# levs57/halo2-liam-eagen-msm

Measured on AMD Instinct MI355X. Metric: BN254 G1 MSM scalar-point-pairs/s, higher is better.
Workload: dtype u32 limbs (256-bit Montgomery integers)

## Files before the change

### halo2_liam_eagen_msm_amd/csrc/fixed_base.inc

```

namespace {

struct FixedPlan { u32 c, W, m, h; u32 kadd[8]; size_t bytes; };

const u32 FIXED_C_MIN = 3, FIXED_C_MAX = 17;

u32 fixed_num_windows(int curve, u32 c, u32 kadd[8]) {
  const u32* order = order_of(curve);
  for (u32 W = (254 + c - 1) / c;; W++) {
    u32 K[8] = {0, 0, 0, 0, 0, 0, 0, 0};
    for (u32 w = 0; w + 1 < W; w++) {
      u32 bit = w * c + c - 1;
      if (bit < 256) K[bit >> 5] |= 1u << (bit & 31);
    }
    u32 s[9]; u64 cy = 0;
    for (int i = 0; i < 8; i++) { cy += (u64)order[i] + K[i] - (i == 0 ? 1u : 0u); s[i] = (u32)cy; cy >>= 32; }
    s[8] = (u32)cy;
    const u32 sh = c * (W - 1);
    u64 top = 0; bool big = s[8] != 0;
    for (int bit = 255; bit >= (int)sh; bit--) {
      if (top >> 62) big = true;
      top = (top << 1) | ((s[bit >> 5] >> (bit & 31)) & 1u);
    }
    if (!big && top < (1ull << (c - 1))) { memcpy(kadd, K, 32); return W; }
  }
}

double fixed_cost(size_t n, u32 c, u32 W, u32 m) {
  const u32 h = (W + m - 1) / m;
  const double slabs = std::ceil((double)n * m / (double)((size_t)1 << MAX_SLAB_LOG));
  return (double)n * W + 2.0 * h * (double)(1u << (c - 1)) + slabs * (double)(1u << 24);
}

const size_t FIXED_AUTO_BYTES = (size_t)16 << 30;

int make_fixed_plan(int curve, size_t n, u32 window_bits, u32 tables, FixedPlan& p) {
  if (curve != LEMSM_BN254_G1 && curve != LEMSM_GRUMPKIN) return LEMSM_ERR_BAD_CURVE;
  if (window_bits && (window_bits < FIXED_C_MIN || window_bits > FIXED_C_MAX)) return LEMSM_ERR_BAD_ARG;
  memset(&p, 0, sizeof p);
  double best = 0; bool have = false;
  for (u32 c = window_bits ? window_bits : FIXED_C_MIN; c <= (window_bits ? window_bits : FIXED_C_MAX); c++) {
    u32 K[8]; const u32 W = fixed_num_windows(curve, c, K);
    if (tables > W) { if (window_bits) return LEMSM_ERR_BAD_ARG; continue; }
    for (u32 m = tables ? tables : 1; m <= (tables ? tables : W); m++) {
      const u32 h = (W + m - 1) / m;
      if (!tables && m > 1 && (W + m - 2) / (m - 1) == h) continue;
      const size_t bytes = (size_t)m * std::max<size_t>(n, 1) * 64;
      if (!tables && m > 1 && bytes > FIXED_AUTO_BYTES) continue;
      const double cost = fixed_cost(n, c, W, m);
      if (!have || cost < best) { best = cost; have = true; p.c = c; p.W = W; p.m = m; p.h = h; memcpy(p.kadd, K, 32); }
    }
  }
  if (!have) return LEMSM_ERR_BAD_ARG;
  p.bytes = (size_t)p.m * n * 64;
  return LEMSM_OK;
}

template <class F>
__global__ __launch_bounds__(256) void k_fixed_table(const uint4* __restrict__ bases, u32 cnt, u32 m, u32 shift,
                                                     uint4* __restrict__ out, char* __restrict__ scratch) {
  typedef XYZZ<F> G; typedef typename F::fe fe;
  const u32 j = blockIdx.x * 256 + threadIdx.x;
  if (j >= cnt) return;
  uint4* o0 = out + (size_t)j * m * 4;
  typename G::aff a;
  F::load(a.x, bases + (size_t)j * 4); F::load(a.y, bases + (size_t)j * 4 + 2);
  for (int q = 0; q < 4; q++) o0[q] = bases[(size_t)j * 4 + q];
  typename G::pt acc; G::from_affine(acc, a);
  fe pref; F::set_one(pref);
  for (u32 k = 1; k < m; k++) {
    for (u32 s = 0; s < shift; s++) { typename G::pt t; G::dbl(t, acc); acc = t; }
    char* sp = scratch + ((size_t)(k - 1) * cnt + j) * 160;
    G::store(sp, acc); F::store(sp + 128, pref);
    if (!G::is_identity(acc)) F::mul(pref, pref, acc.zzz);
  }
  if (m < 2) return;
  fe inv; inv_via_lazy<F>(inv, pref);
  for (u32 k = m - 1; k >= 1; k--) {
    const char* sp = scratch + ((size_t)(k - 1) * cnt + j) * 160;
    typename G::pt q; G::load(q, sp); fe pr; F::load(pr, sp + 128);
    uint4* o = o0 + (size_t)k * 4;
    if (G::is_identity(q)) { uint4 z = make_uint4(0, 0, 0, 0); o[0] = z; o[1] = z; o[2] = z; o[3] = z; continue; }
    fe izzz, izz, x, y;
    F::mul(izzz, inv, pr);
    F::mul(inv, inv, q.zzz);
    F::mul(izz, izzz, q.zz); F::sqr(izz, izz);
    F::mul(x, q.x, izz); F::mul(y, q.y, izzz);
    F::store(o, x); F::store(o + 2, y);
  }
}

struct FixedDigitArgs { KAdd kadd; u32 m, h, W, i0, k0; };

__global__ __launch_bounds__(256) void k_fixed_digits(const uint4* __restrict__ scalars, FixedDigitArgs fa, GroupPlan pl,
                                                      uint16_t* __restrict__ dig16, unsigned long long* __restrict__ signbm,
                                                      u32* __restrict__ block_counts, u32* __restrict__ bin_total, u32* __restrict__ err) {
  __shared__ u32 hist[MAX_BINS];
  const u32 tid = threadIdx.x, r = blockIdx.x;
  for (u32 i = tid; i < pl.nbins; i += 256) hist[i] = 0;
  __syncthreads();
  const u32 c = pl.c, half = 1u << (c - 1);
  const u32 j0 = r * pl.spb, j1 = min(j0 + pl.spb, pl.n);
  for (u32 jb = j0; jb < j1; jb += 256) {
    const u32 j = jb + tid;
    const bool valid = j < j1;
    const u32 kq = fa.k0 + j, q = kq / fa.m, k = kq - q * fa.m;
    const size_t i = (size_t)fa.i0 + q;
    u32 s[8] = {0, 0, 0, 0, 0, 0, 0, 0};
    if (valid) {
      const uint4 a = scalars[2 * i], b = scalars[2 * i + 1];
      s[0] = a.x; s[1] = a.y; s[2] = a.z; s[3] = a.w; s[4] = b.x; s[5] = b.y; s[6] = b.z; s[7] = b.w;
    }
    u32 bw = 0;
#pragma unroll
    for (int w = 0; w < 8; w++) { u32 dmy = __builtin_subc(s[w], fa.kadd.order[w], bw, &bw); (void)dmy; }
    if (valid && !bw) {
      if (k == 0) { atomicAdd(&err[0], 1u); atomicMax(&err[1], ~j); }
#pragma unroll
      for (int w = 0; w < 8; w++) s[w] = 0;
    }
    u32 cy = 0;
#pragma unroll
    for (int w = 0; w < 8; w++) s[w] = __builtin_addc(s[w], fa.kadd.k[w], cy, &cy);
    for (u32 t = pl.w0; t < pl.w1; t++) {
      const u32 ow = k * fa.h + t;
      int d = 0;
      if (valid && ow < fa.W && c * ow < 256) {
        const u32 raw = extract_bits(s, c * ow, c);
        d = (ow + 1 < fa.W) ? (int)raw - (int)half : (int)raw;
      }
      const u32 bucket = (u32)(d < 0 ? -d : d);
      if (c == 17) {
        const u32 neg = d < 0 ? 1u : 0u;
        if (valid) dig16[(size_t)(t - pl.w0) * pl.dstride + j] = (uint16_t)(neg ? bucket - 1u : bucket);
        const unsigned long long bal = __ballot(neg != 0);
        if ((tid & 63u) == 0 && valid) signbm[(size_t)(t - pl.w0) * ((pl.n + 63) / 64) + (j >> 6)] = bal;
      } else if (valid) {
        dig16[(size_t)(t - pl.w0) * pl.dstride + j] = (uint16_t)(d + (int)half);
      }
      if (bucket) atomicAdd(&hist[(t - pl.w0) * pl.BW + ((bucket - 1u) >> pl.LB)], 1u);
    }
  }
  __syncthreads();
  for (u32 i = tid; i < pl.nbins; i += 256) {
    const u32 cnt = hist[i];
    const u32 wl = i / pl.BW, bin = i - wl * pl.BW;
    const size_t slot = ((size_t)wl * pl.nblk1 + r) * pl.BW + bin;
    block_counts[slot] = cnt;
    block_counts[(size_t)pl.nblk1 * pl.nbins + slot] = cnt ? atomicAdd(&bin_total[i], cnt) : 0u;
  }
}

struct FixedProvider {
  const uint4* scalars; FixedDigitArgs fa;
  typedef PipDec Dec;
  int prepare(lemsm_ctx*, hipStream_t st, const GroupPlan& pl, uint16_t* dig16, unsigned long long* signbm, u32* block_counts,
              u32* bin_total, u32* err, Dec& dec) const {
    dec.dig16 = dig16; dec.signbm = pl.c == 17 ? signbm : nullptr;
    hipLaunchKernelGGL(k_fixed_digits, dim3(pl.nblk1), dim3(256), 0, st, scalars, fa, pl, dig16, signbm, block_counts, bin_total, err);
    return LEMSM_OK;
  }
};

}

struct lemsm_fixed_bases { lemsm_ctx* ctx; int device; int curve; size_t n; FixedPlan plan; void* d_table; };

namespace {

template <class P64, class G>
int msm_fixed_t(lemsm_ctx* ctx, const lemsm_fixed_bases* fb, const void* d_scalars, size_t n, u64 out[12]) {
  const FixedPlan& fp = fb->plan;
  const u32 nb = 1u << (fp.c - 1), L = ilog2(nb);
  auto make_src = [&](size_t s0, u32) {
    FixedProvider p; p.scalars = (const uint4*)d_scalars;
    memcpy(p.fa.kadd.k, fp.kadd, 32); memcpy(p.fa.kadd.order, order_of(fb->curve), 32);
    p.fa.m = fp.m; p.fa.h = fp.h; p.fa.W = fp.W; p.fa.i0 = (u32)(s0 / fp.m); p.fa.k0 = (u32)(s0 % fp.m);
    return p;
  };
  std::vector<host::pt> sums;
  int rc = run_windows<P64, G>(ctx, make_src, n * fp.m, fp.c, nb, nb, L, fp.h + 1, 0, fp.h, 0, fb->d_table, sums, true);
  if (rc == LEMSM_ERR_SCALAR_OUT_OF_RANGE) ctx->bad_index /= fp.m;
  if (rc) return rc;
  msm_combine_windows<P64>(fp.c, fp.h, sums.data(), out);
  return LEMSM_OK;
}

}

extern "C" {

int lemsm_fixed_plan(int curve, size_t n, uint32_t window_bits, uint32_t tables, uint32_t* c, uint32_t* num_windows, uint32_t* m,
                     uint32_t* h, size_t* device_bytes) {
  FixedPlan p;
  int rc = make_fixed_plan(curve, n, window_bits, tables, p); if (rc) return rc;
  if (c) *c = p.c;
  if (num_windows) *num_windows = p.W;
  if (m) *m = p.m;
  if (h) *h = p.h;
  if (device_bytes) *device_bytes = p.bytes;
  return LEMSM_OK;
}

int lemsm_fixed_bases_create(lemsm_ctx* ctx, const lemsm_bases* bases, uint32_t window_bits, uint32_t tables, lemsm_fixed_bases** out) {
  if (!ctx || !bases || !out) return LEMSM_ERR_BAD_ARG;
  *out = nullptr;
  if (bases->ctx != ctx) return fail(ctx, LEMSM_ERR_BAD_ARG, "bases belong to another context");
  FixedPlan p;
  int rc = make_fixed_plan(bases->curve, bases->n, window_bits, tables, p);
  if (rc) return fail(ctx, rc, "lemsm_fixed_bases_create: no table geometry for these window_bits / tables");
  HIPCHK(ctx, hipSetDevice(ctx->device));
  const size_t n = bases->n;
  const u32 CHUNK = 1u << 18;
  const size_t scratch_bytes = p.m > 1 ? (size_t)(p.m - 1) * std::min<size_t>(n, CHUNK) * 160 : 0;
  size_t free_b = 0, total_b = 0;
  HIPCHK(ctx, hipMemGetInfo(&free_b, &total_b));
  if (p.bytes + scratch_bytes > free_b) return fail(ctx, LEMSM_ERR_NOMEM, "fixed-base table (" + std::to_string(p.bytes) + " bytes) does not fit in device memory");
  void* d = nullptr;
  hipError_t e = hipMalloc(&d, std::max<size_t>(p.bytes, 64));
  if (e != hipSuccess) { (void)hipGetLastError(); return fail(ctx, LEMSM_ERR_NOMEM, hipGetErrorString(e)); }
  void* scratch = nullptr;
  if (scratch_bytes) {
    e = hipMalloc(&scratch, scratch_bytes);
    if (e != hipSuccess) { (void)hipGetLastError(); (void)hipFree(d); return fail(ctx, LEMSM_ERR_NOMEM, hipGetErrorString(e)); }
  }
  const u32 shift = p.c * p.h;
  for (size_t i0 = 0; i0 < n; i0 += CHUNK) {
    const u32 cnt = (u32)std::min<size_t>(CHUNK, n - i0);
    const uint4* src = (const uint4*)((const char*)bases->d_points + i0 * 64);
    uint4* dst = (uint4*)((char*)d + i0 * p.m * 64);
    if (bases->curve == LEMSM_BN254_G1) hipLaunchKernelGGL((k_fixed_table<FqDev>), dim3((cnt + 255) / 256), dim3(256), 0, ctx->stream, src, cnt, p.m, shift, dst, (char*)scratch);
    else hipLaunchKernelGGL((k_fixed_table<FrDev>), dim3((cnt + 255) / 256), dim3(256), 0, ctx->stream, src, cnt, p.m, shift, dst, (char*)scratch);
  }
  e = hipGetLastError();
  if (e == hipSuccess) e = hipStreamSynchronize(ctx->stream);
  if (scratch) (void)hipFree(scratch);
  if (e != hipSuccess) { (void)hipFree(d); return fail(ctx, LEMSM_ERR_HIP, hipGetErrorString(e)); }
  *out = new lemsm_fixed_bases{ctx, ctx->device, bases->curve, n, p, d};
  return LEMSM_OK;
}

int lemsm_fixed_bases_info(const lemsm_fixed_bases* fb, uint32_t* c, uint32_t* num_windows, uint32_t* m, uint32_t* h, size_t* device_bytes) {
  if (!fb) return LEMSM_ERR_BAD_ARG;
  if (c) *c = fb->plan.c;
  if (num_windows) *num_windows = fb->plan.W;
  if (m) *m = fb->plan.m;
  if (h) *h = fb->plan.h;
  if (device_bytes) *device_bytes = fb->plan.bytes;
  return LEMSM_OK;
}

const void* lemsm_fixed_bases_device_ptr(const lemsm_fixed_bases* fb) { return fb ? fb->d_table : nullptr; }

void lemsm_fixed_bases_free(lemsm_fixed_bases* fb) {
  if (!fb) return;
  (void)hipSetDevice(fb->device);
  (void)hipFree(fb->d_table);
  delete fb;
}

int lemsm_msm_fixed_device(lemsm_ctx* ctx, const lemsm_fixed_bases* fb, const void* d_scalars, size_t n, uint64_t out[12]) {
  if (!ctx || !fb || !out || (n && !d_scalars)) return LEMSM_ERR_BAD_ARG;
  if (fb->ctx != ctx) return fail(ctx, LEMSM_ERR_BAD_ARG, "fixed-base table belongs to another context");
  if (n > fb->n) return fail(ctx, LEMSM_ERR_LEN_MISMATCH, "more scalars than the table has bases");
  if (n == 0) { memset(out, 0, 96); return LEMSM_OK; }
  HIPCHK(ctx, hipSetDevice(ctx->device));
  if (fb->curve == LEMSM_BN254_G1) return msm_fixed_t<host::FqParams64, GqLazy>(ctx, fb, d_scalars, n, out);
  return msm_fixed_t<host::FrParams64, GrLazy>(ctx, fb, d_scalars, n, out);
}

int lemsm_msm_fixed(lemsm_ctx* ctx, const lemsm_fixed_bases* fb, const uint8_t* scalars, size_t n, uint64_t out[12]) {
  if (!ctx || !fb || !out || (n && !scalars)) return LEMSM_ERR_BAD_ARG;
  if (fb->ctx != ctx) return fail(ctx, LEMSM_ERR_BAD_ARG, "fixed-base table belongs to another context");
  if (n > fb->n) return fail(ctx, LEMSM_ERR_LEN_MISMATCH, "more scalars than the table has bases");
  if (n == 0) { memset(out, 0, 96); return LEMSM_OK; }
  HIPCHK(ctx, hipSetDevice(ctx->device));
  int rc = reserve(ctx, ctx->in_s, n * 32); if (rc) return rc;
  HIPCHK(ctx, hipMemcpy(ctx->in_s.p, scalars, n * 32, hipMemcpyHostToDevice));
  return lemsm_msm_fixed_device(ctx, fb, ctx->in_s.p, n, out);
}

}
```

### halo2_liam_eagen_msm_amd/csrc/inst_fq_lazy.hip

```cpp
#include "kernels_ec.cuh"
using namespace lemsm;
typedef XYZZ29<Field29<Fq29Params>> G;
template __global__ void lemsm::k_accum1<G, 2>(GroupPlan, const u32*, const u32*, u32*, const uint4*, char*, u32*, char*);
template __global__ void lemsm::k_accum1<G, 3>(GroupPlan, const u32*, const u32*, u32*, const uint4*, char*, u32*, char*);
template __global__ void lemsm::k_accum1<G, 3, true>(GroupPlan, const u32*, const u32*, u32*, const uint4*, char*, u32*, char*);
template __global__ void lemsm::k_accum1<G, 3, true, true>(GroupPlan, const u32*, const u32*, u32*, const uint4*, char*, u32*, char*);
template __global__ void lemsm::k_accum1<G, 4>(GroupPlan, const u32*, const u32*, u32*, const uint4*, char*, u32*, char*);
template __global__ void lemsm::k_merge_pairs<G>(GroupPlan, u32, MqLayout, const u32*, const u32*, const u32*, const char*, char*, u32*, uint4*);
template __global__ void lemsm::k_merge_serial<G>(u32, MqLayout, const u32*, const uint4*, const char*, char*);
template __global__ void lemsm::k_merge_waves<G>(u32, MqLayout, const u32*, const uint4*, const char*, char*, char*, u32*);
template __global__ void lemsm::k_merge_final<G>(u32, MqLayout, const u32*, const uint4*, const char*, char*, u32*);
template __global__ void lemsm::k_pyramid<G>(const PyrTask*, u32, u32, u32, char*, u32);
template __global__ void lemsm::k_pyramid_first2<G>(PyrFirst2Args, const u32*, char*, u32*);
template __global__ void lemsm::k_pyramid_tail<G>(const PyrTask*, PyrTailArgs, const CopyTaskPod*, u32, char*, u32);
template __global__ void lemsm::k_convert_points<Field29<Fq29Params>>(const uint4*, uint4*, u32);
```

### halo2_liam_eagen_msm_amd/csrc/inst_fq_strict.hip

```cpp
#include "kernels_ec.cuh"
using namespace lemsm;
typedef XYZZ<Field32<FqParams>> G;
template __global__ void lemsm::k_accum1<G, 4>(GroupPlan, const u32*, const u32*, u32*, const uint4*, char*, u32*, char*);
template __global__ void lemsm::k_merge_pairs<G>(GroupPlan, u32, MqLayout, const u32*, const u32*, const u32*, const char*, char*, u32*, uint4*);
template __global__ void lemsm::k_merge_serial<G>(u32, MqLayout, const u32*, const uint4*, const char*, char*);
template __global__ void lemsm::k_merge_waves<G>(u32, MqLayout, const u32*, const uint4*, const char*, char*, char*, u32*);
template __global__ void lemsm::k_merge_final<G>(u32, MqLayout, const u32*, const uint4*, const char*, char*, u32*);
template __global__ void lemsm::k_pyramid<G>(const PyrTask*, u32, u32, u32, char*, u32);
template __global__ void lemsm::k_pyramid_first2<G>(PyrFirst2Args, const u32*, char*, u32*);
template __global__ void lemsm::k_pyramid_tail<G>(const PyrTask*, PyrTailArgs, const CopyTaskPod*, u32, char*, u32);
```

### halo2_liam_eagen_msm_amd/csrc/inst_fr_lazy.hip

```cpp
#include "kernels_ec.cuh"
using namespace lemsm;
typedef XYZZ29<Field29<Fr29Params>> G;
template __global__ void lemsm::k_accum1<G, 2>(GroupPlan, const u32*, const u32*, u32*, const uint4*, char*, u32*, char*);
template __global__ void lemsm::k_accum1<G, 3>(GroupPlan, const u32*, const u32*, u32*, const uint4*, char*, u32*, char*);
template __global__ void lemsm::k_accum1<G, 3, true>(GroupPlan, const u32*, const u32*, u32*, const uint4*, char*, u32*, char*);
template __global__ void lemsm::k_accum1<G, 3, true, true>(GroupPlan, const u32*, const u32*, u32*, const uint4*, char*, u32*, char*);
template __global__ void lemsm::k_accum1<G, 4>(GroupPlan, const u32*, const u32*, u32*, const uint4*, char*, u32*, char*);
template __global__ void lemsm::k_merge_pairs<G>(GroupPlan, u32, MqLayout, const u32*, const u32*, const u32*, const char*, char*, u32*, uint4*);
template __global__ void lemsm::k_merge_serial<G>(u32, MqLayout, const u32*, const uint4*, const char*, char*);
template __global__ void lemsm::k_merge_waves<G>(u32, MqLayout, const u32*, const uint4*, const char*, char*, char*, u32*);
template __global__ void lemsm::k_merge_final<G>(u32, MqLayout, const u32*, const uint4*, const char*, char*, u32*);
template __global__ void lemsm::k_pyramid<G>(const PyrTask*, u32, u32, u32, char*, u32);
template __global__ void lemsm::k_pyramid_first2<G>(PyrFirst2Args, const u32*, char*, u32*);
template __global__ void lemsm::k_pyramid_tail<G>(const PyrTask*, PyrTailArgs, const CopyTaskPod*, u32, char*, u32);
template __global__ void lemsm::k_convert_points<Field29<Fr29Params>>(const uint4*, uint4*, u32);
```

### halo2_liam_eagen_msm_amd/csrc/inst_fr_strict.hip

```cpp
#include "kernels_ec.cuh"
using namespace lemsm;
typedef XYZZ<Field32<FrParams>> G;
template __global__ void lemsm::k_accum1<G, 4>(GroupPlan, const u32*, const u32*, u32*, const uint4*, char*, u32*, char*);
template __global__ void lemsm::k_merge_pairs<G>(GroupPlan, u32, MqLayout, const u32*, const u32*, const u32*, const char*, char*, u32*, uint4*);
template __global__ void lemsm::k_merge_serial<G>(u32, MqLayout, const u32*, const uint4*, const char*, char*);
template __global__ void lemsm::k_merge_waves<G>(u32, MqLayout, const u32*, const uint4*, const char*, char*, char*, u32*);
template __global__ void lemsm::k_merge_final<G>(u32, MqLayout, const u32*, const uint4*, const char*, char*, u32*);
template __global__ void lemsm::k_pyramid<G>(const PyrTask*, u32, u32, u32, char*, u32);
template __global__ void lemsm::k_pyramid_first2<G>(PyrFirst2Args, const u32*, char*, u32*);
template __global__ void lemsm::k_pyramid_tail<G>(const PyrTask*, PyrTailArgs, const CopyTaskPod*, u32, char*, u32);
```

### halo2_liam_eagen_msm_amd/csrc/kernels.cuh

```cuda
#pragma once
#include "kernels_ec.cuh"
#include "inv29.cuh"

namespace lemsm {

__device__ __forceinline__ u32 extract_bits(const u32 (&s)[8], u32 bitpos, u32 c) {
  u32 li = bitpos >> 5, sh = bitpos & 31;
  u32 lo = 0, hi = 0;
#pragma unroll
  for (int i = 0; i < 8; i++) {
    lo = ((u32)i == li) ? s[i] : lo;
    hi = ((u32)i == li + 1) ? s[i] : hi;
  }
  u64 v = ((u64)hi << 32) | lo;
  return (u32)(v >> sh) & ((1u << c) - 1u);
}

struct KAdd { u32 k[8]; u32 order[8]; };

template <int MODE ,
          int BS = 256 >
__global__ __launch_bounds__(BS) void k_pip_digits(const uint4* __restrict__ scalars, KAdd kadd, GroupPlan pl,
                                                    uint16_t* __restrict__ dig16, unsigned long long* __restrict__ signbm,
                                                    u32* __restrict__ block_counts,
                                                    u32* __restrict__ bin_total, u32* __restrict__ err) {
  __shared__ u32 hist[MAX_BINS];
  const u32 tid = threadIdx.x, r = blockIdx.x;
  for (u32 i = tid; i < pl.nbins; i += BS) hist[i] = 0;
  __syncthreads();
  const u32 half = 1u << (pl.c - 1);
  u32 j0 = r * pl.spb, j1 = min(j0 + pl.spb, pl.n);
  for (u32 jb = j0 + tid; jb < j1; jb += BS * 4) {
    uint4 a[4], b[4];
#pragma unroll
    for (int u = 0; u < 4; u++) {
      u32 j = jb + (u32)BS * u;
      if (j < j1) { a[u] = scalars[2 * (size_t)j]; b[u] = scalars[2 * (size_t)j + 1]; }
      else { a[u] = make_uint4(0, 0, 0, 0); b[u] = a[u]; }
    }
#pragma unroll
    for (int u = 0; u < 4; u++) {
      u32 j = jb + (u32)BS * u;
      if (j >= j1) continue;
      u32 s[8] = {a[u].x, a[u].y, a[u].z, a[u].w, b[u].x, b[u].y, b[u].z, b[u].w};
      u32 bw = 0;
#pragma unroll
      for (int i = 0; i < 8; i++) { u32 dmy = __builtin_subc(s[i], kadd.order[i], bw, &bw); (void)dmy; }
      if (!bw) {
        atomicAdd(&err[0], 1u); atomicMax(&err[1], ~j);
#pragma unroll
        for (int i = 0; i < 8; i++) s[i] = 0;
      }
      u32 cy = 0;
#pragma unroll
      for (int i = 0; i < 8; i++) s[i] = __builtin_addc(s[i], kadd.k[i], cy, &cy);
      if (MODE == 2) {
#pragma unroll
        for (int w = 0; w < 15; w++) {
          if ((u32)w < pl.w0 || (u32)w >= pl.w1) continue;
          u32 raw = extract_bits(s, 17u * w, 17u);
          u32 sign = ((u32)w + 1 < pl.W && raw < 65536u) ? 1u : 0u;
          u32 mag = ((u32)w + 1 < pl.W) ? (sign ? 65536u - raw : raw - 65536u) : raw;
          dig16[(size_t)((u32)w - pl.w0) * pl.dstride + j] = (uint16_t)(sign ? mag - 1u : mag);
          unsigned long long bal = __ballot(sign != 0);
          if ((threadIdx.x & 63u) == 0) signbm[(size_t)((u32)w - pl.w0) * ((pl.n + 63) / 64) + (j >> 6)] = bal;
          if (mag) atomicAdd(&hist[((u32)w - pl.w0) * pl.BW + ((mag - 1u) >> pl.LB)], 1u);
        }
      } else if (MODE == 1) {
#pragma unroll
        for (int w = 0; w < 16; w++) {
          if ((u32)w < pl.w0 || (u32)w >= pl.w1) continue;
          u32 raw = (w & 1) ? (s[w >> 1] >> 16) : (s[w >> 1] & 0xffffu);
          dig16[(size_t)((u32)w - pl.w0) * pl.dstride + j] = (uint16_t)raw;
          u32 bucket = ((u32)w + 1 < pl.W) ? (raw < half ? half - raw : raw - half) : raw;
          if (bucket) atomicAdd(&hist[((u32)w - pl.w0) * pl.BW + ((bucket - 1u) >> pl.LB)], 1u);
        }
      } else {
        for (u32 w = pl.w0; w < pl.w1; w++) {
          u32 raw = extract_bits(s, w * pl.c, pl.c);
          dig16[(size_t)(w - pl.w0) * pl.dstride + j] = (uint16_t)raw;
          u32 bucket = (w + 1 < pl.W) ? (raw < half ? half - raw : raw - half) : raw;
          if (bucket) atomicAdd(&hist[(w - pl.w0) * pl.BW + ((bucket - 1u) >> pl.LB)], 1u);
        }
      }
    }
  }
  __syncthreads();
  for (u32 i = tid; i < pl.nbins; i += BS) {
    u32 cnt = hist[i];
    u32 wl = i / pl.BW, bin = i - wl * pl.BW;
    const size_t slot = ((size_t)wl * pl.nblk1 + r) * pl.BW + bin;
    block_counts[slot] = cnt;
    block_counts[(size_t)pl.nblk1 * pl.nbins + slot] = cnt ? atomicAdd(&bin_total[i], cnt) : 0u;
  }
}

struct PipDec {
  static constexpr bool VEC = true;
  const uint16_t* dig16;
  const unsigned long long* signbm;
  __device__ __forceinline__ void get(u32 j, u32 w, const GroupPlan& pl, u32& bucket, u32& sign) const {
    u32 raw = dig16[(size_t)(w - pl.w0) * pl.dstride + j];
    if (signbm) {
      sign = (u32)(signbm[(size_t)(w - pl.w0) * ((pl.n + 63) / 64) + (j >> 6)] >> (j & 63u)) & 1u;
      bucket = sign ? raw + 1u : raw;
      return;
    }
    const u32 half = 1u << (pl.c - 1);
    if (w + 1 < pl.W) {
      sign = raw < half ? 1u : 0u;
      bucket = sign ? half - raw : raw - half;
    } else { sign = 0; bucket = raw; }
  }
};
struct NegDec {
  static constexpr bool VEC = false;
  const uint8_t* digitsT;
  __device__ __forceinline__ void get(u32 j, u32 w, const GroupPlan& pl, u32& bucket, u32& sign) const {
    bucket = digitsT[(size_t)w * pl.nstride + j]; sign = 0;
  }
};

__device__ __forceinline__ u32 block_excl_scan_256(u32 v, u32* total, u32* wsum ) {
  const u32 lane = threadIdx.x & 63, wave = threadIdx.x >> 6;
  u32 x = v;
#pragma unroll
  for (int o = 1; o < 64; o <<= 1) {
    u32 y = __shfl_up(x, o);
    if (lane >= (u32)o) x += y;
  }
  if (lane == 63) wsum[wave] = x;
  __syncthreads();
  u32 base = 0, tot = 0;
#pragma unroll
  for (u32 w = 0; w < 4; w++) {
    u32 s = wsum[w];
    if (w < wave) base += s;
    tot += s;
  }
  __syncthreads();
  *total = tot;
  return base + x - v;
}

static const u32 BW_MAX = 512;
static const u32 STAGE = 4096;
static const u32 STAGE2 = 8192;

template <class Dec>
__global__ __launch_bounds__(256) void k_count1(Dec dec, GroupPlan pl, u32* __restrict__ block_counts,
                                                u32* __restrict__ bin_total) {
  __shared__ u32 hist[256];
  const u32 tid = threadIdx.x, wl = blockIdx.x, r = blockIdx.y, w = pl.w0 + wl;
  hist[tid] = 0;
  __syncthreads();
  u32 j0 = r * pl.spb, j1 = min(j0 + pl.spb, pl.n);
  constexpr int PER = STAGE / 256;
  u32 bk[PER];
#pragma unroll
  for (int k = 0; k < PER; k++) {
    u32 j = j0 + tid + 256u * k, sign;
    bk[k] = 0;
    if (j < j1) dec.get(j, w, pl, bk[k], sign);
  }
  const bool few = pl.BW <= 16u;
  const u32 rep = few ? (tid & 15u) << 4 : 0u;
#pragma unroll
  for (int k = 0; k < PER; k++)
    if (bk[k]) atomicAdd(&hist[rep + ((bk[k] - 1u) >> pl.LB)], 1u);
  __syncthreads();
  if (few) {
    u32 c = 0;
    if (tid < 16u) {
#pragma unroll
      for (int r = 0; r < 16; r++) c += hist[r * 16 + tid];
    }
    __syncthreads();
    if (tid < 16u) hist[tid] = c;
    __syncthreads();
  }
  if (tid < pl.BW) {
    u32 cnt = hist[tid];
    const size_t slot = ((size_t)wl * pl.nblk1 + r) * pl.BW + tid;
    block_counts[slot] = cnt;
    block_counts[(size_t)pl.nblk1 * pl.nbins + slot] = cnt ? atomicAdd(&bin_total[wl * pl.BW + tid], cnt) : 0u;
  }
}

__device__ __forceinline__ u32 block_excl_scan_1024(u32 v, u32* total, u32* wsum ) {
  const u32 lane = threadIdx.x & 63, wave = threadIdx.x >> 6;
  u32 x = v;
#pragma unroll
  for (int o = 1; o < 64; o <<= 1) {
    u32 y = __shfl_up(x, o);
    if (lane >= (u32)o) x += y;
  }
  if (lane == 63) wsum[wave] = x;
  __syncthreads();
  u32 base = 0, tot = 0;
  for (u32 w = 0; w < 16; w++) {
    u32 s = wsum[w];
    if (w < wave) base += s;
    tot += s;
  }
  __syncthreads();
  *total = tot;
  return base + x - v;
}

__global__ __launch_bounds__(1024) void k_binscan(GroupPlan pl, const u32* __restrict__ bin_total,
                                                  u32* __restrict__ bin_start, u32* __restrict__ tile_prefix,
                                                  u32* __restrict__ meta) {
  __shared__ u32 wsum[16];
  const u32 t = threadIdx.x;
  constexpr int PB = MAX_BINS / 1024;
  u32 cnt[PB], tl[PB], s = 0, st = 0;
#pragma unroll
  for (int k = 0; k < PB; k++) {
    u32 b = t * PB + k;
    cnt[k] = b < pl.nbins ? bin_total[b] : 0;
    tl[k] = (pl.bin_cap && cnt[k] <= pl.bin_cap) ? 0u : (cnt[k] + pl.T2 - 1) / pl.T2;
    s += cnt[k]; st += tl[k];
  }
  u32 tot, tott;
  u32 off = block_excl_scan_1024(s, &tot, wsum);
  u32 offt = block_excl_scan_1024(st, &tott, wsum);
#pragma unroll
  for (int k = 0; k < PB; k++) {
    u32 b = t * PB + k;
    if (b < pl.nbins) { bin_start[b] = off; tile_prefix[b] = offt; }
    off += cnt[k]; offt += tl[k];
  }
  if (t == 0) {
    bin_start[pl.nbins] = tot; tile_prefix[pl.nbins] = tott;
    meta[META_M] = tot; meta[META_TILES] = tott;
  }
}

template <class Dec, int STG , int BS = 256,
          bool LEAN = false >
__global__ __launch_bounds__(BS) void k_scatter1(Dec dec, GroupPlan pl, const u32* __restrict__ block_counts,
                                                 const u32* __restrict__ bin_start,
                                                 u32* __restrict__ entries, u32 xcd_windows ) {
  static_assert(BS == 256 || BS == 1024, "block size");
  static_assert(STG <= 16384, "jl field is 14 bits");
  static_assert(!LEAN || BS == 256, "the lean form is the 256-thread one");
  __shared__ __align__(8) u32 delta[BW_MAX];
  __shared__ __align__(8) u32 lcur[BW_MAX];
  __shared__ u32 wsum[16];
  __shared__ u32 stage[STG];
  const u32 tid = threadIdx.x;
  u32 wl, r;
  if (xcd_windows) {
    const u32 wpx = (pl.w1 - pl.w0 + 7u) >> 3, slot = blockIdx.x >> 3;
    wl = (blockIdx.x & 7u) + 8u * (slot % wpx); r = slot / wpx;
    if (wl >= pl.w1 - pl.w0) return;
  } else { wl = blockIdx.x; r = blockIdx.y; }
  const u32 w = pl.w0 + wl;
  const u32 lmask = (1u << pl.LB) - 1u;
  u32 j0 = r * pl.spb, j1 = min(j0 + pl.spb, pl.n);
  constexpr int PER = STG / BS;
  u32 bk[PER];
  u32 jl0, jls;
  if constexpr (Dec::VEC) {
    static_assert(PER == 16 || PER == 32, "digits per thread");
    jl0 = tid * PER; jls = 1;
    const u32 jb = j0 + jl0;
    uint4 dv[PER / 8];
    u32 sbits = 0;
    if (jb < j1) {
      const uint4* p = (const uint4*)(dec.dig16 + (size_t)wl * pl.dstride + jb);
#pragma unroll
      for (int v = 0; v < PER / 8; v++) dv[v] = p[v];
      if (dec.signbm) {
        const unsigned long long* sw = dec.signbm + (size_t)wl * ((pl.n + 63) / 64);
        if (PER == 16) sbits = ((const uint16_t*)sw)[jb >> 4]; else sbits = ((const u32*)sw)[jb >> 5];
      }
    } else {
#pragma unroll
      for (int v = 0; v < PER / 8; v++) dv[v] = make_uint4(0, 0, 0, 0);
    }
    const u32 half = 1u << (pl.c - 1);
    const bool top = !(w + 1 < pl.W);
#pragma unroll
    for (int k = 0; k < PER; k++) {
      const uint4 q4 = dv[k / 8];
      const u32 word = ((k / 2) % 4 == 0) ? q4.x : ((k / 2) % 4 == 1) ? q4.y : ((k / 2) % 4 == 2) ? q4.z : q4.w;
      const u32 raw = (k & 1) ? (word >> 16) : (word & 0xffffu);
      u32 bucket, sign;
      if (dec.signbm) { sign = (sbits >> k) & 1u; bucket = raw + sign; }
      else if (top) { sign = 0; bucket = raw; }
      else { sign = raw < half ? 1u : 0u; bucket = sign ? half - raw : raw - half; }
      bk[k] = (jb + (u32)k < j1 && bucket) ? (bucket | (sign << 31)) : 0u;
    }
  } else {
    jl0 = tid; jls = BS;
#pragma unroll
    for (int k = 0; k < PER; k++) {
      u32 j = j0 + tid + (u32)BS * k, b = 0, sgn = 0;
      if (j < j1) dec.get(j, w, pl, b, sgn);
      bk[k] = b ? (b | (sgn << 31)) : 0u;
    }
  }
  const size_t crow = ((size_t)wl * pl.nblk1 + r) * pl.BW;
  const u32* __restrict__ block_offs = block_counts + (size_t)pl.nblk1 * pl.nbins;
  u32 total;
  const bool few = !Dec::VEC && BS == 256 && !LEAN && pl.BW <= 16u;
  if (few) {
    lcur[tid] = 0;
    __syncthreads();
#pragma unroll
    for (int k = 0; k < PER; k++)
      if (bk[k]) atomicAdd(&lcur[((((bk[k] & 0x7fffffffu) - 1u) >> pl.LB) << 4) | (tid & 15u)], 1u);
    __syncthreads();
    const u32 v = lcur[tid];
    const u32 off = block_excl_scan_256(v, &total, wsum);
    lcur[tid] = off;
    const u32 b = tid >> 4;
    if ((tid & 15u) == 0 && b < pl.BW) delta[b] = bin_start[wl * pl.BW + b] + block_offs[crow + b] - off;
  } else
  if constexpr (LEAN) {
    const u32 b0 = 2u * tid;
    const bool h = b0 < pl.BW;
    const uint2 z2 = make_uint2(0u, 0u);
    const uint2 cnt = h ? *reinterpret_cast<const uint2*>(block_counts + crow + b0) : z2;
    const uint2 clm = h ? *reinterpret_cast<const uint2*>(block_offs + crow + b0) : z2;
    const uint2 bs = h ? *reinterpret_cast<const uint2*>(bin_start + (size_t)wl * pl.BW + b0) : z2;
    const u32 off0 = block_excl_scan_256(cnt.x + cnt.y, &total, wsum), off1 = off0 + cnt.x;
    *reinterpret_cast<uint2*>(&delta[b0]) = make_uint2(bs.x + clm.x - off0, bs.y + clm.y - off1);
    *reinterpret_cast<uint2*>(&lcur[b0]) = make_uint2(off0, off1);
  } else if constexpr (BS == 256) {
    const bool h0 = tid < pl.BW, h1 = tid + 256u < pl.BW;
    u32 cnt0 = h0 ? block_counts[crow + tid] : 0u, cnt1 = h1 ? block_counts[crow + tid + 256u] : 0u;
    u32 g0 = h0 ? bin_start[wl * pl.BW + tid] + block_offs[crow + tid] : 0u;
    u32 g1 = h1 ? bin_start[wl * pl.BW + tid + 256u] + block_offs[crow + tid + 256u] : 0u;
    u32 total0, total1;
    u32 off0 = block_excl_scan_256(cnt0, &total0, wsum);
    u32 off1 = block_excl_scan_256(cnt1, &total1, wsum) + total0;
    total = total0 + total1;
    delta[tid] = g0 - off0; delta[tid + 256u] = g1 - off1;
    lcur[tid] = off0; lcur[tid + 256u] = off1;
  } else {
    const bool h0 = tid < pl.BW;
    u32 cnt0 = h0 ? block_counts[crow + tid] : 0u;
    u32 g0 = h0 ? bin_start[wl * pl.BW + tid] + block_offs[crow + tid] : 0u;
    u32 off0 = block_excl_scan_1024(cnt0, &total, wsum);
    if (tid < BW_MAX) { delta[tid] = g0 - off0; lcur[tid] = off0; }
  }
  __syncthreads();
#pragma unroll
  for (int k = 0; k < PER; k++) {
    if (bk[k]) {
      u32 kk = (bk[k] & 0x7fffffffu) - 1u, b = kk >> pl.LB;
      u32 q = atomicAdd(&lcur[few ? ((b << 4) | (tid & 15u)) : b], 1u);
      if constexpr (LEAN) stage[q] = (bk[k] & 0x80000000u) | (jl0 + jls * (u32)k) | (b << 14) | ((kk & lmask) << 24);
      else stage[q] = (jl0 + jls * (u32)k) | ((kk & lmask) << 14) | ((bk[k] >> 31) << 21) | (b << 22);
    }
  }
  __syncthreads();
  if constexpr (LEAN) {
    u32 v[PER];
#pragma unroll
    for (int k = 0; k < PER; k++) { const u32 q = tid + (u32)BS * k; v[k] = q < total ? stage[q] : 0u; }
#pragma unroll
    for (int k = 0; k < PER; k++) {
      const u32 q = tid + (u32)BS * k;
      if (q < total) entries[delta[(v[k] >> 14) & 511u] + q] = (v[k] & 0xff003fffu) + j0;
    }
  } else {
    for (u32 q = tid; q < total; q += BS) {
      u32 v = stage[q];
      entries[delta[v >> 22] + q] = (j0 + (v & 0x3fffu)) | (((v >> 14) & 127u) << 24) | (((v >> 21) & 1u) << 31);
    }
  }
}

__global__ __launch_bounds__(256) void k_tilemap(GroupPlan pl, const u32* __restrict__ bin_start,
                                                 const u32* __restrict__ tile_prefix, const u32* __restrict__ meta,
                                                 uint4* __restrict__ tile_info) {
  u32 t = blockIdx.x * 256 + threadIdx.x;
  if (t >= pl.max_tiles) return;
  if (t >= meta[META_TILES]) { tile_info[t] = make_uint4(0, 0, 0, 0); return; }
  u32 lo = 0, hi = pl.nbins;
  while (hi - lo > 1) {
    u32 mid = (lo + hi) >> 1;
    if (tile_prefix[mid] <= t) lo = mid; else hi = mid;
  }
  u32 off = bin_start[lo] + (t - tile_prefix[lo]) * pl.T2;
  u32 end = min(off + pl.T2, bin_start[lo + 1]);
  tile_info[t] = make_uint4(lo, off, end, 1u);
}
__device__ __forceinline__ bool locate_tile(const uint4* __restrict__ tile_info, u32 t, u32& bin, u32& off, u32& end) {
  uint4 ti = tile_info[t];
  bin = ti.x; off = ti.y; end = ti.z;
  return ti.w != 0;
}

__global__ __launch_bounds__(256) void k_count2(GroupPlan pl, const u32* __restrict__ entries,
                                                const uint4* __restrict__ tile_info, u32* __restrict__ bucket_count) {
  __shared__ u32 hist[1u << MAX_LB];
  const u32 tid = threadIdx.x;
  for (u32 t = blockIdx.x; t < pl.max_tiles; t += gridDim.x) {
    u32 bin, off, end;
    if (!locate_tile(tile_info, t, bin, off, end)) return;
    if (tid < (1u << MAX_LB)) hist[tid] = 0;
    __syncthreads();
    constexpr int PER = STAGE2 / 256;
    u32 e[PER];
#pragma unroll
    for (int k = 0; k < PER; k++) { u32 i = off + tid + 256u * k; e[k] = i < end ? entries[i] : 0xffffffffu; }
#pragma unroll
    for (int k = 0; k < PER; k++) { u32 i = off + tid + 256u * k; if (i < end) atomicAdd(&hist[(e[k] >> 24) & 127u], 1u); }
    __syncthreads();
    if (tid < (1u << pl.LB)) {
      u32 cnt = hist[tid];
      if (cnt) atomicAdd(&bucket_count[(bin << pl.LB) + tid], cnt);
    }
    __syncthreads();
  }
}

__global__ __launch_bounds__(256) void k_bucketscan(GroupPlan pl, const u32* __restrict__ bin_start,
                                                    const u32* __restrict__ bucket_count,
                                                    u32* __restrict__ bucket_start) {
  __shared__ u32 ex[256];
  __shared__ u32 wsum[4];
  const u32 tid = threadIdx.x;
  const u32 key = blockIdx.x * 256 + tid;
  const u32 nkeys = pl.nbins << pl.LB;
  u32 cnt = key < nkeys ? bucket_count[key] : 0u;
  u32 total;
  u32 e = block_excl_scan_256(cnt, &total, wsum);
  ex[tid] = e;
  __syncthreads();
  if (key < nkeys) {
    u32 first = tid & ~((1u << pl.LB) - 1u);
    const u32 b0 = bin_start[key >> pl.LB];
    if (!(pl.bin_cap && bin_start[(key >> pl.LB) + 1] - b0 <= pl.bin_cap))
      bucket_start[key] = b0 + (e - ex[first]);
  }
  if (key == 0) bucket_start[nkeys] = bin_start[pl.nbins];
}

__global__ __launch_bounds__(256) void k_scatter2(GroupPlan pl, const u32* __restrict__ entries,
                                                  const uint4* __restrict__ tile_info, const u32* __restrict__ bucket_start,
                                                  u32* __restrict__ bucket_cursor, u32* __restrict__ sorted) {
  __shared__ u32 hist[256];
  __shared__ u32 lstart[257];
  __shared__ u32 delta[256];
  __shared__ u32 wsum[4];
  __shared__ u32 stage[STAGE2];
  const u32 tid = threadIdx.x;
  for (u32 t = blockIdx.x; t < pl.max_tiles; t += gridDim.x) {
    u32 bin, off, end;
    if (!locate_tile(tile_info, t, bin, off, end)) return;
    hist[tid] = 0;
    __syncthreads();
    constexpr int PER = STAGE2 / 256;
    u32 e[PER], rk[PER];
#pragma unroll
    for (int k = 0; k < PER; k++) { u32 i = off + tid + 256u * k; e[k] = i < end ? entries[i] : 0xffffffffu; }
#pragma unroll
    for (int k = 0; k < PER; k++) {
      u32 i = off + tid + 256u * k;
      rk[k] = i < end ? atomicAdd(&hist[(e[k] >> 24) & 127u], 1u) : 0u;
    }
    __syncthreads();
    u32 cnt = tid < (1u << pl.LB) ? hist[tid] : 0u;
    u32 total;
    u32 o = block_excl_scan_256(cnt, &total, wsum);
    lstart[tid] = o;
    if (tid == 255) lstart[256] = total;
    u32 key = (bin << pl.LB) + tid;
    delta[tid] = cnt ? bucket_start[key] + atomicAdd(&bucket_cursor[key], cnt) - o : 0u;
    __syncthreads();
#pragma unroll
    for (int k = 0; k < PER; k++) {
      u32 i = off + tid + 256u * k;
      if (i < end) {
        u32 l = (e[k] >> 24) & 127u;
        stage[lstart[l] + rk[k]] = e[k];
      }
    }
    __syncthreads();
    for (u32 q = tid; q < total; q += 256) {
      u32 v = stage[q];
      sorted[delta[(v >> 24) & 127u] + q] = v & 0x80ffffffu;
    }
    __syncthreads();
  }
}

static const u32 BIN_CAP = 36864;
static const u32 BIN_CAP_SMALL = 8192;
template <u32 CAP>
__global__ __launch_bounds__(1024) void k_binsort(GroupPlan pl, const u32* __restrict__ entries, const u32* __restrict__ bin_start,
                                                  u32* __restrict__ sorted, u32* __restrict__ bucket_start) {
  __shared__ u32 stage[CAP];
  __shared__ u32 hist[256];
  __shared__ u32 lstart[256];
  __shared__ u32 wsum[4];
  const u32 tid = threadIdx.x, bin = blockIdx.x;
  const u32 off = bin_start[bin], end = bin_start[bin + 1], cnt = end - off;
  if (cnt > pl.bin_cap) return;
  const u32 nl = 1u << pl.LB, lmask = nl - 1u;
  if (tid < 256) hist[tid] = 0;
  __syncthreads();
  constexpr int PER = CAP / 1024;
  u32 e[PER], rk[PER];
#pragma unroll
  for (int k = 0; k < PER; k++) { u32 i = off + tid + 1024u * k; e[k] = i < end ? entries[i] : 0u; }
#pragma unroll
  for (int k = 0; k < PER; k++) {
    u32 i = off + tid + 1024u * k;
    rk[k] = i < end ? atomicAdd(&hist[(e[k] >> 24) & lmask], 1u) : 0u;
  }
  __syncthreads();
  if (tid < 256) {
    u32 c = tid < nl ? hist[tid] : 0u, total;
    const u32 lane = tid & 63, wave = tid >> 6;
    u32 x = c;
#pragma unroll
    for (int o = 1; o < 64; o <<= 1) { u32 y = __shfl_up(x, o); if (lane >= (u32)o) x += y; }
    if (lane == 63) wsum[wave] = x;
    lstart[tid] = x - c;
    (void)total;
  }
  __syncthreads();
  const u32 wb1 = wsum[0], wb2 = wb1 + wsum[1], wb3 = wb2 + wsum[2];
  if (tid < nl) {
    u32 l = tid, base = l < 64 ? 0u : (l < 128 ? wb1 : (l < 192 ? wb2 : wb3));
    bucket_start[(bin << pl.LB) + l] = off + base + lstart[l];
  }
#pragma unroll
  for (int k = 0; k < PER; k++) {
    u32 i = off + tid + 1024u * k;
    if (i < end) {
      u32 l = (e[k] >> 24) & lmask, base = l < 64 ? 0u : (l < 128 ? wb1 : (l < 192 ? wb2 : wb3));
      stage[base + lstart[l] + rk[k]] = e[k] & 0x80ffffffu;
    }
  }
  __syncthreads();
  for (u32 q = tid; q < cnt; q += 1024) sorted[off + q] = stage[q];
}

__global__ void k_copy_points(const CopyTask* __restrict__ tasks, u32 ntasks, u32 nwin, u32 pt_bytes, char* __restrict__ arena) {
  u32 gid = blockIdx.x * blockDim.x + threadIdx.x;
  u32 wpp = pt_bytes / 16;
  u32 word = gid % wpp; u32 r = gid / wpp;
  u32 ti = r / nwin, w = r - ti * nwin;
  if (ti >= ntasks) return;
  CopyTask tk = tasks[ti];
  uint4 v = make_uint4(0, 0, 0, 0);
  if (tk.src_idx < tk.src_valid_idx)
    v = reinterpret_cast<const uint4*>(arena + ((size_t)tk.src_off + (size_t)w * tk.src_wstride + tk.src_idx) * pt_bytes)[word];
  reinterpret_cast<uint4*>(arena + ((size_t)tk.dst_off + (size_t)w * tk.dst_wstride) * pt_bytes)[word] = v;
}

__global__ __launch_bounds__(256) void k_negbase_digits(const uint4* __restrict__ scalars, u32 n, u32 base, u32 d,
                                                        const u32* __restrict__ bound , int check_range,
                                                        uint8_t* __restrict__ digits, uint8_t* __restrict__ digitsT,
                                                        u32* __restrict__ err, u32 row_begin, u32 row_end ,
                                                        const uint8_t* __restrict__ negative = nullptr ,
                                                        uint8_t* __restrict__ trunc = nullptr ) {
  u32 j = blockIdx.x * 256 + threadIdx.x;
  if (j >= n) return;
  uint4 a = scalars[2 * (size_t)j], b = scalars[2 * (size_t)j + 1];
  u32 s[8] = {a.x, a.y, a.z, a.w, b.x, b.y, b.z, b.w};
  u32 bw = 0;
#pragma unroll
  for (int i = 0; i < 8; i++) { u32 dummy = __builtin_subc(s[i], bound[i], bw, &bw); (void)dummy; }
  bool in_range = bw != 0;
  if (check_range && !in_range) { atomicMin(&err[0], j); }
  u32 h[16];
#pragma unroll
  for (int i = 0; i < 8; i++) { h[2 * i] = s[i] & 0xffffu; h[2 * i + 1] = s[i] >> 16; }
  bool neg = negative ? negative[j] != 0 : false;
  {
    u32 nz0 = 0;
#pragma unroll
    for (int k = 0; k < 16; k++) nz0 |= h[k];
    if (!nz0) neg = false;
  }
  const float rb = 1.0f / (float)base;
  const u32 shift = (base & (base - 1u)) == 0 ? (u32)__builtin_ctz(base) : 0u;
  u32 i_begin = 0;
  if (shift && !(s[4] | s[5] | s[6] | s[7])) {
    u32 m0 = s[0], m1 = s[1], m2 = s[2], m3 = s[3];
    for (u32 i = 0; i < d; i++) {
      const u32 rem = m0 & (base - 1u);
      m0 = __builtin_amdgcn_alignbit(m1, m0, shift); m1 = __builtin_amdgcn_alignbit(m2, m1, shift);
      m2 = __builtin_amdgcn_alignbit(m3, m2, shift); m3 >>= shift;
      u32 digit;
      if (!neg) { digit = rem; neg = true; }
      else {
        digit = rem ? base - rem : 0u;
        if (rem) {
          m0 += 1u; const u32 c0 = m0 == 0u; m1 += c0; const u32 c1 = c0 & (m1 == 0u); m2 += c1; const u32 c2 = c1 & (m2 == 0u); m3 += c2;
        }
        neg = false;
      }
      if (!(m0 | m1 | m2 | m3)) neg = false;
      if (digits) digits[(size_t)j * d + i] = (uint8_t)digit;
      if (digitsT && i >= row_begin && i < row_end) digitsT[(size_t)i * n + j] = (uint8_t)digit;
    }
    h[0] = m0 & 0xffffu; h[1] = m0 >> 16; h[2] = m1 & 0xffffu; h[3] = m1 >> 16; h[4] = m2 & 0xffffu; h[5] = m2 >> 16; h[6] = m3 & 0xffffu; h[7] = m3 >> 16;
    i_begin = d;
  }
  for (u32 i = i_begin; i < d; i++) {
    u32 rem = 0;
    if (shift) {
      rem = h[0] & (base - 1u);
#pragma unroll
      for (int k = 0; k < 16; k++) {
        u32 nxt = k < 15 ? h[k + 1] : 0u;
        h[k] = ((h[k] | (nxt << 16)) >> shift) & 0xffffu;
      }
    } else {
#pragma unroll
      for (int k = 15; k >= 0; k--) {
        u32 cur = (rem << 16) | h[k];
        u32 q = (u32)((float)cur * rb);
        int r = (int)cur - (int)(q * base);
        if (r < 0) { q--; r += (int)base; }
        if (r >= (int)base) { q++; r -= (int)base; }
        h[k] = q; rem = (u32)r;
      }
    }
    u32 digit;
    if (!neg) { digit = rem; neg = true; }
    else {
      digit = rem ? base - rem : 0u;
      if (rem) {
        u32 cy = 1;
#pragma unroll
        for (int k = 0; k < 16; k++) { u32 v = h[k] + cy; h[k] = v & 0xffffu; cy = v >> 16; }
      }
      neg = false;
    }
    u32 nz = 0;
#pragma unroll
    for (int k = 0; k < 16; k++) nz |= h[k];
    if (!nz) neg = false;
    if (digits) digits[(size_t)j * d + i] = (uint8_t)digit;
    if (digitsT && i >= row_begin && i < row_end) digitsT[(size_t)i * n + j] = (uint8_t)digit;
  }
  u32 nz = 0;
// ... 165 lines not shown
```

### halo2_liam_eagen_msm_amd/csrc/kernels_ec.cuh

```cuda
#pragma once
#include "plan.h"
#include "xyzz.cuh"
#include "xyzz29.cuh"

namespace lemsm {

static const u32 KEY_NONE = 0xffffffffu;

enum { META_M = 0, META_TILES = 1, META_WORDS = 4, META_CLOCK = 8  };

template <class G, int WPS ,
          bool ABI = false ,
          bool RING = false >
__global__ __launch_bounds__(256, WPS) void k_accum1(GroupPlan pl, const u32* __restrict__ sorted,
                                                const u32* __restrict__ bucket_start, u32* __restrict__ meta,
                                                const uint4* __restrict__ points, char* __restrict__ bucket_sum,
                                                u32* __restrict__ rec_key, char* __restrict__ rec_pt) {
  typedef typename G::F_ F;
  typedef typename F::fe fe;
  const u32 t = blockIdx.x * 256 + threadIdx.x;
  if (t >= pl.nthr1) return;
  const u32 M = meta[META_M];
  const bool stamp = blockIdx.x == (gridDim.x >> 1) && threadIdx.x == 0;
  if (stamp) {
    u64* ck = reinterpret_cast<u64*>(meta + META_CLOCK);
    ck[0] = __builtin_amdgcn_s_memtime(); ck[1] = __builtin_amdgcn_s_memrealtime();
  }
  const u64 s64 = (u64)t * pl.L1;
  const u32 r0 = 2 * t;
  if (s64 >= M) { rec_key[t] = KEY_NONE; return; }
  const u32 start = (u32)s64;
  const u32 end = (u32)min((u64)M, s64 + pl.L1);

  u32 lo = 0, hi = pl.nbins << pl.LB;
  while (hi - lo > 1) {
    u32 mid = (lo + hi) >> 1;
    if (bucket_start[mid] <= start) lo = mid; else hi = mid;
  }
  const u32 nkeys = pl.nbins << pl.LB;
  u32 key = lo;
  u32 kbeg = bucket_start[key];
  u32 kend = bucket_start[key + 1];
  u32 kend2 = bucket_start[min(key + 2u, nkeys)], kend3 = bucket_start[min(key + 3u, nkeys)];
  u32 seg_begin = start;

  typename G::pt acc; G::set_identity(acc);
  bool empty = true;

  auto flush = [&](u32 seg_end) {
    bool complete = (seg_begin == kbeg) && (seg_end == kend);
    if (complete) {
      G::store(bucket_sum + (size_t)key * G::PT_BYTES, acc);
    } else {
      G::store(rec_pt + (size_t)(r0 + (seg_end == end ? 1u : 0u)) * G::PT_BYTES, acc);
    }
  };

  __shared__ u32 ering[RING ? 4 : 1][2][4][64][RING ? 4 : 1];
  const u32 wv = threadIdx.x >> 6, lane = threadIdx.x & 63u;
  auto ring_fill = [&](u32 blk) {
#pragma unroll
    for (int k = 0; k < 4; k++)
      __builtin_amdgcn_global_load_lds((const __attribute__((address_space(1))) void*)(sorted + start + 16u * blk + 4u * k),
                                       (__attribute__((address_space(3))) void*)&ering[wv][blk & 1u][k][0][0], 16, 0, 0);
  };
  auto ring_read = [&](u32 rel) -> u32 { return ering[wv][(rel >> 4) & 1u][(rel >> 2) & 3u][lane][rel & 3u]; };
  u32 e_next;
  if constexpr (RING) {
    ring_fill(0);
    if (pl.L1 > 16) ring_fill(1);
    asm volatile("s_waitcnt vmcnt(0)" ::: "memory");
    e_next = ring_read(0);
  } else {
    e_next = sorted[start];
  }
  uint4 nx0, nx1, ny0, ny1;
  { const uint4* p = points + (size_t)(e_next & 0xffffffu) * 4; nx0 = p[0]; nx1 = p[1]; ny0 = p[2]; ny1 = p[3]; }

  for (u32 i = start; i < end; i++) {
    u32 e = e_next; fe px, py;
    F::from_words(px, nx0, nx1); F::from_words(py, ny0, ny1);
    if (i >= kend) {
      flush(i);
      key++; kend = kend2; kend2 = kend3;
      while (i >= kend) { key++; kend = kend2; kend2 = bucket_start[min(key + 2u, nkeys)]; }
      kbeg = i; seg_begin = i;
      G::set_identity(acc); empty = true;
    }
    if (i + 1 < end) {
      if constexpr (RING) {
        const u32 rel1 = i + 1 - start;
        if ((rel1 & 15u) == 0) asm volatile("s_waitcnt vmcnt(0)" ::: "memory");
        e_next = ring_read(rel1);
        if ((rel1 & 15u) == 0 && rel1 + 16u < pl.L1) ring_fill((rel1 >> 4) + 1u);
      } else {
        e_next = sorted[i + 1];
      }
      const uint4* p = points + (size_t)(e_next & 0xffffffu) * 4;
      nx0 = p[0]; nx1 = p[1]; ny0 = p[2]; ny1 = p[3];
    }
    kend3 = bucket_start[min(key + 3u, nkeys)];
    if (!G::aff_is_identity(px, py)) {
      F::cneg(py, py, (e >> 31) != 0);
      if (ABI) G::madd_abi(acc, px, py, empty); else G::madd(acc, px, py, empty);
    }
  }
  flush(end);
  if (stamp) {
    u64* ck = reinterpret_cast<u64*>(meta + META_CLOCK);
    ck[2] = __builtin_amdgcn_s_memtime(); ck[3] = __builtin_amdgcn_s_memrealtime();
  }
  rec_key[t] = (seg_begin == kbeg && end != kend) ? key : KEY_NONE;
}

enum { MQ_S = 0, MQ_M = 1, MQ_L = 2, MQ_F = 3, MQ_P = 4, MQ_WORDS = 16  };
static const u32 MQ_DST_BUCKET = 0xffffffffu;

template <class G>
__device__ __forceinline__ void merge_load_piece(typename G::pt& q, const char* __restrict__ rec_pt, u32 t, bool first_slot, u32 scaled) {
  G::load(q, rec_pt + (size_t)(2u * t + (first_slot ? 0u : 1u)) * G::PT_BYTES);
  if (scaled) G::unscale(q);
}

template <class G>
__global__ __launch_bounds__(256) void k_merge_pairs(GroupPlan pl, u32 scaled, MqLayout lay, const u32* __restrict__ bucket_start,
                                                     const u32* __restrict__ meta, const u32* __restrict__ rec_key,
                                                     const char* __restrict__ rec_pt, char* __restrict__ bucket_sum,
                                                     u32* __restrict__ mq_cnt, uint4* __restrict__ mq_items) {
  __shared__ u32 lc[5], lbase[5];
  const u32 t = blockIdx.x * 256 + threadIdx.x;
  if (threadIdx.x < 5) lc[threadIdx.x] = 0;
  __syncthreads();
  const u32 key = t < pl.nthr1 ? rec_key[t] : KEY_NONE;
  u32 P = 0, lastfirst = 0, cls = 0, loff = 0, nsub = 0, poff = 0, foff = 0;
  if (key != KEY_NONE) {
    const u32 e = bucket_start[key + 1], M = meta[META_M];
    const u32 tb = (e - 1u) / pl.L1;
    P = tb - t + 1u;
    lastfirst = ((u64)(tb + 1u) * pl.L1 == (u64)e || e == M) ? 0u : 1u;
    cls = P == 2 ? 1u : (P <= 8 ? 2u : (P <= 32 ? 3u : 4u));
    if (cls == 2) loff = atomicAdd(&lc[MQ_S], 1u);
    else if (cls == 3) loff = atomicAdd(&lc[MQ_M], 1u);
    else if (cls == 4) {
      nsub = (P + lay.slice - 1u) / lay.slice;
      loff = atomicAdd(&lc[MQ_L], nsub);
      if (nsub > 1) { poff = atomicAdd(&lc[MQ_P], nsub); foff = atomicAdd(&lc[MQ_F], 1u); }
    }
  }
  __syncthreads();
  if (threadIdx.x < 5) lbase[threadIdx.x] = lc[threadIdx.x] ? atomicAdd(&mq_cnt[threadIdx.x], lc[threadIdx.x]) : 0u;
  __syncthreads();
  if (cls == 2) { u32 i = lbase[MQ_S] + loff; if (i < lay.capS) mq_items[lay.offS + i] = make_uint4(key, t, P | (lastfirst << 31), MQ_DST_BUCKET); }
  else if (cls == 3) { u32 i = lbase[MQ_M] + loff; if (i < lay.capM) mq_items[lay.offM + i] = make_uint4(key, t, P | (lastfirst << 31), MQ_DST_BUCKET); }
  else if (cls == 4) {
    const u32 i0 = lbase[MQ_L] + loff, p0 = lbase[MQ_P] + poff;
    for (u32 k = 0; k < nsub; k++) {
      const u32 cnt = min(lay.slice, P - k * lay.slice);
      const u32 lf = (k + 1 == nsub) ? lastfirst : 0u;
      if (i0 + k < lay.capL) mq_items[lay.offL + i0 + k] = make_uint4(key, t + k * lay.slice, cnt | (lf << 31), nsub > 1 ? p0 + k : MQ_DST_BUCKET);
    }
    if (nsub > 1) { u32 f = lbase[MQ_F] + foff; if (f < lay.capF) mq_items[lay.offF + f] = make_uint4(key, p0, nsub, 0); }
  }
  if (cls == 1) {
    typename G::pt acc, q;
    merge_load_piece<G>(acc, rec_pt, t, false, scaled);
    merge_load_piece<G>(q, rec_pt, t + 1u, lastfirst != 0, scaled);
    G::add(acc, q);
    if (scaled) G::scale(acc);
    G::store(bucket_sum + (size_t)key * G::PT_BYTES, acc);
  }
}

template <class G, bool FROM_PARTIALS>
__device__ __forceinline__ u32 merge_wave_sum(typename G::pt& acc, u32 lane, u32 n, u32 t0, u32 lf, u32 scaled,
                                              const char* __restrict__ src, u32 cap) {
  G::set_identity(acc);
  u32 m = 1; while (m < n && m < 64u) m <<= 1;
  const u32 nser = (n + 63u) >> 6;
  const u32 nscan = m <= 16u ? (u32)__builtin_ctz(m) : (m == 32u ? 5u : 6u);
#pragma unroll 1
  for (u32 s = 0; s < nser + nscan; s++) {
    typename G::pt q;
    if (s < nser) {
      const u32 j = (lane & (m - 1u)) + 64u * s;
      if (j < n) {
        if constexpr (FROM_PARTIALS) { if (t0 + j < cap) G::load(q, src + (size_t)(t0 + j) * G::PT_BYTES); else G::set_identity(q); }
        else merge_load_piece<G>(q, src, t0 + j, j + 1 == n && lf, scaled);
      } else G::set_identity(q);
    } else {
      G::scan_fetch(q, acc, (int)(s - nser));
    }
    G::add(acc, q);
  }
  return m - 1u;
}

static const u32 MERGE_LDS_PAD_WORDS = 21504;

template <class G>
__global__ __launch_bounds__(256) void k_merge_serial(u32 scaled, MqLayout lay, const u32* __restrict__ mq_cnt,
                                                      const uint4* __restrict__ mq_items, const char* __restrict__ rec_pt,
                                                      char* __restrict__ bucket_sum) {
  __shared__ u32 pad_[MERGE_LDS_PAD_WORDS];
  if (scaled > 1) pad_[threadIdx.x] = scaled;
  const u32 cS = min(mq_cnt[MQ_S], lay.capS), cMall = min(mq_cnt[MQ_M], lay.capM);
  const u32 cM = cMall > lay.wave_th ? cMall : 0u;
  const u32 chS = (cS + 63u) >> 6, chM = (cM + 63u) >> 6;
  const u32 lane = threadIdx.x & 63u;
#pragma unroll 1
  for (u32 c = blockIdx.x + gridDim.x * (threadIdx.x >> 6); c < chS + chM; c += gridDim.x * 4u) {
    uint4 it;
    if (c < chS) { const u32 v = 64u * c + lane; if (v >= cS) continue; it = mq_items[lay.offS + v]; }
    else { const u32 v = 64u * (c - chS) + lane; if (v >= cM) continue; it = mq_items[lay.offM + v]; }
    const u32 key = it.x, t0 = it.y, n = it.z & 0x7fffffffu, lf = it.z >> 31;
    typename G::pt acc, q; G::set_identity(acc);
#pragma unroll 1
    for (u32 j = 0; j < n; j++) {
      merge_load_piece<G>(q, rec_pt, t0 + j, j + 1 == n && lf, scaled);
      G::add(acc, q);
    }
    if (scaled) G::scale(acc);
    G::store(bucket_sum + (size_t)key * G::PT_BYTES, acc);
  }
}

template <class G>
__global__ __launch_bounds__(256) void k_merge_waves(u32 scaled, MqLayout lay, const u32* __restrict__ mq_cnt,
                                                     const uint4* __restrict__ mq_items, const char* __restrict__ rec_pt,
                                                     char* __restrict__ partial, char* __restrict__ bucket_sum, u32* __restrict__ dbg) {
  __shared__ u32 pad_[MERGE_LDS_PAD_WORDS];
  if (scaled > 1) pad_[threadIdx.x] = scaled;
  const unsigned long long tk0 = __builtin_amdgcn_s_memtime();
  const u32 cMall = min(mq_cnt[MQ_M], lay.capM), cL = min(mq_cnt[MQ_L], lay.capL);
  const u32 lane = threadIdx.x & 63u;
  const u32 nwaves = gridDim.x * 4u;
  const u32 cM = cMall > lay.wave_th ? 0u : cMall;
#pragma unroll 1
  for (u32 w = blockIdx.x * 4u + (threadIdx.x >> 6); w < cM + cL; w += nwaves) {
    const uint4 it = w < cM ? mq_items[lay.offM + w] : mq_items[lay.offL + (w - cM)];
    const u32 key = it.x, dst = it.w;
    typename G::pt acc;
    const unsigned long long tk1 = __builtin_amdgcn_s_memtime();
    const u32 rl = merge_wave_sum<G, false>(acc, lane, it.z & 0x7fffffffu, it.y, it.z >> 31, scaled, rec_pt, 0);
    const unsigned long long tk2 = __builtin_amdgcn_s_memtime();
    if (lane == rl) {
      if (dst == MQ_DST_BUCKET) { if (scaled) G::scale(acc); G::store(bucket_sum + (size_t)key * G::PT_BYTES, acc); }
      else if (dst < lay.capP) G::store(partial + (size_t)dst * G::PT_BYTES, acc);
    }
    if (dbg && w == 0 && lane == 0) { dbg[8] = (u32)(tk1 - tk0); dbg[9] = (u32)(tk2 - tk1); dbg[10] = (u32)(__builtin_amdgcn_s_memtime() - tk2); dbg[11] = it.z; }
  }
}

template <class G>
__global__ __launch_bounds__(256) void k_merge_final(u32 scaled, MqLayout lay, const u32* __restrict__ mq_cnt, const uint4* __restrict__ mq_items,
                                                     const char* __restrict__ partial, char* __restrict__ bucket_sum, u32* __restrict__ dbg) {
  __shared__ u32 pad_[MERGE_LDS_PAD_WORDS];
  if (scaled > 1) pad_[threadIdx.x] = scaled;
  const unsigned long long tk0 = __builtin_amdgcn_s_memtime();
  const u32 cF = min(mq_cnt[MQ_F], lay.capF);
  const u32 lane = threadIdx.x & 63u, nwaves = gridDim.x * 4u;
#pragma unroll 1
  for (u32 w = blockIdx.x * 4u + (threadIdx.x >> 6); w < cF; w += nwaves) {
    const uint4 it = mq_items[lay.offF + w];
    typename G::pt acc;
    const unsigned long long tk1 = __builtin_amdgcn_s_memtime();
    const u32 rl = merge_wave_sum<G, true>(acc, lane, it.z, it.y, 0, 0, partial, lay.capP);
    const unsigned long long tk2 = __builtin_amdgcn_s_memtime();
    if (lane == rl) { if (scaled) G::scale(acc); G::store(bucket_sum + (size_t)it.x * G::PT_BYTES, acc); }
    if (dbg && w == 0 && lane == 0) { dbg[12] = (u32)(tk1 - tk0); dbg[13] = (u32)(tk2 - tk1); dbg[14] = (u32)(__builtin_amdgcn_s_memtime() - tk2); dbg[15] = it.z; }
  }
}

typedef CopyTask CopyTaskPod;


template <class G>
__device__ __forceinline__ void pyr_item(const PyrTask& tk, u32 w, u32 i, char* __restrict__ arena) {
  u32 ia = (2 * i) * tk.stride + tk.phase, ib = (2 * i + 1) * tk.stride + tk.phase;
  const char* src = arena + ((size_t)tk.src_off + (size_t)w * tk.src_wstride) * G::PT_BYTES;
  typename G::pt a, b;
  if (ia < tk.src_valid) G::load(a, src + (size_t)ia * G::PT_BYTES); else G::set_identity(a);
  if (ib < tk.src_valid) G::load(b, src + (size_t)ib * G::PT_BYTES); else G::set_identity(b);
  if (tk.src_scaled) { G::unscale(a); G::unscale(b); }
  G::add(a, b);
  G::store(arena + ((size_t)tk.dst_off + (size_t)w * tk.dst_wstride + i) * G::PT_BYTES, a);
}

template <class G>
__device__ __forceinline__ bool pyr_try4(const PyrTask& tk, u32 w, u32 i, char* __restrict__ arena, u32 q) {
  if constexpr (G::CONVERTED_DOMAIN) {
    const u32 ia = (2 * i) * tk.stride + tk.phase, ib = (2 * i + 1) * tk.stride + tk.phase;
    if (ia >= tk.src_valid || ib >= tk.src_valid || tk.src_scaled) return false;
    const char* src = arena + ((size_t)tk.src_off + (size_t)w * tk.src_wstride) * G::PT_BYTES;
    return G::add4_mem(src + (size_t)ia * G::PT_BYTES, src + (size_t)ib * G::PT_BYTES,
                       arena + ((size_t)tk.dst_off + (size_t)w * tk.dst_wstride + i) * G::PT_BYTES, q);
  } else return false;
}

template <class G>
__global__ __launch_bounds__(256) void k_pyramid(const PyrTask* __restrict__ tasks, u32 ntasks, u32 nwin,
                                                 u32 max_count, char* __restrict__ arena, u32 quad ) {
  const u32 t = blockIdx.x * 256 + threadIdx.x;
  const u32 gid = quad ? t >> 2 : t;
  u32 per_task = max_count * nwin;
  u32 ti = gid / per_task;
  if (ti >= ntasks) return;
  u32 rem = gid - ti * per_task;
  u32 w = rem / max_count, i = rem - w * max_count;
  PyrTask tk = tasks[ti];
  if (i >= tk.count) return;
  bool serial = true;
  if (quad) serial = !pyr_try4<G>(tk, w, i, arena, t & 3u) && (t & 3u) == 0u;
  if (serial) pyr_item<G>(tk, w, i, arena);
}

template <class G>
__global__ __launch_bounds__(256) void k_sum_slabs(char* __restrict__ bucket_sum, u32 nbuckets, u32 nslabs, u32 scaled_mask) {
  const u32 i = blockIdx.x * 256 + threadIdx.x;
  if (i >= nbuckets) return;
  typename G::pt acc, q;
  G::load(acc, bucket_sum + (size_t)i * G::PT_BYTES);
  if (scaled_mask & 1u) G::unscale(acc);
#pragma unroll 1
  for (u32 k = 1; k < nslabs; k++) {
    G::load(q, bucket_sum + ((size_t)k * nbuckets + i) * G::PT_BYTES);
    if ((scaled_mask >> k) & 1u) G::unscale(q);
    G::add(acc, q);
  }
  G::store(bucket_sum + (size_t)i * G::PT_BYTES, acc);
}


struct PyrFirst2Args {
  u32 nwin, nb, nbw, nbp;
  u32 bucket_off, a2_off, r02_off, r11_off, wstride;
  u32 scaled;
};

template <class G>
__global__ __launch_bounds__(256, 1) void k_pyramid_first2(PyrFirst2Args a, const u32* __restrict__ bucket_start, char* __restrict__ arena, u32* __restrict__ dbg) {
  const unsigned long long tk0 = __builtin_amdgcn_s_memtime(), tr0 = __builtin_amdgcn_s_memrealtime();
  const u32 gid = blockIdx.x * 256 + threadIdx.x;
  const u32 per_win = a.nbp >> 3;
  const u32 w = gid / per_win, i = gid - w * per_win;
  if (w >= a.nwin) return;
  const u32 key0 = w * a.nbw + 8u * i;
  typename G::pt A, B, D, x, y;
  G::set_identity(A); G::set_identity(B); G::set_identity(D);
  const size_t o_a2 = (size_t)a.a2_off + (size_t)w * a.wstride + 2u * i;
  const size_t o_r02 = (size_t)a.r02_off + (size_t)w * a.wstride + i, o_r11 = (size_t)a.r11_off + (size_t)w * a.wstride + i;
  auto operands = [&](u32 step, u32& kx, u32& ky, size_t& tx, size_t& ty) {
    kx = 8; ky = 8; tx = ~(size_t)0; ty = ~(size_t)0;
    switch (step) {
      case 0: kx = 0; ky = 1; break;
      case 1: kx = 2; ky = 3; break;
      case 3: ty = o_r11; break;
      case 4: kx = 4; ky = 5; break;
      case 5: ky = 7; break;
      case 6: tx = o_r02; break;
      case 7: kx = 6; ky = 7; break;
      case 9: tx = o_r11; break;
      default: break;
    }
    if (kx < 8) tx = (size_t)a.bucket_off + key0 + kx;
    if (ky < 8) ty = (size_t)a.bucket_off + key0 + ky;
  };
  uint4 rx[G::RAW_WORDS], ry[G::RAW_WORDS];
  {
    u32 kx, ky; size_t tx, ty; operands(0, kx, ky, tx, ty);
    G::load_raw(rx, arena + tx * G::PT_BYTES); G::load_raw(ry, arena + ty * G::PT_BYTES);
  }
  u32 have = 0;
#pragma unroll
  for (u32 k = 0; k < 8; k++)
    if (8u * i + k < a.nb && bucket_start[key0 + k + 1] != bucket_start[key0 + k]) have |= 1u << k;
#pragma unroll 1
  for (u32 step = 0; step < 10; step++) {
    {
      u32 kx, ky; size_t tx, ty; operands(step, kx, ky, tx, ty);
      if (tx != ~(size_t)0) { G::from_raw(x, rx); if (kx < 8) { if (!((have >> kx) & 1u)) G::set_identity(x); else if (a.scaled) G::unscale(x); } }
      if (ty != ~(size_t)0) { G::from_raw(y, ry); if (ky < 8) { if (!((have >> ky) & 1u)) G::set_identity(y); else if (a.scaled) G::unscale(y); } }
      if (step < 9) {
        operands(step + 1, kx, ky, tx, ty);
        if (tx != ~(size_t)0) G::load_raw(rx, arena + tx * G::PT_BYTES);
        if (ty != ~(size_t)0) G::load_raw(ry, arena + ty * G::PT_BYTES);
      }
    }
    switch (step) {
      case 0: B = y; break;
      case 1: D = y; break;
      case 2: x = B; y = D; break;
      case 3: x = A; break;
      case 4: D = y; break;
      case 5: x = D; break;
      case 6: y = D; break;
      case 8: x = A; y = B; break;
      case 9: y = B; break;
      default: break;
    }
    const unsigned long long ta0 = __builtin_amdgcn_s_memtime();
    G::add(x, y);
    if (dbg && gid == 0) { if (step == 2) dbg[8] = (u32)(__builtin_amdgcn_s_memtime() - ta0); if (step == 0) dbg[9] = (u32)(__builtin_amdgcn_s_memtime() - tk0); }
    size_t dst = ~(size_t)0;
    switch (step) {
      case 0: A = x; break;
      case 1: dst = o_r11; break;
      case 2: dst = o_r02; break;
      case 3: dst = o_a2; break;
      case 4: A = x; break;
      case 5: D = x; break;
      case 6: dst = o_r02; break;
      case 7: B = x; break;
      case 8: dst = o_a2 + 1; break;
      default: dst = o_r11; break;
    }
    if (dst != ~(size_t)0) G::store(arena + dst * G::PT_BYTES, x);
  }
  if (dbg && gid == 0) { dbg[10] = (u32)(__builtin_amdgcn_s_memtime() - tk0); dbg[11] = (u32)(__builtin_amdgcn_s_memrealtime() - tr0); }
}

struct PyrTailArgs { u32 first, last, max_count[20], step_off[21]; };
template <class G>
__global__ __launch_bounds__(1024) __attribute__((amdgpu_waves_per_eu(4, 4))) void k_pyramid_tail(const PyrTask* __restrict__ tasks, PyrTailArgs ta, const CopyTaskPod* __restrict__ copy,
                                                       u32 do_copy, char* __restrict__ arena, u32 quad ) {
  const u32 w = blockIdx.x, tid = threadIdx.x;
  for (u32 s = ta.first; s <= ta.last; s++) {
    const u32 k = s - ta.first;
    const u32 nt = ta.step_off[k + 1] - ta.step_off[k], mc = ta.max_count[k];
    const u32 lanes = quad ? 4u * nt * mc : nt * mc;
    for (u32 t = tid; t < lanes; t += 1024) {
      const u32 it = quad ? t >> 2 : t;
      const u32 ti = it / mc, i = it - ti * mc;
      PyrTask tk = tasks[ta.step_off[k] + ti];
      bool serial = i < tk.count;
      if (quad && serial) serial = !pyr_try4<G>(tk, w, i, arena, t & 3u) && (t & 3u) == 0u;
      if (serial) pyr_item<G>(tk, w, i, arena);
    }
    __threadfence_block();
    __syncthreads();
  }
  if (do_copy) {
    const u32 wpp = G::PT_BYTES / 16;
    if (tid < wpp) {
      CopyTaskPod tk = *copy;
      uint4 v = make_uint4(0, 0, 0, 0);
      if (tk.src_idx < tk.src_valid_idx)
        v = reinterpret_cast<const uint4*>(arena + ((size_t)tk.src_off + (size_t)w * tk.src_wstride + tk.src_idx) * G::PT_BYTES)[tid];
      reinterpret_cast<uint4*>(arena + ((size_t)tk.dst_off + (size_t)w * tk.dst_wstride) * G::PT_BYTES)[tid] = v;
    }
  }
}

template <class F29>
__global__ __launch_bounds__(256) void k_convert_points(const uint4* __restrict__ in, uint4* __restrict__ out, u32 n) {
  u32 i = blockIdx.x * 256 + threadIdx.x;
  if (i >= 2 * n) return;
  typename F29::fe a, r;
  F29::load(a, in + 2 * (size_t)i);
  F29::from_abi(r, a);
  F29::store(out + 2 * (size_t)i, r);
}

}
```

### halo2_liam_eagen_msm_amd/csrc/lemsm.hip

```cpp
#include <hip/hip_runtime.h>
#include <math.h>
#include <stdio.h>
#include <stdlib.h>
#include <string.h>

#include <algorithm>
#include <cmath>
#include <map>
#include <string>
#include <vector>

#include "../../include/lemsm.h"
#include "hostmath.hpp"
#include "hostpool.hpp"
#include "hosttail.hpp"
#include <memory>
#include "kernels.cuh"
#include "rccl_dyn.hpp"
#include "roctx_dyn.hpp"
#include "divisor.cuh"
#include "regfn_eval.cuh"
#include <rocprim/rocprim.hpp>
#include <chrono>
#include <functional>
#include <thread>

using namespace lemsm;

namespace {

typedef Field32<FqParams> FqDev;
typedef Field32<FrParams> FrDev;
typedef XYZZ<FqDev> GqStrict;
typedef XYZZ<FrDev> GrStrict;
typedef XYZZ29<Field29<Fq29Params>> GqLazy;
typedef XYZZ29<Field29<Fr29Params>> GrLazy;

const u32 ORDER_R[8] = {0xf0000001u, 0x43e1f593u, 0x79b97091u, 0x2833e848u, 0x8181585du, 0xb85045b6u, 0xe131a029u, 0x30644e72u};
const u32 ORDER_P[8] = {0xd87cfd47u, 0x3c208c16u, 0x6871ca8du, 0x97816a91u, 0x8181585du, 0xb85045b6u, 0xe131a029u, 0x30644e72u};
const u32 BOUND_R[8] = {0xc7b81b1bu, 0xc6fb4e9fu, 0xeeb859fcu, 0x6f4d8248u, 0, 0, 0, 0};
const u32 BOUND_P[8] = {0xc7b81b1cu, 0xc6fb4e9fu, 0xeeb859fcu, 0x6f4d8248u, 0, 0, 0, 0};

const u32* order_of(int curve) { return curve == LEMSM_BN254_G1 ? ORDER_R : ORDER_P; }
const u32* bound_of(int curve) { return curve == LEMSM_BN254_G1 ? BOUND_R : BOUND_P; }

}
#define LEMSM_EXTERN_G(G)                                                                                   \
  extern template __global__ void lemsm::k_merge_pairs<G>(GroupPlan, u32, MqLayout, const u32*, const u32*, const u32*, const char*, char*, u32*, uint4*); \
  extern template __global__ void lemsm::k_merge_serial<G>(u32, MqLayout, const u32*, const uint4*, const char*, char*); \
  extern template __global__ void lemsm::k_merge_waves<G>(u32, MqLayout, const u32*, const uint4*, const char*, char*, char*, u32*); \
  extern template __global__ void lemsm::k_merge_final<G>(u32, MqLayout, const u32*, const uint4*, const char*, char*, u32*); \
  extern template __global__ void lemsm::k_pyramid<G>(const PyrTask*, u32, u32, u32, char*, u32); \
  extern template __global__ void lemsm::k_pyramid_first2<G>(PyrFirst2Args, const u32*, char*, u32*); \
  extern template __global__ void lemsm::k_pyramid_tail<G>(const PyrTask*, PyrTailArgs, const CopyTaskPod*, u32, char*, u32);
#define LEMSM_EXTERN_ACC(G, W) \
  extern template __global__ void lemsm::k_accum1<G, W>(GroupPlan, const u32*, const u32*, u32*, const uint4*, char*, u32*, char*);
LEMSM_EXTERN_G(GqStrict) LEMSM_EXTERN_G(GrStrict) LEMSM_EXTERN_G(GqLazy) LEMSM_EXTERN_G(GrLazy)
LEMSM_EXTERN_ACC(GqStrict, 4) LEMSM_EXTERN_ACC(GrStrict, 4)
LEMSM_EXTERN_ACC(GqLazy, 2) LEMSM_EXTERN_ACC(GqLazy, 3) LEMSM_EXTERN_ACC(GqLazy, 4)
LEMSM_EXTERN_ACC(GrLazy, 2) LEMSM_EXTERN_ACC(GrLazy, 3) LEMSM_EXTERN_ACC(GrLazy, 4)
extern template __global__ void lemsm::k_accum1<GqLazy, 3, true>(GroupPlan, const u32*, const u32*, u32*, const uint4*, char*, u32*, char*);
extern template __global__ void lemsm::k_accum1<GrLazy, 3, true>(GroupPlan, const u32*, const u32*, u32*, const uint4*, char*, u32*, char*);
extern template __global__ void lemsm::k_accum1<GqLazy, 3, true, true>(GroupPlan, const u32*, const u32*, u32*, const uint4*, char*, u32*, char*);
extern template __global__ void lemsm::k_accum1<GrLazy, 3, true, true>(GroupPlan, const u32*, const u32*, u32*, const uint4*, char*, u32*, char*);
extern template __global__ void lemsm::k_convert_points<Field29<Fq29Params>>(const uint4*, uint4*, u32);
extern template __global__ void lemsm::k_convert_points<Field29<Fr29Params>>(const uint4*, uint4*, u32);
namespace {

struct DevBuf {
  void* p = nullptr;
  size_t cap = 0;
};


struct PyrCacheEntry { DevBuf buf; PyrPlan pp; };

}

struct HostStage { const uint8_t* h_scalars; const void* h_points; char* d_scalars; char* d_points; };

struct lemsm_ctx {
  int device = 0;
  u32 num_cus = 256;
  hipStream_t stream = nullptr;
  hipStream_t stream_sort = nullptr;
  hipStream_t stream_tail = nullptr;
  std::vector<hipEvent_t> evpool;
  hipEvent_t wait_accum = nullptr;
  hipEvent_t ev_call_done = nullptr;
  hipEvent_t ev_batch_up = nullptr;
  hipEvent_t dw_ev[2] = {nullptr, nullptr};
  hipEvent_t ev[5] = {nullptr, nullptr, nullptr, nullptr, nullptr};
  DevBuf ws;
  DevBuf in_s;
  DevBuf in_p;
  DevBuf in_aux;
  DevBuf gather;
  DevBuf fail_buf;
  DevBuf dw_tab, dw_arena, dw_tmp;
  u32 dw_logn = 0, dw_gexp = 0;
  double dw_ntt_ms = 0; u64 dw_ntt_bytes = 0, dw_ntt_bflies = 0; u32 dw_reuse_levels = 0;
  DevBuf rf_coef, rf_ws;
  double rf_ms = 0; u64 rf_bytes = 0, rf_mults = 0;
  double dw_phase_ms[4] = {0, 0, 0, 0};
  ncclComm_t comm = nullptr; int comm_size = 1, comm_rank = 0;
  int plan_world = 1;
  u32* h_small = nullptr;
  lemsm_ctx* peer = nullptr;
  void* h_pin = nullptr; size_t h_pin_cap = 0;
  std::unique_ptr<lemsm::host::Pool> pool;
  std::string last_error;
  long opt_host_threads = 0;
  long opt_window_bits = 0, opt_chunk = 0, opt_tile = 0, opt_field = 0, opt_accum_waves = 0, opt_groups = 0, opt_host_slab_bits = 0, opt_slab_bits = 0, opt_abi_points = 0, opt_stage2x = 0, opt_xcd_windows = 0, opt_entry_ring = 0, opt_validate_points = 0, opt_pyr_fuse = 0, opt_ntt_tiled = 0, opt_ws_canary = 0, opt_binsort = 0, opt_dw_wrap = 0, opt_dw_fuse = 0, opt_dw_kb = 0, opt_merge_slice = 0, opt_merge_wave_th = 0, opt_dbg_repeat = 0, opt_pyr_first2 = 0, opt_dw_reuse = 0, opt_dw_pw_lazy = 0, opt_dw_halves = 0, opt_dw_ntt_lazy = 0, opt_slab_tail = 0, opt_pyr_quad = 0, opt_scatter_lean = 0;
  u32 plan_slab_n = 0;
  bool plan_ring = false;
  const struct HostStage* host_stage = nullptr;
  double t_total_ms = 0, t_accum_ms = 0; int n_accum = 0;
  double host_us[4] = {0, 0, 0, 0};
  uint32_t dbg_stamps[8] = {0, 0, 0, 0, 0, 0, 0, 0};
  uint64_t dbg_merge[4] = {0, 0, 0, 0};
  double accum_clock_mhz = 0;
  size_t bad_index = 0;
  size_t truncated = 0;
  std::map<std::vector<u32>, PyrCacheEntry> pyr_cache;
};

namespace {

#define HIPCHK(ctx, expr)                                                                   \
  do {                                                                                      \
    hipError_t e_ = (expr);                                                                 \
    if (e_ != hipSuccess) {                                                                 \
      (ctx)->last_error = std::string(#expr) + ": " + hipGetErrorString(e_);                \
      return LEMSM_ERR_HIP;                                                                 \
    }                                                                                       \
  } while (0)

int fail(lemsm_ctx* ctx, int code, const std::string& msg) {
  if (ctx) ctx->last_error = msg;
  return code;
}

int reserve(lemsm_ctx* ctx, DevBuf& b, size_t bytes) {
  if (b.cap >= bytes) return LEMSM_OK;
  if (b.p) { HIPCHK(ctx, hipFree(b.p)); b.p = nullptr; b.cap = 0; }
  size_t want = bytes + bytes / 8 + 4096;
  hipError_t e = hipMalloc(&b.p, want);
  if (e != hipSuccess) { b.p = nullptr; return fail(ctx, LEMSM_ERR_NOMEM, "hipMalloc failed: " + std::string(hipGetErrorString(e))); }
  b.cap = want;
  return LEMSM_OK;
}

int reserve_pinned(lemsm_ctx* ctx, size_t bytes) {
  if (ctx->h_pin_cap >= bytes) return LEMSM_OK;
  if (ctx->h_pin) { HIPCHK(ctx, hipHostFree(ctx->h_pin)); ctx->h_pin = nullptr; ctx->h_pin_cap = 0; }
  size_t want = bytes + bytes / 4 + 4096;
  hipError_t e = hipHostMalloc(&ctx->h_pin, want, hipHostMallocDefault);
  if (e != hipSuccess) { ctx->h_pin = nullptr; return fail(ctx, LEMSM_ERR_NOMEM, "hipHostMalloc failed: " + std::string(hipGetErrorString(e))); }
  ctx->h_pin_cap = want;
  return LEMSM_OK;
}

void host_parallel(lemsm_ctx* ctx, int njobs, const std::function<void(int)>& fn) {
  if (!ctx || njobs <= 1 || ctx->opt_host_threads == 1) { for (int i = 0; i < njobs; i++) fn(i); return; }
  int want = ctx->opt_host_threads > 1 ? (int)ctx->opt_host_threads : std::min(8, lemsm::host::Pool::usable_cpus());
  if (!ctx->pool || ctx->pool->workers() != want - 1) ctx->pool.reset(new lemsm::host::Pool(std::max(0, want - 1)));
  ctx->pool->run(njobs, fn);
}

bool geq8(const u32* a, const u32* b) {
  for (int i = 7; i >= 0; i--) { if (a[i] > b[i]) return true; if (a[i] < b[i]) return false; }
  return true;
}
void add8(u32* r, const u32* a, const u32* b) {
  u64 c = 0;
  for (int i = 0; i < 8; i++) { c += (u64)a[i] + b[i]; r[i] = (u32)c; c >>= 32; }
}
u32 logb_ceil8(const u32* x, u32 base) {
  u32 m[8]; memcpy(m, x, 32); u32 i = 0;
  for (;;) {
    u32 nz = 0; for (int k = 0; k < 8; k++) nz |= m[k];
    if (!nz) break;
    u64 rem = 0;
    for (int k = 7; k >= 0; k--) { u64 cur = (rem << 32) | m[k]; m[k] = (u32)(cur / base); rem = cur % base; }
    i++;
  }
  return i;
}
u32 next_pow2(u32 x) { u32 p = 1; while (p < x) p <<= 1; return p; }
u32 ilog2(u32 x) { u32 l = 0; while ((1u << l) < x) l++; return l; }

struct MsmPlan {
  u32 c, W, nb, nbp, L;
  u32 kadd[8];
};

u32 choose_c(const lemsm_ctx* ctx, size_t n) {
  if (ctx && ctx->opt_window_bits >= 2 && ctx->opt_window_bits <= 17) return (u32)ctx->opt_window_bits;
  u32 lg = 0; while (((size_t)1 << (lg + 1)) <= n) lg++;
  if (lg >= 24) return (ctx && ctx->plan_world > 1) ? 16u : 17u;
  int c = (int)lg - 3;
  if (c < 3) c = 3;
  if (c > 16) c = 16;
  return (u32)c;
}

u32 host_slab_log(const lemsm_ctx* ctx, size_t n) {
  u32 lg = 0; while (((size_t)2 << lg) <= n) lg++;
  u32 auto_log = std::min(21u, std::max(19u, lg >= 2 ? lg - 2 : 0u));
  if (ctx->host_stage && !ctx->host_stage->h_points) auto_log = std::min(22u, std::max(19u, lg >= 2 ? lg - 2 : 0u));
  return std::min<u32>(MAX_SLAB_LOG, ctx->opt_host_slab_bits ? (u32)ctx->opt_host_slab_bits : auto_log);
}

MsmPlan make_msm_plan(const lemsm_ctx* ctx, int curve, size_t n) {
  MsmPlan p; memset(&p, 0, sizeof p);
  size_t n_pass = n;
  if (ctx && ctx->host_stage) n_pass = std::min(n, (size_t)1 << host_slab_log(ctx, n));
  else if (ctx && ctx->opt_slab_bits) n_pass = std::min(n, (size_t)1 << ctx->opt_slab_bits);
  p.c = choose_c(ctx, n_pass);
  p.nb = 1u << (p.c - 1);
  p.nbp = p.nb; p.L = ilog2(p.nbp);
  const u32* order = order_of(curve);
  for (u32 W = (254 + p.c - 1) / p.c;; W++) {
    u32 K[8] = {0, 0, 0, 0, 0, 0, 0, 0};
    for (u32 w = 0; w + 1 < W; w++) {
      u32 bit = w * p.c + p.c - 1;
      if (bit < 256) K[bit >> 5] |= 1u << (bit & 31);
    }
    u32 s[9]; u64 cy = 0;
    for (int i = 0; i < 8; i++) { cy += (u64)order[i] + K[i]; s[i] = (u32)cy; cy >>= 32; }
    s[8] = (u32)cy;
    u32 sh = p.c * (W - 1);
    bool fits = true;
    if (s[8]) fits = false;
    u64 top = 0; bool big = false;
    for (int bit = 255; bit >= (int)sh; bit--) {
      u32 b = (s[bit >> 5] >> (bit & 31)) & 1u;
      if (top >> 62) big = true;
      top = (top << 1) | b;
    }
    if (big || top > p.nb) fits = false;
    if (sh >= 256) { fits = true; }
    if (fits) { p.W = W; memcpy(p.kadd, K, 32); break; }
  }
  if (p.c == 17 && p.W != 15) {
    lemsm_ctx tmp_opts; tmp_opts.opt_window_bits = 16;
    return make_msm_plan(&tmp_opts, curve, n);
  }
  return p;
}

template <class F> struct FieldTag {};

size_t align_up(size_t x, size_t a) { return (x + a - 1) / a * a; }

struct GroupWs {
  u32* err;
  char* arena;
  u32* bin_total; u32* bin_cursor; u32* bin_start; u32* tile_prefix; u32* meta;
  u32* bucket_count; u32* bucket_cursor; u32* bucket_start;
  u32* block_counts;
  uint16_t* dig16;
  unsigned long long* signbm;
  uint4* tile_info;
  u32* entries; u32* sorted;
  u32* rec_key; char* rec_pt;
  u32* mq_cnt; uint4* mq_items; char* mq_partial; MqLayout mq;
  size_t zero_begin, zero_bytes;
  size_t zero_bytes_counters;
  size_t total;
  std::vector<size_t> guards;
};

MqLayout make_mq_layout(const lemsm_ctx* ctx, u32 nthr1) {
  return make_mq_layout_t(nthr1, ctx && ctx->opt_merge_slice ? (u32)ctx->opt_merge_slice : 512u,
                          ctx && ctx->opt_merge_wave_th ? (u32)ctx->opt_merge_wave_th - 1u : 2048u);
}

const size_t WS_GUARD = 256;
GroupWs carve(char* base, const GroupPlan& pl, const ArenaLayout& ar, const MqLayout& mq, size_t ptb, bool guard = false) {
  GroupWs w; size_t off = 0;
  auto take = [&](size_t bytes) {
    size_t o = off;
    if (guard) { size_t g = align_up(off + bytes, 16); w.guards.push_back(g); off = align_up(g + WS_GUARD, 256); }
    else off = align_up(off + bytes, 256);
    return o;
  };
  u32 NBpad = pl.nbins << pl.LB;
  size_t z0 = off;
  size_t o_err = take(64);
  size_t o_mqcnt = take(MQ_WORDS * 4);
  size_t o_bin_total = take(MAX_BINS * 4), o_bin_cursor = take(MAX_BINS * 4);
  size_t o_bcount = take((size_t)NBpad * 4), o_bcursor = take((size_t)NBpad * 4);
  size_t o_arena = take((size_t)ar.total_points * ptb);
  size_t zend = o_arena + (size_t)(ar.apyr_off - ar.bucket_off) * ptb;
  w.zero_bytes_counters = o_arena - z0;
  size_t o_bin_start = take((MAX_BINS + 1) * 4), o_tile_prefix = take((MAX_BINS + 1) * 4), o_meta = take(64);
  size_t o_bstart = take(((size_t)NBpad + 1) * 4);
  size_t o_blockc = take((size_t)pl.nblk1 * pl.nbins * 8);
  size_t o_dig = take(pl.c ? (size_t)pl.dstride * (pl.w1 - pl.w0) * 2 + 64 : 16);
  size_t o_tinfo = take((size_t)pl.max_tiles * 16 + 16);
  size_t o_sbm = take(pl.c == 17 ? (size_t)(pl.w1 - pl.w0) * ((pl.n + 63) / 64) * 8 + 16 : 16);
  size_t Mmax = (size_t)pl.n * (pl.w1 - pl.w0);
  size_t o_entries = take(Mmax * 4 + 4 * (size_t)pl.L1 + 512), o_sorted = take(Mmax * 4 + 4 * (size_t)pl.L1 + 512);
  w.mq = mq;
  size_t o_rk = take((size_t)pl.nthr1 * 4 + 16), o_rp = take(2 * (size_t)pl.nthr1 * ptb + 256);
  size_t o_mqi = take(((size_t)mq.offF + mq.capF) * 16), o_mqp = take((size_t)mq.capP * ptb + 256);
  w.total = off;
  if (base) {
    w.err = (u32*)(base + o_err);
    w.bin_total = (u32*)(base + o_bin_total); w.bin_cursor = (u32*)(base + o_bin_cursor);
    w.bucket_count = (u32*)(base + o_bcount); w.bucket_cursor = (u32*)(base + o_bcursor);
    w.arena = base + o_arena;
    w.bin_start = (u32*)(base + o_bin_start); w.tile_prefix = (u32*)(base + o_tile_prefix); w.meta = (u32*)(base + o_meta);
    w.bucket_start = (u32*)(base + o_bstart); w.block_counts = (u32*)(base + o_blockc); w.dig16 = (uint16_t*)(base + o_dig); w.tile_info = (uint4*)(base + o_tinfo); w.signbm = (unsigned long long*)(base + o_sbm);
    w.entries = (u32*)(base + o_entries); w.sorted = (u32*)(base + o_sorted);
    w.rec_key = (u32*)(base + o_rk); w.rec_pt = base + o_rp;
    w.mq_cnt = (u32*)(base + o_mqcnt); w.mq_items = (uint4*)(base + o_mqi); w.mq_partial = base + o_mqp;
  }
  w.zero_begin = z0; w.zero_bytes = zend - z0;
  return w;
}

u32 choose_lb(const lemsm_ctx* ctx, u32 nb, u32 n, u32 d) {
  if (ctx && ctx->plan_slab_n) n = ctx->plan_slab_n;
  u32 LB = 0;
  while (((nb + (1u << LB) - 1) >> LB) > 256 && LB < MAX_LB) LB++;
  if (d == 0 && ctx && ctx->opt_binsort != 2 && LB > 0) {
    const u32 cap = ctx->opt_binsort > 2 ? std::min((u32)ctx->opt_binsort, (u32)BIN_CAP) : (u32)BIN_CAP;
    const u32 BW = (nb + (1u << LB) - 1) >> LB;
    if ((u64)n / BW > (u64)cap * 9 / 10 && 2 * BW <= BW_MAX && (u64)n / (2 * BW) <= (u64)cap * 9 / 10) LB--;
  }
  return LB;
}

GroupPlan make_group_plan(const lemsm_ctx* ctx, u32 n, u32 c, u32 nb, u32 W, u32 w0, u32 w1, u32 d) {
  GroupPlan g; memset(&g, 0, sizeof g);
  g.n = n; g.c = c; g.nb = nb; g.W = W; g.w0 = w0; g.w1 = w1; g.d = d; g.nstride = n;
  u32 LB = choose_lb(ctx, nb, n, d);
  g.LB = LB;
  g.BW = (nb + (1u << LB) - 1) >> LB;
  g.nbw = g.BW << LB;
  g.NB = (w1 - w0) * g.nbw;
  g.nbins = (w1 - w0) * g.BW;
  u32 spb = (n + 1023) / 1024;
  spb = std::max(256u, std::min((u32)STAGE, spb));
  spb = (spb + 255) / 256 * 256;
  if (n >= (1u << 16)) spb = STAGE;
  if (n >= (1u << 16) && d == 0 && ctx->opt_stage2x == 4) spb = 4 * STAGE;
  if (n >= (1u << 16) && d == 0 && ctx->opt_stage2x == 2) spb = 2 * STAGE;
  g.spb = spb;
  g.dstride = (n + 63u) / 64u * 64u;
  g.nblk1 = (n + spb - 1) / spb;
  if (g.nblk1 == 0) g.nblk1 = 1;
  size_t Mmax = (size_t)n * (w1 - w0);
  u32 T2 = ctx->opt_tile > 0 ? std::min((u32)ctx->opt_tile, (u32)STAGE2) : (u32)STAGE2;
  g.T2 = T2;
  g.max_tiles = (u32)(Mmax / T2) + g.nbins + 1;
  g.bin_cap = ctx->opt_binsort == 2 ? 0u : (ctx->opt_binsort > 2 ? std::min((u32)ctx->opt_binsort, (u32)BIN_CAP) : (u32)BIN_CAP);
  if (g.bin_cap == BIN_CAP && g.BW && (u64)n * 3 / 2 / g.BW <= BIN_CAP_SMALL) g.bin_cap = BIN_CAP_SMALL;
  u32 L1;
  if (ctx->opt_chunk > 0) L1 = (u32)ctx->opt_chunk;
  else {
    size_t target = (size_t)256 * 4 * 3 * 64 * 2;
    size_t l = (Mmax + target - 1) / target;
    L1 = (u32)std::max((size_t)8, std::min((size_t)256, l));
  }
  if (ctx->plan_ring && ctx->opt_chunk == 0 && L1 >= 128) L1 = (L1 + 15u) & ~15u;
  g.L1 = L1;
  g.nthr1 = (u32)((Mmax + L1 - 1) / L1);
  if (g.nthr1 == 0) g.nthr1 = 1;
  return g;
}

u32 max_group_windows(const lemsm_ctx* ctx, u32 nb, u32 n, u32 d) {
  u32 LB = choose_lb(ctx, nb, n, d);
  u32 BW = (nb + (1u << LB) - 1) >> LB;
  u32 cap = MAX_BINS / BW;
  return cap == 0 ? 1 : cap;
}

struct PipProvider {
  const uint4* scalars; KAdd kadd;
  typedef PipDec Dec;
  int prepare(lemsm_ctx*, hipStream_t st, const GroupPlan& pl, uint16_t* dig16, unsigned long long* signbm, u32* block_counts,
              u32* bin_total, u32* err, Dec& dec) const {
    dec.dig16 = dig16; dec.signbm = nullptr;
    if (pl.c == 17) {
      dec.signbm = signbm;
      if (pl.nblk1 < 2048)
        hipLaunchKernelGGL((k_pip_digits<2, 1024>), dim3(pl.nblk1), dim3(1024), 0, st, scalars, kadd, pl, dig16, signbm, block_counts, bin_total, err);
      else
        hipLaunchKernelGGL((k_pip_digits<2>), dim3(pl.nblk1), dim3(256), 0, st, scalars, kadd, pl, dig16, signbm, block_counts, bin_total, err);
    } else if (pl.c == 16 && pl.W == 16) {
      if (pl.nblk1 < 1024)
        hipLaunchKernelGGL((k_pip_digits<1, 1024>), dim3(pl.nblk1), dim3(1024), 0, st, scalars, kadd, pl, dig16, signbm, block_counts, bin_total, err);
      else
        hipLaunchKernelGGL((k_pip_digits<1>), dim3(pl.nblk1), dim3(256), 0, st, scalars, kadd, pl, dig16, signbm, block_counts, bin_total, err);
    } else {
      if (pl.nblk1 < 1024)
        hipLaunchKernelGGL((k_pip_digits<0, 1024>), dim3(pl.nblk1), dim3(1024), 0, st, scalars, kadd, pl, dig16, signbm, block_counts, bin_total, err);
      else
        hipLaunchKernelGGL((k_pip_digits<0>), dim3(pl.nblk1), dim3(256), 0, st, scalars, kadd, pl, dig16, signbm, block_counts, bin_total, err);
    }
    return LEMSM_OK;
  }
};
struct NegProvider {
  const uint8_t* digitsT;
  typedef NegDec Dec;
  int prepare(lemsm_ctx*, hipStream_t st, const GroupPlan& pl, uint16_t*, unsigned long long*, u32* block_counts, u32* bin_total, u32*, Dec& dec) const {
    dec.digitsT = digitsT;
    hipLaunchKernelGGL((k_count1<NegDec>), dim3(pl.w1 - pl.w0, pl.nblk1), dim3(256), 0, st, dec, pl, block_counts, bin_total);
    return LEMSM_OK;
  }
};

__global__ __launch_bounds__(256) void k_group_finish(const uint4* __restrict__ out_area, uint4* __restrict__ d_out, u32 n16,
                                                      const u32* __restrict__ err, const u32* __restrict__ clock, const u32* __restrict__ mq_cnt,
                                                      u32* __restrict__ slot) {
  const u32 i = blockIdx.x * 256 + threadIdx.x;
  if (i < n16) d_out[i] = out_area[i];
  if (blockIdx.x == 0 && threadIdx.x < 24) {
    const u32 k = threadIdx.x;
    slot[k] = k < 2 ? err[k] : (k < 4 ? 0u : (k < 12 ? clock[k - 4] : (k < 16 ? mq_cnt[k - 12] : mq_cnt[k - 8])));
  }
}

template <class G, class Prov>
int run_group(lemsm_ctx* ctx, const Prov& prov, const GroupPlan& pl, u32 nbp, u32 L, const void* d_points,
              bool abi ,
              char* ws_base, char* d_out , u32* d_slot , hipStream_t s_sort, hipStream_t s_acc,
              hipStream_t s_tail, hipEvent_t ev_sorted, hipEvent_t ev_acc0, hipEvent_t ev_acc1,
              hipEvent_t ev_points  = nullptr,
              u32 slab_k = 0, u32 nba = 1 , u32 scaled_mask = 0 ) {
  hipStream_t st = s_sort;
  u32 gw = pl.w1 - pl.w0;
  u32 NBpad = pl.nbins << pl.LB;
  ArenaLayout ar = make_arena(NBpad, nbp, gw, L, nba);
  const bool abi_pyr = nba > 1 ? false : abi;
  const bool last_slab = slab_k + 1 == nba;
  std::vector<u32> pkey = {NBpad, pl.nb, pl.nbw, nbp, L, gw, abi_pyr ? 1u : 0u, nba};
  auto pit = ctx->pyr_cache.find(pkey);
  if (pit == ctx->pyr_cache.end()) {
    PyrCacheEntry ent;
    ent.pp = make_pyr_plan(ar, pl.nb, pl.nbw, nbp, L, abi_pyr);
    std::vector<PyrTask> flat;
    for (auto& s : ent.pp.steps) flat.insert(flat.end(), s.begin(), s.end());
    size_t tb = align_up(flat.size() * sizeof(PyrTask), 256);
    int rcr = reserve(ctx, ent.buf, tb + sizeof(CopyTask) + 64); if (rcr) return rcr;
    HIPCHK(ctx, hipMemcpy(ent.buf.p, flat.data(), flat.size() * sizeof(PyrTask), hipMemcpyHostToDevice));
    HIPCHK(ctx, hipMemcpy((char*)ent.buf.p + tb, &ent.pp.copy, sizeof(CopyTask), hipMemcpyHostToDevice));
    pit = ctx->pyr_cache.emplace(pkey, std::move(ent)).first;
  }
  const PyrPlan& pp = pit->second.pp;
  size_t ntasks_total = 0;
  for (auto& s : pp.steps) ntasks_total += s.size();
  PyrTask* d_tasks = (PyrTask*)pit->second.buf.p;
  CopyTask* d_copy = (CopyTask*)((char*)pit->second.buf.p + align_up(ntasks_total * sizeof(PyrTask), 256));
  const size_t ptb = G::PT_BYTES;
  const MqLayout mq = make_mq_layout(ctx, pl.nthr1);
  GroupWs w = carve(ws_base, pl, ar, mq, ptb, ctx->opt_ws_canary != 0);
  if (pl.nbins > MAX_BINS || pl.BW > BW_MAX || pl.LB > MAX_LB || pl.spb > 4 * STAGE || (pl.c && pl.dstride < pl.n) || pl.T2 > STAGE2 || pl.bin_cap > BIN_CAP)
    return fail(ctx, LEMSM_ERR_HIP, "internal: window-group plan exceeds a kernel limit (bins " + std::to_string(pl.nbins) + ", bins per window " + std::to_string(pl.BW) + ")");

  const bool first2 = L >= 5 && ctx->opt_pyr_first2 == 1 && nba == 1;
  RoctxRange rg_group("lemsm: window group (digits + sort + accumulate + tail enqueued)");
  HIPCHK(ctx, hipMemsetAsync(ws_base + w.zero_begin, 0, (first2 || slab_k > 0) ? w.zero_bytes_counters : w.zero_bytes, st));
  for (size_t g : w.guards) HIPCHK(ctx, hipMemsetAsync(ws_base + g, 0xA5, WS_GUARD, st));

  typename Prov::Dec dec;
  { int rcp = prov.prepare(ctx, st, pl, w.dig16, w.signbm, w.block_counts, w.bin_total, w.err, dec); if (rcp) return rcp; }
  hipLaunchKernelGGL(k_binscan, dim3(1), dim3(1024), 0, st, pl, w.bin_total, w.bin_start, w.tile_prefix, w.meta);
  const u32 xw = (gw >= 8 && ctx->opt_xcd_windows != 1) ? 1u : 0u;
  dim3 g1 = xw ? dim3(8u * ((gw + 7) / 8) * pl.nblk1) : dim3(gw, pl.nblk1);
  if (pl.spb > 2 * STAGE)
    hipLaunchKernelGGL((k_scatter1<typename Prov::Dec, 4 * STAGE, 1024>), g1, dim3(1024), 0, st, dec, pl, w.block_counts, w.bin_start, w.entries, xw);
  else if (pl.spb > STAGE)
    hipLaunchKernelGGL((k_scatter1<typename Prov::Dec, 2 * STAGE>), g1, dim3(256), 0, st, dec, pl, w.block_counts, w.bin_start, w.entries, xw);
  else if (Prov::Dec::VEC && (pl.BW & 1u) == 0 && ctx->opt_scatter_lean == 1)
    hipLaunchKernelGGL((k_scatter1<typename Prov::Dec, STAGE, 256, true>), g1, dim3(256), 0, st, dec, pl, w.block_counts, w.bin_start, w.entries, xw);
  else
    hipLaunchKernelGGL((k_scatter1<typename Prov::Dec, STAGE>), g1, dim3(256), 0, st, dec, pl, w.block_counts, w.bin_start, w.entries, xw);
  const u32* d_sorted = w.entries;
  const u32* d_bstart = w.bin_start;
  if (pl.LB > 0) {
    if (pl.bin_cap && pl.bin_cap <= BIN_CAP_SMALL) hipLaunchKernelGGL((k_binsort<BIN_CAP_SMALL>), dim3(pl.nbins), dim3(1024), 0, st, pl, w.entries, w.bin_start, w.sorted, w.bucket_start);
    else if (pl.bin_cap) hipLaunchKernelGGL((k_binsort<BIN_CAP>), dim3(pl.nbins), dim3(1024), 0, st, pl, w.entries, w.bin_start, w.sorted, w.bucket_start);
    hipLaunchKernelGGL(k_tilemap, dim3((pl.max_tiles + 255) / 256), dim3(256), 0, st, pl, w.bin_start, w.tile_prefix, w.meta, w.tile_info);
    const u32 g2 = pl.bin_cap ? std::min(pl.max_tiles, 768u) : pl.max_tiles;
    hipLaunchKernelGGL(k_count2, dim3(g2), dim3(256), 0, st, pl, w.entries, w.tile_info, w.bucket_count);
    hipLaunchKernelGGL(k_bucketscan, dim3(((pl.nbins << pl.LB) + 255) / 256), dim3(256), 0, st, pl, w.bin_start, w.bucket_count, w.bucket_start);
    hipLaunchKernelGGL(k_scatter2, dim3(g2), dim3(256), 0, st, pl, w.entries, w.tile_info,
                       w.bucket_start, w.bucket_cursor, w.sorted);
    d_sorted = w.sorted; d_bstart = w.bucket_start;
  }

  HIPCHK(ctx, hipEventRecord(ev_sorted, s_sort));
  st = s_acc;
  HIPCHK(ctx, hipStreamWaitEvent(s_acc, ev_sorted, 0));
  if (ev_points) HIPCHK(ctx, hipStreamWaitEvent(s_acc, ev_points, 0));
  if (ctx->wait_accum) HIPCHK(ctx, hipStreamWaitEvent(s_acc, ctx->wait_accum, 0));
  HIPCHK(ctx, hipEventRecord(ev_acc0, s_acc));
  {
    dim3 grid((pl.nthr1 + 255) / 256), blk(256);
    char* bsum = w.arena + ((size_t)ar.bucket_off + (size_t)slab_k * NBpad) * ptb;
    int wps = G::CONVERTED_DOMAIN ? (ctx->opt_accum_waves ? (int)ctx->opt_accum_waves : 3) : 4;
    if constexpr (G::CONVERTED_DOMAIN) {
      if (wps == 2) hipLaunchKernelGGL((k_accum1<G, 2>), grid, blk, 0, st, pl, d_sorted, d_bstart, w.meta, (const uint4*)d_points, bsum, w.rec_key, w.rec_pt);
      else if (wps == 4) hipLaunchKernelGGL((k_accum1<G, 4>), grid, blk, 0, st, pl, d_sorted, d_bstart, w.meta, (const uint4*)d_points, bsum, w.rec_key, w.rec_pt);
      else if (abi && (pl.L1 & 15u) == 0 && pl.L1 >= 32 && ctx->opt_entry_ring != 1) hipLaunchKernelGGL((k_accum1<G, 3, true, true>), grid, blk, 0, st, pl, d_sorted, d_bstart, w.meta, (const uint4*)d_points, bsum, w.rec_key, w.rec_pt);
      else if (abi) hipLaunchKernelGGL((k_accum1<G, 3, true>), grid, blk, 0, st, pl, d_sorted, d_bstart, w.meta, (const uint4*)d_points, bsum, w.rec_key, w.rec_pt);
      else hipLaunchKernelGGL((k_accum1<G, 3>), grid, blk, 0, st, pl, d_sorted, d_bstart, w.meta, (const uint4*)d_points, bsum, w.rec_key, w.rec_pt);
    } else {
      hipLaunchKernelGGL((k_accum1<G, 4>), grid, blk, 0, st, pl, d_sorted, d_bstart, w.meta, (const uint4*)d_points, bsum, w.rec_key, w.rec_pt);
    }
  }
  HIPCHK(ctx, hipEventRecord(ev_acc1, s_acc));
  st = s_tail;
  HIPCHK(ctx, hipStreamWaitEvent(s_tail, ev_acc1, 0));

  {
    RoctxRange rg_tail("lemsm: edge-record merge");
    const u32 sc = abi ? 1u : 0u;
    char* bsum = w.arena + ((size_t)ar.bucket_off + (size_t)slab_k * NBpad) * ptb;
    hipLaunchKernelGGL((k_merge_pairs<G>), dim3((pl.nthr1 + 255) / 256), dim3(256), 0, st, pl, sc, mq, d_bstart, w.meta, w.rec_key, w.rec_pt, bsum, w.mq_cnt, w.mq_items);
    hipLaunchKernelGGL((k_merge_serial<G>), dim3(std::min(ctx->num_cus, std::max(1u, (mq.capS + mq.capM + 63) / 64))), dim3(256), 0, st, sc, mq, w.mq_cnt, w.mq_items, w.rec_pt, bsum);
    hipLaunchKernelGGL((k_merge_waves<G>), dim3(std::min(ctx->num_cus, std::max(1u, (mq.capM + mq.capL + 3) / 4))), dim3(256), 0, st, sc, mq, w.mq_cnt, w.mq_items, w.rec_pt, w.mq_partial, bsum, w.mq_cnt);
    hipLaunchKernelGGL((k_merge_final<G>), dim3(std::min(ctx->num_cus, std::max(1u, (mq.capF + 3) / 4))), dim3(256), 0, st, sc, mq, w.mq_cnt, w.mq_items, w.mq_partial, bsum, w.mq_cnt);
  }
  RoctxRange rg_pyr("lemsm: bucket-reduction pyramid");
  if (nba > 1 && last_slab)
    hipLaunchKernelGGL((k_sum_slabs<G>), dim3((NBpad + 255) / 256), dim3(256), 0, st, w.arena + (size_t)ar.bucket_off * ptb, NBpad, nba, scaled_mask);
  if (last_slab) {
    size_t toff = 0;
    u32 s_begin = 1;
    if (first2) {
      PyrFirst2Args fa; memset(&fa, 0, sizeof fa);
      fa.nwin = gw; fa.nb = pl.nb; fa.nbw = pl.nbw; fa.nbp = nbp; fa.bucket_off = ar.bucket_off; fa.wstride = nbp;
      fa.a2_off = ar.apyr_off + nbp / 2;
      fa.r02_off = ar.rbuf_off + nbp / 4;
      fa.r11_off = ar.rbuf_off + nbp / 2;
      fa.scaled = abi_pyr ? 1u : 0u;
      const u32 threads = gw * (nbp / 8);
      hipLaunchKernelGGL((k_pyramid_first2<G>), dim3((threads + 255) / 256), dim3(256), 0, st, fa, d_bstart, w.arena, w.mq_cnt);
      toff = pp.steps[0].size() + pp.steps[1].size();
      s_begin = 3;
    }
    u32 first_fused = L + 1;
    if (ctx->opt_pyr_fuse != 1) {
      const size_t lim = ctx->opt_pyr_fuse == 2 ? 2048 : 256;
      for (u32 s = s_begin; s <= L; s++) {
        bool fits = true;
        for (u32 q = s; q <= L; q++) if ((size_t)pp.steps[q - 1].size() * pp.step_max_count[q - 1] > lim) fits = false;
        if (fits && L - s + 1 <= 20) { first_fused = s; break; }
      }
      if (first_fused == L) first_fused = L + 1;
    }
    for (u32 s = s_begin; s <= L && s < first_fused; s++) {
      auto& tasks = pp.steps[s - 1];
      u32 maxc = pp.step_max_count[s - 1];
      size_t threads = (size_t)tasks.size() * maxc * gw;
      const u32 quad = (G::CONVERTED_DOMAIN && ctx->opt_pyr_quad != 2 && threads <= 32768 && !(s == 1 && abi_pyr)) ? 1u : 0u;
      if (quad) threads *= 4;
      hipLaunchKernelGGL((k_pyramid<G>), dim3((u32)((threads + 255) / 256)), dim3(256), 0, st, d_tasks + toff, (u32)tasks.size(), gw, maxc, w.arena, quad);
      toff += tasks.size();
    }
    const bool need_copy = !(L == 1 && abi_pyr);
    if (first_fused <= L) {
      PyrTailArgs ta; memset(&ta, 0, sizeof ta);
      ta.first = first_fused; ta.last = L;
      u32 o = (u32)toff;
      for (u32 s = first_fused; s <= L; s++) { ta.step_off[s - first_fused] = o; ta.max_count[s - first_fused] = pp.step_max_count[s - 1]; o += (u32)pp.steps[s - 1].size(); }
      ta.step_off[L - first_fused + 1] = o;
      hipLaunchKernelGGL((k_pyramid_tail<G>), dim3(gw), dim3(1024), 0, st, (const PyrTask*)d_tasks, ta, (const CopyTaskPod*)d_copy, need_copy ? 1u : 0u, w.arena,
                         (G::CONVERTED_DOMAIN && ctx->opt_pyr_quad != 2) ? 1u : 0u);
    } else if (need_copy) {
      u32 cthreads = gw * (u32)(ptb / 16);
      hipLaunchKernelGGL(k_copy_points, dim3((cthreads + 63) / 64), dim3(64), 0, st, d_copy, 1u, gw, (u32)ptb, w.arena);
    }
  }
  {
    const u32 n16 = last_slab ? (u32)((size_t)gw * (L + 1) * ptb / 16) : 0u;
    hipLaunchKernelGGL(k_group_finish, dim3(std::max(1u, (n16 + 255) / 256)), dim3(256), 0, st, (const uint4*)(w.arena + (size_t)ar.out_off * ptb), (uint4*)d_out, n16,
                       w.err, w.meta + META_CLOCK, w.mq_cnt, d_slot);
  }
  HIPCHK(ctx, hipGetLastError());
  if (!w.guards.empty()) {
    std::vector<unsigned char> host(w.guards.size() * WS_GUARD);
    for (size_t i = 0; i < w.guards.size(); i++) HIPCHK(ctx, hipMemcpyAsync(host.data() + i * WS_GUARD, ws_base + w.guards[i], WS_GUARD, hipMemcpyDeviceToHost, st));
    HIPCHK(ctx, hipStreamSynchronize(s_sort)); HIPCHK(ctx, hipStreamSynchronize(s_acc)); HIPCHK(ctx, hipStreamSynchronize(st));
    for (size_t i = 0; i < host.size(); i++)
      if (host[i] != 0xA5) return fail(ctx, LEMSM_ERR_HIP, "workspace guard " + std::to_string(i / WS_GUARD) + " overwritten at byte " + std::to_string(i % WS_GUARD) + " (option ws_canary)");
  }
  return LEMSM_OK;
}

size_t group_ws_bytes(const lemsm_ctx* ctx, const GroupPlan& pl, u32 nbp, u32 L, size_t ptb, bool guard, u32 nba = 1) {
  u32 gw = pl.w1 - pl.w0;
  ArenaLayout ar = make_arena(pl.nbins << pl.LB, nbp, gw, L, nba);
  GroupWs w = carve(nullptr, pl, ar, make_mq_layout(ctx, pl.nthr1), ptb, guard);
  return w.total + 4096;
}


struct WinRun {
  size_t nslabs = 0, ng = 0, out_slab = 0, SLAB = 0, err_slot = 0;
  size_t nrec = 0;
  size_t err_stride = 1;
  size_t err_cap = 0;
  char* d_out = nullptr; char* d_err = nullptr;
  u32 nw = 0, nw_pad = 0, L = 0; size_t ptb = 0;
  size_t send_bytes() const { return out_slab * nrec; }
  static constexpr size_t STATUS_BYTES = 256;
  size_t send_total() const { return out_slab * nrec + err_cap + STATUS_BYTES; }
};

bool shared_tail(const lemsm_ctx* ctx, size_t nslabs) { return nslabs > 1 && nslabs <= 8 && ctx->opt_slab_tail != 2 && ctx->opt_groups <= 1; }

template <class G>
void win_sizes(const lemsm_ctx* ctx, size_t n, u32 nw_pad, u32 L, WinRun& wr) {
  const u32 slab_log = ctx->opt_slab_bits ? (u32)ctx->opt_slab_bits : MAX_SLAB_LOG;
  wr.SLAB = (size_t)1 << slab_log;
  wr.nslabs = n ? (n + wr.SLAB - 1) / wr.SLAB : 1;
  wr.nrec = shared_tail(ctx, wr.nslabs) ? 1 : wr.nslabs;
  wr.ptb = G::PT_BYTES; wr.L = L; wr.nw_pad = nw_pad; wr.nw = 0; wr.ng = 0;
  wr.out_slab = align_up((size_t)std::max(nw_pad, 1u) * (L + 1) * wr.ptb, 256);
  wr.err_slot = 96; wr.err_stride = std::max<size_t>(nw_pad, 1);
  wr.err_cap = align_up(wr.nslabs * wr.err_stride * wr.err_slot, 256);
  wr.d_out = nullptr; wr.d_err = nullptr;
}

void comm_abort(lemsm_ctx* ctx) {
  if (!ctx->comm) return;
  Rccl& rc = Rccl::get();
  if (rc.CommAbort) (void)rc.CommAbort(ctx->comm); else (void)rc.CommDestroy(ctx->comm);
  ctx->comm = nullptr; ctx->comm_size = 1; ctx->comm_rank = 0;
  ctx->last_error += " [communicator aborted: this rank could not enter the exchange]";
}

template <class P64, class G, class MakeSrc>
int run_windows_enqueue(lemsm_ctx* ctx, MakeSrc make_src, size_t n, u32 c, u32 nb, u32 nbp, u32 L, u32 W, u32 wb, u32 we, u32 d,
                        const void* d_points, u32 nw_pad, WinRun& wr) {
  u32 nw = we - wb;
  if (nw_pad < nw) nw_pad = nw;
  ctx->plan_ring = false;
  const HostStage* hs = ctx->host_stage;
  u32 slab_log = ctx->opt_slab_bits ? (u32)ctx->opt_slab_bits : MAX_SLAB_LOG;
  if (hs) slab_log = host_slab_log(ctx, n);
  const size_t SLAB = (size_t)1 << slab_log;
  const size_t nslabs = n ? (n + SLAB - 1) / SLAB : 1;
  const bool shared = shared_tail(ctx, nslabs);
  const u32 nba = shared ? (u32)nslabs : 1u;
  const size_t nrec = shared ? 1 : nslabs;
  ctx->plan_slab_n = (u32)std::min(SLAB, n);
  u32 gmax = max_group_windows(ctx, nb, ctx->plan_slab_n, d);
  const size_t ptb = G::PT_BYTES;
  u32 ngroups = 1;
  if (ctx->opt_groups > 0) ngroups = std::min((u32)ctx->opt_groups, std::max(nw, 1u));
  u32 gsz = std::max(1u, std::min(gmax, (nw + ngroups - 1) / ngroups));
  struct Grp { u32 g0, g1; size_t off; };
  std::vector<Grp> groups;
  size_t ws_total = 0;
  if (n) {
    u32 sn0 = (u32)std::min(SLAB, n), snl = (u32)(n - (nslabs - 1) * SLAB);
    for (u32 g0 = wb; g0 < we; g0 += gsz) {
      u32 g1 = std::min(we, g0 + gsz);
      size_t bytes = group_ws_bytes(ctx, make_group_plan(ctx, sn0, c, nb, W, g0, g1, d), nbp, L, ptb, ctx->opt_ws_canary != 0, nba);
      if (snl != sn0) bytes = std::max(bytes, group_ws_bytes(ctx, make_group_plan(ctx, snl, c, nb, W, g0, g1, d), nbp, L, ptb, ctx->opt_ws_canary != 0, nba));
      groups.push_back({g0, g1, ws_total});
      ws_total += align_up(bytes + 8192, 256);
    }
  }
  const size_t ng = groups.size();
  const size_t out_slab = align_up((size_t)std::max(nw_pad, 1u) * (L + 1) * ptb, 256);
  const size_t ERR_SLOT = 96;
  const size_t err_stride = std::max<size_t>(nw_pad, 1);
  const size_t err_bytes = align_up(nslabs * err_stride * ERR_SLOT, 256);
  size_t conv_bytes = G::CONVERTED_DOMAIN ? align_up(std::min(SLAB, n) * 64, 256) : 0;
  wr.nslabs = nslabs; wr.nrec = nrec; wr.ng = ng; wr.out_slab = out_slab; wr.SLAB = SLAB; wr.err_slot = ERR_SLOT; wr.err_stride = err_stride; wr.err_cap = err_bytes;
  wr.nw = nw; wr.nw_pad = nw_pad; wr.L = L; wr.ptb = ptb;
  int rc = reserve(ctx, ctx->ws, ws_total + conv_bytes + out_slab * nrec + err_bytes + WinRun::STATUS_BYTES + 4096);
  if (rc) return rc;
  char* ws_base = (char*)ctx->ws.p;
  char* d_conv = ws_base + ws_total;
  char* d_out = d_conv + conv_bytes;
  char* d_err = d_out + out_slab * nrec;
  wr.d_out = d_out; wr.d_err = d_err;
  while (ctx->evpool.size() < 3 * ng * nslabs + (hs ? nslabs : 0)) {
    hipEvent_t e; HIPCHK(ctx, hipEventCreate(&e)); ctx->evpool.push_back(e);
  }
  hipEvent_t* ev_up = ctx->evpool.data() + 3 * ng * nslabs;
  hipStream_t s_sort = ctx->stream_sort, s_acc = ctx->stream, s_tail = ctx->stream_tail;
  const bool one_queue = ctx->opt_groups <= 1;
  if (one_queue) { s_sort = s_acc; s_tail = s_acc; }
  hipStream_t s_up = ctx->stream_sort;
  if (hs && !one_queue) return fail(ctx, LEMSM_ERR_BAD_ARG, "option groups > 1 is only available on the device-pointer entries");
  if (!one_queue) HIPCHK(ctx, hipStreamSynchronize(s_acc));
  HIPCHK(ctx, hipEventRecord(ctx->ev[0], s_acc));
  ctx->t_accum_ms = 0; ctx->n_accum = 0;
  if (nw_pad != nw || n == 0 || nw == 0)
    HIPCHK(ctx, hipMemsetAsync(d_out, 0, out_slab * nrec, s_acc));
  HIPCHK(ctx, hipMemsetAsync(d_err, 0, err_bytes + WinRun::STATUS_BYTES, s_acc));
  u32 scaled_mask = 0;
  for (size_t k = 0; k < nslabs && n && nw; k++) {
    const size_t s0 = k * SLAB;
    u32 sn = (u32)std::min(SLAB, n - s0);
    if (hs) {
      HIPCHK(ctx, hipMemcpyAsync(hs->d_scalars + s0 * 32, hs->h_scalars + s0 * 32, (size_t)sn * 32, hipMemcpyHostToDevice, s_up));
      if (hs->h_points)
        HIPCHK(ctx, hipMemcpyAsync(hs->d_points + s0 * 64, (const char*)hs->h_points + s0 * 64, (size_t)sn * 64, hipMemcpyHostToDevice, s_up));
      HIPCHK(ctx, hipEventRecord(ev_up[k], s_up));
      HIPCHK(ctx, hipStreamWaitEvent(s_acc, ev_up[k], 0));
    }
    const char* pts = (const char*)d_points + s0 * 64;
    bool abi = false;
    hipEvent_t ev_points = nullptr;
    ctx->plan_ring = false;
    if constexpr (G::CONVERTED_DOMAIN) {
      GroupPlan pl0 = make_group_plan(ctx, sn, c, nb, W, groups[0].g0, groups[0].g1, d);
      double S = std::max(1.0, std::min((double)pl0.L1, (double)sn / (double)nb));
      double P = 1.0 - std::pow(1.0 - 1.0 / S, 64.0);
      abi = P * (double)(groups[0].g1 - groups[0].g0) < 7.0 && (ctx->opt_accum_waves == 0 || ctx->opt_accum_waves == 3);
      if (ctx->opt_abi_points == 1) abi = false;
      if (ctx->opt_abi_points == 2) abi = (ctx->opt_accum_waves == 0 || ctx->opt_accum_waves == 3);
      ctx->plan_ring = abi && ctx->opt_entry_ring != 1;
      if (!abi) {
        if (one_queue && !hs) {
          HIPCHK(ctx, hipEventRecord(ctx->ev[2], s_acc));
          HIPCHK(ctx, hipStreamWaitEvent(ctx->stream_sort, ctx->ev[2], 0));
          hipLaunchKernelGGL((k_convert_points<typename G::F_>), dim3((2 * sn + 255) / 256), dim3(256), 0, ctx->stream_sort, (const uint4*)pts, (uint4*)d_conv, sn);
          HIPCHK(ctx, hipEventRecord(ctx->ev[3], ctx->stream_sort));
          ev_points = ctx->ev[3];
        } else {
          hipLaunchKernelGGL((k_convert_points<typename G::F_>), dim3((2 * sn + 255) / 256), dim3(256), 0, s_acc, (const uint4*)pts, (uint4*)d_conv, sn);
        }
        pts = d_conv;
      }
    }
    for (size_t gi = 0; gi < ng; gi++) {
      const Grp& gr = groups[gi];
      GroupPlan pl = make_group_plan(ctx, sn, c, nb, W, gr.g0, gr.g1, d);
      pl.nstride = (u32)n;
      auto src = make_src(s0, sn);
      hipEvent_t* ev = ctx->evpool.data() + 3 * (k * ng + gi);
      if (gi == 0 && abi) scaled_mask |= 1u << k;
      rc = run_group<G>(ctx, src, pl, nbp, L, pts, abi, ws_base + gr.off, d_out + (shared ? 0 : k) * out_slab + (size_t)(gr.g0 - wb) * (L + 1) * ptb,
                        (u32*)(d_err + (k * err_stride + gi) * ERR_SLOT), s_sort, s_acc, s_tail, ev[0], ev[1], ev[2], gi == 0 ? ev_points : nullptr,
                        shared ? (u32)k : 0u, nba, scaled_mask);
      if (rc) return rc;
    }
    if (!one_queue) {
      HIPCHK(ctx, hipStreamSynchronize(s_sort));
      HIPCHK(ctx, hipStreamSynchronize(s_acc));
      HIPCHK(ctx, hipStreamSynchronize(s_tail));
    }
  }
  if (n == 0 || nw == 0) { wr.ng = 0; }
  return LEMSM_OK;
}

hipStream_t records_stream(const lemsm_ctx* ctx) { return ctx->opt_groups <= 1 ? ctx->stream : ctx->stream_tail; }

int collect_local_stats(lemsm_ctx* ctx, const WinRun& wr, const u32* slots) {
  u64 clk_cyc = 0, clk_ticks = 0;
  const size_t sw = wr.err_slot / 4;
  for (int q = 0; q < 4; q++) ctx->dbg_merge[q] = 0;
  for (size_t k = 0; k < wr.nslabs; k++)
    for (size_t gi = 0; gi < wr.ng; gi++) {
      const u32* ew = slots + (k * wr.err_stride + gi) * sw;
      const size_t i = k * wr.ng + gi;
      for (int q = 0; q < 4; q++) ctx->dbg_merge[q] += ew[12 + q];
      for (int q = 0; q < 8; q++) ctx->dbg_stamps[q] = ew[16 + q];
      float a = 0; HIPCHK(ctx, hipEventElapsedTime(&a, ctx->evpool[3 * i + 1], ctx->evpool[3 * i + 2]));
      ctx->t_accum_ms += a; ctx->n_accum++;
      u64 ck[4]; memcpy(ck, ew + 4, 32);
      if (ck[2] > ck[0] && ck[3] > ck[1] && ck[2] - ck[0] < ((u64)1 << 40)) { clk_cyc += ck[2] - ck[0]; clk_ticks += ck[3] - ck[1]; }
    }
  ctx->accum_clock_mhz = clk_ticks ? (double)clk_cyc / (double)clk_ticks * 100.0 : 0.0;
  return LEMSM_OK;
}

size_t first_bad_scalar(const WinRun& wr, const u32* slots) {
  size_t best = SIZE_MAX;
  const size_t sw = wr.err_slot / 4;
  for (size_t k = 0; k < wr.nslabs; k++)
    for (size_t gi = 0; gi < wr.err_stride; gi++) {
      const u32* ew = slots + (k * wr.err_stride + gi) * sw;
      if (ew[0]) best = std::min(best, k * wr.SLAB + (size_t)(~ew[1]));
    }
  return best;
}

int run_windows_finish(lemsm_ctx* ctx, const WinRun& wr, const char* d_raw, size_t raw_bytes, std::vector<char>& raw) {
  RoctxRange rg_fin("lemsm: read-back and wait");
  hipStream_t s_tail = records_stream(ctx);
  raw.resize(raw_bytes);
  const size_t err_bytes = wr.ng ? wr.err_cap : 0;
  { int rcp = reserve_pinned(ctx, raw_bytes + err_bytes + 64); if (rcp) return rcp; }
  char* hp = (char*)ctx->h_pin;
  if (d_raw == wr.d_out && raw_bytes == wr.send_bytes() && raw_bytes + err_bytes) {
    HIPCHK(ctx, hipMemcpyAsync(hp, d_raw, raw_bytes + err_bytes, hipMemcpyDeviceToHost, s_tail));
  } else {
    if (raw_bytes) HIPCHK(ctx, hipMemcpyAsync(hp, d_raw, raw_bytes, hipMemcpyDeviceToHost, s_tail));
    if (err_bytes) HIPCHK(ctx, hipMemcpyAsync(hp + raw_bytes, wr.d_err, err_bytes, hipMemcpyDeviceToHost, s_tail));
  }
  HIPCHK(ctx, hipEventRecord(ctx->ev[1], s_tail));
  const auto th0 = std::chrono::steady_clock::now();
  HIPCHK(ctx, hipEventSynchronize(ctx->ev[1]));
  ctx->host_us[0] = std::chrono::duration<double, std::micro>(std::chrono::steady_clock::now() - th0).count();
  if (raw_bytes) memcpy(raw.data(), hp, raw_bytes);
  float ms = 0; HIPCHK(ctx, hipEventElapsedTime(&ms, ctx->ev[0], ctx->ev[1]));
  ctx->t_total_ms = ms;
  if (!err_bytes) return LEMSM_OK;
  std::vector<u32> slots(err_bytes / 4);
  memcpy(slots.data(), hp + raw_bytes, err_bytes);
  const size_t bad = first_bad_scalar(wr, slots.data());
  if (bad != SIZE_MAX) {
    ctx->bad_index = bad;
    return fail(ctx, LEMSM_ERR_SCALAR_OUT_OF_RANGE, "scalar is not a canonical field element (>= order)");
  }
  return collect_local_stats(ctx, wr, slots.data());
}


template <class P64, class G>
void from_device_records(const char* raw, size_t n, host::pt* out) { from_device_records_t<P64, G::CONVERTED_DOMAIN, G::PT_BYTES>(raw, n, out); }

template <class P64, class G>
void sum_slab_records(lemsm_ctx* ctx, const char* raw, size_t out_slab, size_t nslabs, u32 nw, u32 L, std::vector<host::pt>& host_out,
                      bool fold = false ) {
  typedef host::HG<P64> HGp;
  const size_t ptb = G::PT_BYTES;
  RoctxRange rg_host("lemsm: host fold of the window records");
  host_out.assign(fold ? (size_t)nw : (size_t)nw * (L + 1), HGp::identity());
  host_parallel(ctx, (int)nw, [&](int w) {
    std::vector<host::pt> tmp(L + 1), acc(L + 1);
    host::pt* dst = fold ? acc.data() : host_out.data() + (size_t)w * (L + 1);
    for (size_t k = 0; k < nslabs; k++) {
      from_device_records<P64, G>(raw + k * out_slab + (size_t)w * (L + 1) * ptb, L + 1, tmp.data());
      if (k == 0) memcpy(dst, tmp.data(), (L + 1) * sizeof(host::pt));
      else for (u32 i = 0; i <= L; i++) dst[i] = HGp::add(dst[i], tmp[i]);
    }
    if (fold) host_out[w] = window_sum<P64>(dst, L);
  });
}

template <class P64, class G, class MakeSrc>
int run_windows(lemsm_ctx* ctx, MakeSrc make_src, size_t n, u32 c, u32 nb, u32 nbp, u32 L, u32 W, u32 wb, u32 we, u32 d,
                const void* d_points, std::vector<host::pt>& host_out, bool fold = false ) {
  typedef host::HG<P64> HGp;
  u32 nw = we - wb;
  host_out.assign(fold ? (size_t)nw : (size_t)nw * (L + 1), HGp::identity());
  if (n == 0 || nw == 0) return LEMSM_OK;
  WinRun wr;
  int rc = run_windows_enqueue<P64, G>(ctx, make_src, n, c, nb, nbp, L, W, wb, we, d, d_points, nw, wr);
  if (rc) return rc;
  std::vector<char> raw;
  rc = run_windows_finish(ctx, wr, wr.d_out, wr.send_bytes(), raw);
  if (rc) return rc;
  const auto th0 = std::chrono::steady_clock::now();
  sum_slab_records<P64, G>(ctx, raw.data(), wr.out_slab, wr.nrec, nw, L, host_out, fold);
  ctx->host_us[1] = std::chrono::duration<double, std::micro>(std::chrono::steady_clock::now() - th0).count();
  return LEMSM_OK;
}

template <class P64>
void window_sums_par(lemsm_ctx* ctx, const host::pt* recs , u32 nw, u32 L, std::vector<host::pt>& out) {
  out.resize(nw);
  host_parallel(ctx, (int)nw, [&](int w) { out[w] = window_sum<P64>(recs + (size_t)w * (L + 1), L); });
}

template <class P64>
void msm_combine_t(const MsmPlan& mp, const host::pt* sums , u64 out[12]) { msm_combine_windows<P64>(mp.c, mp.W, sums, out); }

template <class P64, class G>
int msm_partial_t(lemsm_ctx* ctx, int curve, const void* d_scalars, const void* d_points, size_t n, u32 wb, u32 we,
                  std::vector<host::pt>& out) {
  MsmPlan mp = make_msm_plan(ctx, curve, n);
  if (wb > we || we > mp.W) return fail(ctx, LEMSM_ERR_BAD_ARG, "window range out of bounds");
  auto make_src = [&](size_t s0, u32) {
    PipProvider s; s.scalars = (const uint4*)((const char*)d_scalars + s0 * 32);
    memcpy(s.kadd.k, mp.kadd, 32); memcpy(s.kadd.order, order_of(curve), 32); return s;
  };
  int rc = run_windows<P64, G>(ctx, make_src, n, mp.c, mp.nb, mp.nbp, mp.L, mp.W, wb, we, 0, d_points, out, true);
  return rc;
}

template <class P64, class G>
int msm_batch_t(lemsm_ctx* ctx, int curve, const void* const* d_scalars, const void* d_points, size_t n, size_t K, u64* outs,
                const uint8_t* const* h_scalars = nullptr ) {
  lemsm_ctx* lane[2] = {ctx, ctx->peer};
  MsmPlan mp = make_msm_plan(ctx, curve, n);
  WinRun wr[2];
  auto enqueue = [&](size_t k) -> int {
    lemsm_ctx* c = lane[k & 1];
    const void* sc = h_scalars ? nullptr : d_scalars[k];
    if (h_scalars) {
      int rcr = reserve(c, c->in_s, n * 32); if (rcr) return rcr;
      if (!c->ev_batch_up) HIPCHK(c, hipEventCreateWithFlags(&c->ev_batch_up, hipEventDisableTiming));
      HIPCHK(c, hipMemcpyAsync(c->in_s.p, h_scalars[k], n * 32, hipMemcpyHostToDevice, c->stream_sort));
      HIPCHK(c, hipEventRecord(c->ev_batch_up, c->stream_sort));
      HIPCHK(c, hipStreamWaitEvent(c->stream, c->ev_batch_up, 0));
      sc = c->in_s.p;
    }
    auto make_src = [&](size_t s0, u32) {
      PipProvider s; s.scalars = (const uint4*)((const char*)sc + s0 * 32);
      memcpy(s.kadd.k, mp.kadd, 32); memcpy(s.kadd.order, order_of(curve), 32); return s;
    };
    c->wait_accum = nullptr;
    if (k > 0) {
      lemsm_ctx* o = lane[(k - 1) & 1]; const WinRun& w = wr[(k - 1) & 1];
      if (h_scalars) c->wait_accum = o->ev_call_done;
      else if (w.ng && w.nslabs && o->evpool.size() >= 3 * w.ng * w.nslabs) c->wait_accum = o->evpool[3 * (w.ng * w.nslabs - 1) + 2];
    }
    int rce = run_windows_enqueue<P64, G>(c, make_src, n, mp.c, mp.nb, mp.nbp, mp.L, mp.W, 0, mp.W, 0, d_points, mp.W, wr[k & 1]);
    c->wait_accum = nullptr;
    if (!rce && h_scalars) {
      if (!c->ev_call_done) HIPCHK(c, hipEventCreateWithFlags(&c->ev_call_done, hipEventDisableTiming));
      HIPCHK(c, hipEventRecord(c->ev_call_done, records_stream(c)));
    }
    return rce;
  };
  auto finish = [&](size_t k) -> int {
    lemsm_ctx* c = lane[k & 1];
    std::vector<char> raw;
    int rc = run_windows_finish(c, wr[k & 1], wr[k & 1].d_out, wr[k & 1].send_bytes(), raw);
    if (rc) { ctx->last_error = c->last_error; ctx->bad_index = c->bad_index; return rc; }
    std::vector<host::pt> sums;
    sum_slab_records<P64, G>(ctx, raw.data(), wr[k & 1].out_slab, wr[k & 1].nrec, mp.W, mp.L, sums, true);
    msm_combine_t<P64>(mp, sums.data(), outs + 12 * k);
    return LEMSM_OK;
  };
  int rc = LEMSM_OK; size_t enq = 0;
  const bool stamps = getenv("LEMSM_DEBUG_STAMPS") != nullptr;
  auto now_us = [] { return std::chrono::duration<double, std::micro>(std::chrono::steady_clock::now().time_since_epoch()).count(); };
  const double tb = now_us();
  for (size_t k = 0; k < K && !rc; k++) {
    const double t0 = now_us();
    rc = enqueue(k);
    const double t1 = now_us();
    if (rc) { if (lane[k & 1] != ctx) ctx->last_error = lane[k & 1]->last_error; break; }
    enq = k + 1;
    if (k > 0) rc = finish(k - 1);
    if (stamps) fprintf(stderr, "[lemsm batch] call %zu: enqueue (upload + launches) %.0f us at %.0f, finish of the call before %.0f us\n", k, t1 - t0, t0 - tb, now_us() - t1);
  }
  if (!rc && enq == K && K) rc = finish(K - 1);
  if (rc) for (lemsm_ctx* c : lane) { (void)hipSetDevice(c->device); (void)hipStreamSynchronize(c->stream); }
  return rc;
}

int check_curve(lemsm_ctx* ctx, int curve) {
  if (curve != LEMSM_BN254_G1 && curve != LEMSM_GRUMPKIN) return fail(ctx, LEMSM_ERR_BAD_CURVE, "unknown curve id");
  return LEMSM_OK;
}

int stage(lemsm_ctx* ctx, DevBuf& b, const void* host, size_t bytes) {
  int rc = reserve(ctx, b, bytes ? bytes : 16);
  if (rc) return rc;
  if (bytes) HIPCHK(ctx, hipMemcpyAsync(b.p, host, bytes, hipMemcpyHostToDevice, ctx->stream));
  return LEMSM_OK;
}

struct LhsPlan { u32 base, d, nb, nbp, L; };
int make_lhs_plan(int curve, u32 base, LhsPlan& lp) {
  if (base < 3) return LEMSM_ERR_BAD_BASE;
  lp.base = base; lp.d = logb_ceil8(bound_of(curve), base) + 1;
  lp.nb = base - 1; lp.nbp = next_pow2(lp.nb); if (lp.nbp < 2) lp.nbp = 2;
  lp.L = ilog2(lp.nbp);
  return LEMSM_OK;
}

struct LhsDigits { uint8_t* digitsT; u32* err; };
struct Words12 { u32 w[12]; };
__global__ void k_set_words12(u32* __restrict__ dst, Words12 v) { if (threadIdx.x < 12) dst[threadIdx.x] = v.w[threadIdx.x]; }

int lhs_err_words(lemsm_ctx* ctx, size_t n, u32 err[2]) {
  err[0] = 0xffffffffu; err[1] = 0;
  if (!n) return LEMSM_OK;
  HIPCHK(ctx, hipEventSynchronize(ctx->ev[4]));
  err[0] = ctx->h_small[0]; err[1] = ctx->h_small[1];
  return LEMSM_OK;
}

int lhs_digits(lemsm_ctx* ctx, int curve, const void* d_scalars, size_t n, const LhsPlan& lp, DevBuf& buf, LhsDigits& out, u32 row_begin, u32 row_end) {
  size_t bytes = align_up((size_t)lp.d * n, 256) + 256 + 64;
  int rc = reserve(ctx, buf, bytes);
  if (rc) return rc;
  char* base = (char*)buf.p;
  out.digitsT = (uint8_t*)base;
  u32* bound_d = (u32*)(base + align_up((size_t)lp.d * n, 256));
  out.err = bound_d + 8;
  Words12 init;
  memcpy(init.w, bound_of(curve), 32); init.w[8] = 0xffffffffu; init.w[9] = 0; init.w[10] = 0xffffffffu; init.w[11] = 0;
  hipLaunchKernelGGL(k_set_words12, dim3(1), dim3(64), 0, ctx->stream, bound_d, init);
  if (n) {
    hipLaunchKernelGGL(k_negbase_digits, dim3((u32)((n + 255) / 256)), dim3(256), 0, ctx->stream, (const uint4*)d_scalars, (u32)n,
                       lp.base, lp.d, bound_d, 1, (uint8_t*)nullptr, out.digitsT, out.err, row_begin, row_end);
    if (!ctx->h_small) HIPCHK(ctx, hipHostMalloc((void**)&ctx->h_small, 256, hipHostMallocDefault));
    HIPCHK(ctx, hipMemcpyAsync(ctx->h_small, out.err, 8, hipMemcpyDeviceToHost, ctx->stream));
    HIPCHK(ctx, hipEventRecord(ctx->ev[4], ctx->stream));
  }
  HIPCHK(ctx, hipGetLastError());
  return LEMSM_OK;
}

template <class P64, class G>
int lhs_partial_t(lemsm_ctx* ctx, int curve, const void* d_scalars, const void* d_points, size_t n, const LhsPlan& lp,
                  u32 pb, u32 pe, std::vector<host::pt>& out, size_t* bad_index) {
  if (pb > pe || pe > lp.d) return fail(ctx, LEMSM_ERR_BAD_ARG, "position range out of bounds");
  if (n >= ((size_t)1 << 32)) return fail(ctx, LEMSM_ERR_BAD_ARG, "n too large");
  LhsDigits dg;
  int rc = lhs_digits(ctx, curve, d_scalars, n, lp, ctx->in_aux, dg, pb, pe);
  if (rc) return rc;
  auto make_src = [&](size_t s0, u32) { NegProvider s; s.digitsT = dg.digitsT + s0; return s; };
  rc = run_windows<P64, G>(ctx, make_src, n, 0, lp.nb, lp.nbp, lp.L, lp.d, pb, pe, lp.d, d_points, out, true);
  if (rc) return rc;
  u32 err[2];
  { int rce = lhs_err_words(ctx, n, err); if (rce) return rce; }
  ctx->truncated = err[1];
  if (err[0] != 0xffffffffu) {
    if (bad_index) *bad_index = err[0];
    return fail(ctx, LEMSM_ERR_SCALAR_OUT_OF_RANGE, "scalar out of range (>= isqrt(order)+2)");
  }
  return LEMSM_OK;
}

template <class P64>
void lhs_combine_t(const LhsPlan& lp, const host::pt* sums, u64 out_carry[12], u64* out_carries) { lhs_combine_positions<P64>(lp.base, lp.d, sums, out_carry, out_carries); }

int msm_partial_dispatch(lemsm_ctx* ctx, int curve, const void* d_scalars, const void* d_points, size_t n, u32 wb, u32 we,
                         std::vector<host::pt>& out) {
  if (ctx->opt_field == 1) {
    if (curve == LEMSM_BN254_G1) return msm_partial_t<host::FqParams64, GqStrict>(ctx, curve, d_scalars, d_points, n, wb, we, out);
    return msm_partial_t<host::FrParams64, GrStrict>(ctx, curve, d_scalars, d_points, n, wb, we, out);
  }
  if (curve == LEMSM_BN254_G1) return msm_partial_t<host::FqParams64, GqLazy>(ctx, curve, d_scalars, d_points, n, wb, we, out);
  return msm_partial_t<host::FrParams64, GrLazy>(ctx, curve, d_scalars, d_points, n, wb, we, out);
}
int lhs_partial_dispatch(lemsm_ctx* ctx, int curve, const void* d_scalars, const void* d_points, size_t n, const LhsPlan& lp,
                         u32 pb, u32 pe, std::vector<host::pt>& out, size_t* bad_index) {
  if (ctx->opt_field == 1) {
    if (curve == LEMSM_BN254_G1) return lhs_partial_t<host::FqParams64, GqStrict>(ctx, curve, d_scalars, d_points, n, lp, pb, pe, out, bad_index);
    return lhs_partial_t<host::FrParams64, GrStrict>(ctx, curve, d_scalars, d_points, n, lp, pb, pe, out, bad_index);
  }
  if (curve == LEMSM_BN254_G1) return lhs_partial_t<host::FqParams64, GqLazy>(ctx, curve, d_scalars, d_points, n, lp, pb, pe, out, bad_index);
  return lhs_partial_t<host::FrParams64, GrLazy>(ctx, curve, d_scalars, d_points, n, lp, pb, pe, out, bad_index);
}

struct Exchange { int world, rank; bool sim; };
int validate_points(lemsm_ctx* ctx, int curve, const void* d_points, size_t n);

#define RCCLCHK(ctx, expr)                                                                     \
  do {                                                                                         \
    ncclResult_t r_ = (expr);                                                                  \
    if (r_ != ncclSuccess) {                                                                   \
      (ctx)->last_error = std::string(#expr) + ": " + Rccl::get().GetErrorString(r_);          \
      return LEMSM_ERR_RCCL;                                                                   \
    }                                                                                          \
  } while (0)


template <class P64, class G, class MakeSrc>
int sharded_records(lemsm_ctx* ctx, MakeSrc make_src, size_t n, u32 c, u32 nb, u32 nbp, u32 L, u32 W, u32 d, const void* d_points,
                    const Exchange& ex, std::vector<host::pt>& all, int rc_pre = LEMSM_OK ) {
  u32 max_nw = 0;
  for (int r = 0; r < ex.world; r++) { u32 a, b; shard_range(W, ex.world, r, a, b); max_nw = std::max(max_nw, b - a); }
  WinRun wr; std::vector<char> raw;
  size_t sb = 0;
  if (!ex.sim) {
    u32 a, b; shard_range(W, ex.world, ex.rank, a, b);
    int rc_local = rc_pre;
    if (!rc_local) rc_local = run_windows_enqueue<P64, G>(ctx, make_src, n, c, nb, nbp, L, W, a, b, d, d_points, max_nw, wr);
    else win_sizes<G>(ctx, n, max_nw, L, wr);
    sb = wr.send_total();
    hipStream_t st = records_stream(ctx);
    const char* send = wr.d_out;
    if (rc_local) {
      if (reserve(ctx, ctx->fail_buf, sb) != LEMSM_OK) { comm_abort(ctx); return rc_local; }
      HIPCHK(ctx, hipMemsetAsync(ctx->fail_buf.p, 0, sb, st));
      HIPCHK(ctx, hipMemsetD32Async((hipDeviceptr_t)((char*)ctx->fail_buf.p + sb - WinRun::STATUS_BYTES), rc_local, 1, st));
      send = (const char*)ctx->fail_buf.p;
    }
    if (reserve(ctx, ctx->gather, sb * ex.world) != LEMSM_OK) { comm_abort(ctx); return rc_local ? rc_local : LEMSM_ERR_NOMEM; }
    {
      ncclResult_t r_ = Rccl::get().AllGather(send, ctx->gather.p, sb, ncclUint8, ctx->comm, st);
      if (r_ != ncclSuccess) { ctx->last_error = std::string("ncclAllGather: ") + Rccl::get().GetErrorString(r_); comm_abort(ctx); return LEMSM_ERR_RCCL; }
    }
    { int rcp = reserve_pinned(ctx, sb * ex.world + 64); if (rcp) return rcp; }
    HIPCHK(ctx, hipMemcpyAsync(ctx->h_pin, ctx->gather.p, sb * ex.world, hipMemcpyDeviceToHost, st));
    HIPCHK(ctx, hipEventRecord(ctx->ev[1], st));
    HIPCHK(ctx, hipEventSynchronize(ctx->ev[1]));
    const char* hp = (const char*)ctx->h_pin;
    std::vector<u32> status(ex.world);
    for (int r = 0; r < ex.world; r++) memcpy(&status[r], hp + (size_t)r * sb + sb - WinRun::STATUS_BYTES, 4);
    int failed_rank = -1;
    const int agreed = merge_rank_status(status.data(), ex.world, ex.rank, rc_local, &failed_rank);
    if (agreed != LEMSM_OK) {
      if (agreed != rc_local || !rc_local) ctx->last_error = "rank " + std::to_string(failed_rank) + " failed before the exchange with status " + std::to_string(status[failed_rank]) + " (" + lemsm_strerror((int)status[failed_rank]) + ")";
      return agreed;
    }
    float ms = 0; HIPCHK(ctx, hipEventElapsedTime(&ms, ctx->ev[0], ctx->ev[1]));
    ctx->t_total_ms = ms;
    size_t bad = SIZE_MAX;
    for (int r = 0; r < ex.world; r++) bad = std::min(bad, first_bad_scalar(wr, (const u32*)(hp + (size_t)r * sb + wr.send_bytes())));
    if (bad != SIZE_MAX) {
      ctx->bad_index = bad;
      return fail(ctx, LEMSM_ERR_SCALAR_OUT_OF_RANGE, "scalar is not a canonical field element (>= order)");
    }
    { int rcs = collect_local_stats(ctx, wr, (const u32*)(hp + (size_t)ex.rank * sb + wr.send_bytes())); if (rcs) return rcs; }
// ... 1320 lines not shown
```

### halo2_liam_eagen_msm_amd/csrc/xyzz.cuh

```cuda
#pragma once
#include "field32.cuh"

namespace lemsm {

template <class F>
struct XYZZ {
  typedef F F_;
  typedef typename F::fe fe;
  static constexpr bool CONVERTED_DOMAIN = false;
  static __device__ __forceinline__ bool aff_is_identity(const fe& x, const fe& y) { return F::is_zero(x) && F::is_zero(y); }
  struct pt { fe x, y, zz, zzz; };
  struct aff { fe x, y; };

  static __device__ __forceinline__ void set_identity(pt& p) {
    F::set_zero(p.x); F::set_zero(p.y); F::set_zero(p.zz); F::set_zero(p.zzz);
  }
  static __device__ __forceinline__ bool is_identity(const pt& p) { return F::is_zero(p.zz); }
  static __device__ __forceinline__ bool aff_is_identity(const aff& a) {
    return F::is_zero(a.x) && F::is_zero(a.y);
  }
  static __device__ __forceinline__ void from_affine(pt& r, const aff& a) {
    if (aff_is_identity(a)) { set_identity(r); return; }
    r.x = a.x; r.y = a.y; F::set_one(r.zz); F::set_one(r.zzz);
  }

  static __device__ __noinline__ void dbl_affine(pt& r, const fe& x, const fe& y) {
    fe U, V, W, S, M, t;
    F::dbl(U, y);
    F::sqr(V, U);
    F::mul(W, U, V);
    F::mul(S, x, V);
    F::sqr(t, x); F::dbl(M, t); F::add(M, M, t);
    F::sqr(r.x, M); F::sub(r.x, r.x, S); F::sub(r.x, r.x, S);
    F::sub(t, S, r.x); F::mul(t, M, t); F::mul(U, W, y); F::sub(r.y, t, U);
    r.zz = V; r.zzz = W;
  }
  static __device__ __noinline__ void dbl(pt& r, const pt& p) {
    fe U, V, W, S, M, t, x3;
    F::dbl(U, p.y);
    F::sqr(V, U);
    F::mul(W, U, V);
    F::mul(S, p.x, V);
    F::sqr(t, p.x); F::dbl(M, t); F::add(M, M, t);
    F::sqr(x3, M); F::sub(x3, x3, S); F::sub(x3, x3, S);
    F::sub(t, S, x3); F::mul(t, M, t); F::mul(U, W, p.y);
    F::sub(r.y, t, U);
    r.x = x3;
    F::mul(r.zz, V, p.zz);
    F::mul(r.zzz, W, p.zzz);
  }

  static __device__ __forceinline__ void madd_abi(pt& acc, const fe& x2, const fe& y2, bool& empty) { madd(acc, x2, y2, empty); }
  static __device__ __forceinline__ void madd(pt& acc, const fe& x2, const fe& y2, bool& empty) { madd(acc, x2, y2); empty = is_identity(acc); }
  static __device__ __forceinline__ void unscale(pt&) {}
  static __device__ __forceinline__ void scale(pt&) {}

  static __device__ __forceinline__ void madd(pt& acc, const fe& x2, const fe& y2) {
    if (is_identity(acc)) {
      acc.x = x2; acc.y = y2; F::set_one(acc.zz); F::set_one(acc.zzz);
      return;
    }
    fe U2, S2, P, R;
    F::mul(U2, x2, acc.zz);
    F::mul(S2, y2, acc.zzz);
    F::sub(P, U2, acc.x);
    F::sub(R, S2, acc.y);
    if (F::is_zero(P)) {
      if (F::is_zero(R)) { pt res; fe xx = x2, yy = y2; dbl_affine(res, xx, yy); acc = res; }
      else set_identity(acc);
      return;
    }
    fe PP, PPP, Q, t;
    F::sqr(PP, P);
    F::mul(PPP, P, PP);
    F::mul(Q, acc.x, PP);
    F::sqr(t, R); F::sub(t, t, PPP); F::sub(t, t, Q); F::sub(t, t, Q);
    F::mul(U2, acc.y, PPP);
    acc.x = t;
    F::sub(t, Q, t); F::mul(t, R, t); F::sub(acc.y, t, U2);
    F::mul(acc.zz, acc.zz, PP);
    F::mul(acc.zzz, acc.zzz, PPP);
  }

  static __device__ __forceinline__ void add(pt& acc, const pt& q) {
    if (is_identity(q)) return;
    if (is_identity(acc)) { acc = q; return; }
    fe U1, U2, S1, S2, P, R;
    F::mul(U1, acc.x, q.zz);
    F::mul(U2, q.x, acc.zz);
    F::mul(S1, acc.y, q.zzz);
    F::mul(S2, q.y, acc.zzz);
    F::sub(P, U2, U1);
    F::sub(R, S2, S1);
    if (F::is_zero(P)) {
      if (F::is_zero(R)) { pt t = acc, res; dbl(res, t); acc = res; }
      else set_identity(acc);
      return;
    }
    fe PP, PPP, Q, t;
    F::sqr(PP, P);
    F::mul(PPP, P, PP);
    F::mul(Q, U1, PP);
    F::sqr(t, R); F::sub(t, t, PPP); F::sub(t, t, Q); F::sub(t, t, Q);
    acc.x = t;
    F::sub(t, Q, t); F::mul(t, R, t); F::mul(S1, S1, PPP); F::sub(acc.y, t, S1);
    F::mul(t, acc.zz, q.zz); F::mul(acc.zz, t, PP);
    F::mul(t, acc.zzz, q.zzz); F::mul(acc.zzz, t, PPP);
  }

  static __device__ __forceinline__ void neg(pt& p) { F::neg(p.y, p.y); }

  template <int CTRL, int ROW_MASK>
  static __device__ __forceinline__ void dpp_move(pt& r, const pt& p) {
#pragma unroll
    for (int i = 0; i < 8; i++) {
      r.x.v[i] = (u32)__builtin_amdgcn_update_dpp(0, (int)p.x.v[i], CTRL, ROW_MASK, 0xf, false);
      r.y.v[i] = (u32)__builtin_amdgcn_update_dpp(0, (int)p.y.v[i], CTRL, ROW_MASK, 0xf, false);
      r.zz.v[i] = (u32)__builtin_amdgcn_update_dpp(0, (int)p.zz.v[i], CTRL, ROW_MASK, 0xf, false);
      r.zzz.v[i] = (u32)__builtin_amdgcn_update_dpp(0, (int)p.zzz.v[i], CTRL, ROW_MASK, 0xf, false);
    }
  }
  static __device__ __forceinline__ void scan_fetch(pt& r, const pt& p, int step) {
    switch (step) {
      case 0: dpp_move<0x111, 0xf>(r, p); break;
      case 1: dpp_move<0x112, 0xf>(r, p); break;
      case 2: dpp_move<0x114, 0xf>(r, p); break;
      case 3: dpp_move<0x118, 0xf>(r, p); break;
      case 4: dpp_move<0x142, 0xa>(r, p); break;
      default: dpp_move<0x143, 0xc>(r, p); break;
    }
  }

  static constexpr u32 PT_BYTES = 128;
  static __device__ __forceinline__ void load(pt& p, const void* mem) {
    const char* m = reinterpret_cast<const char*>(mem);
    F::load(p.x, m); F::load(p.y, m + 32); F::load(p.zz, m + 64); F::load(p.zzz, m + 96);
  }
  static constexpr int RAW_WORDS = 8;
  static __device__ __forceinline__ void load_raw(uint4 (&r)[RAW_WORDS], const void* mem) {
    const uint4* q = reinterpret_cast<const uint4*>(mem);
#pragma unroll
    for (int i = 0; i < RAW_WORDS; i++) r[i] = q[i];
  }
  static __device__ __forceinline__ void from_raw(pt& p, const uint4 (&r)[RAW_WORDS]) {
    F::from_words(p.x, r[0], r[1]); F::from_words(p.y, r[2], r[3]); F::from_words(p.zz, r[4], r[5]); F::from_words(p.zzz, r[6], r[7]);
  }
  static __device__ __forceinline__ void store(void* mem, const pt& p) {
    char* m = reinterpret_cast<char*>(mem);
    F::store(m, p.x); F::store(m + 32, p.y); F::store(m + 64, p.zz); F::store(m + 96, p.zzz);
  }
};

}
```

### halo2_liam_eagen_msm_amd/csrc/xyzz29.cuh

```cuda
#pragma once
#include "field29.cuh"

namespace lemsm {

template <class F>
struct XYZZ29 {
  typedef F F_;
  typedef typename F::fe fe;
  static constexpr bool CONVERTED_DOMAIN = true;
  static __device__ __forceinline__ bool aff_is_identity(const fe&, const fe& y) { return F::limbs_zero(y); }
  struct pt { fe x, y, zz, zzz; };

  static __device__ __forceinline__ void set_identity(pt& p) {
    F::set_zero(p.x); F::set_zero(p.y); F::set_zero(p.zz); F::set_zero(p.zzz);
  }
  static __device__ __forceinline__ bool is_identity(const pt& p) { return F::limbs_zero(p.zz); }

  static __device__ __forceinline__ void hi_term(fe& t, const fe& ppp, const fe& q) {
#pragma unroll
    for (int i = 0; i < 9; i++) {
      i32 n2 = (i32)((((u32)F::P_::N[i] << 1) & (u32)F::MASK) | (i ? ((u32)F::P_::N[i - 1] >> 28) : 0u));
      t.l[i] = n2 - ppp.l[i] - 2 * q.l[i];
    }
  }

  static __device__ __forceinline__ bool pp_is_zero(const fe& pp) {
    if (pp.l[0] != 0 && pp.l[0] != F::P_::N[0]) return false;
    i32 z = 0, e = 0;
#pragma unroll
    for (int i = 0; i < 9; i++) { z |= pp.l[i]; e |= pp.l[i] ^ F::P_::N[i]; }
    return z == 0 || e == 0;
  }

  template <bool AFFINE>
  static __device__ __noinline__ void dbl_impl(pt& r, const pt& p) {
    fe U, V, W, S, M, t, nW, x3;
    F::add(U, p.y, p.y); F::wnorm(U);
    F::sqr(V, U);
    F::mul(W, U, V);
    F::mul(S, p.x, V);
    F::sqr(t, p.x); F::add(M, t, t); F::add(M, M, t); F::wnorm(M);
    fe zero; F::set_zero(zero);
    hi_term(t, zero, S);
    F::sqr_addhi(x3, M, t);
    F::sub(t, S, x3); F::neg(nW, W);
    fe y = p.y; F::wnorm(y);
    F::mul2(r.y, M, t, nW, y);
    r.x = x3;
    if (AFFINE) { r.zz = V; r.zzz = W; }
    else { F::mul(r.zz, V, p.zz); F::mul(r.zzz, W, p.zzz); }
  }

  static __device__ __forceinline__ void madd(pt& acc, const fe& x2, const fe& y2, bool& empty) {
    if (empty) {
      acc.x = x2; acc.y = y2; F::wnorm(acc.y); F::set_one(acc.zz); F::set_one(acc.zzz);
      empty = false;
      return;
    }
    madd_nonempty(acc, x2, y2, empty);
  }
  static __device__ __forceinline__ void madd(pt& acc, const fe& x2, const fe& y2) {
    bool empty = is_identity(acc);
    madd(acc, x2, y2, empty);
  }
  static __device__ __forceinline__ void madd_nonempty(pt& acc, const fe& x2, const fe& y2, bool& empty) {
    fe U2, S2, P, R, PP;
    F::mul(U2, x2, acc.zz);
    F::mul(S2, y2, acc.zzz);
    F::sub(P, U2, acc.x);
    F::sub(R, S2, acc.y);
    F::sqr(PP, P);
    if (pp_is_zero(PP)) {
      if (F::is_zero_mod(R)) {
        pt a, res; a.x = x2; a.y = y2; F::set_one(a.zz); F::set_one(a.zzz);
        dbl_impl<true>(res, a);
        acc = res;
      } else { set_identity(acc); empty = true; }
      return;
    }
    fe PPP, Q, t, nY;
    F::mul(PPP, P, PP);
    F::mul(Q, acc.x, PP);
    hi_term(t, PPP, Q);
    F::neg(nY, acc.y);
    F::sqr_addhi(acc.x, R, t);
    F::sub(t, Q, acc.x);
    F::mul2(acc.y, R, t, nY, PPP);
    F::mul(acc.zz, acc.zz, PP);
    F::mul(acc.zzz, acc.zzz, PPP);
  }

  static __device__ __forceinline__ void madd_abi(pt& acc, const fe& x2a, const fe& y2a, bool& empty) {
    if (empty) {
      F::mul32(acc.x, x2a); F::mul32(acc.y, y2a); F::set_c266(acc.zz); F::set_c266(acc.zzz);
      empty = false;
      return;
    }
    fe U2, S2, P, R, PP;
    F::mul(U2, x2a, acc.zz);
    F::mul(S2, y2a, acc.zzz);
    F::sub(P, U2, acc.x);
    F::sub(R, S2, acc.y);
    F::sqr(PP, P);
    if (pp_is_zero(PP)) {
      if (F::is_zero_mod(R)) {
        pt a, res; F::from_abi(a.x, x2a); F::from_abi(a.y, y2a); F::set_one(a.zz); F::set_one(a.zzz);
        dbl_impl<true>(res, a);
        F::from_abi(res.zz, res.zz); F::from_abi(res.zzz, res.zzz);
        acc = res;
      } else { set_identity(acc); empty = true; }
      return;
    }
    fe PPP, Q, t, nY;
    F::mul(PPP, P, PP);
    F::mul(Q, acc.x, PP);
    hi_term(t, PPP, Q);
    F::neg(nY, acc.y);
    F::sqr_addhi(acc.x, R, t);
    F::sub(t, Q, acc.x);
    F::mul2(acc.y, R, t, nY, PPP);
    F::mul(acc.zz, acc.zz, PP);
    F::mul(acc.zzz, acc.zzz, PPP);
  }
  static __device__ __forceinline__ void unscale(pt& p) {
    if (is_identity(p)) return;
    F::div32(p.zz, p.zz); F::div32(p.zzz, p.zzz);
  }
  static __device__ __forceinline__ void scale(pt& p) {
    if (is_identity(p)) return;
    F::from_abi(p.zz, p.zz); F::from_abi(p.zzz, p.zzz);
  }

  static __device__ __forceinline__ void add(pt& acc, const pt& q) {
    if (is_identity(q)) return;
    if (is_identity(acc)) { acc = q; return; }
    fe U1, U2, S1, S2, P, R, PP;
    F::mul(U1, acc.x, q.zz);
    F::mul(U2, q.x, acc.zz);
    F::mul(S1, acc.y, q.zzz);
    F::mul(S2, q.y, acc.zzz);
    F::sub(P, U2, U1);
    F::sub(R, S2, S1);
    F::sqr(PP, P);
    if (pp_is_zero(PP)) {
      if (F::is_zero_mod(R)) { pt t = acc, res; dbl_impl<false>(res, t); acc = res; }
      else set_identity(acc);
      return;
    }
    fe PPP, Q, t, nS;
    F::mul(PPP, P, PP);
    F::mul(Q, U1, PP);
    hi_term(t, PPP, Q);
    F::neg(nS, S1);
    F::sqr_addhi(acc.x, R, t);
    F::sub(t, Q, acc.x);
    F::mul2(acc.y, R, t, nS, PPP);
    F::mul(t, acc.zz, q.zz); F::mul(acc.zz, t, PP);
    F::mul(t, acc.zzz, q.zzz); F::mul(acc.zzz, t, PPP);
  }

  template <int CTRL>
  static __device__ __forceinline__ void quad_move(fe& r, const fe& a) {
#pragma unroll
    for (int i = 0; i < 9; i++) r.l[i] = (i32)__builtin_amdgcn_update_dpp(0, (int)a.l[i], CTRL, 0xf, 0xf, false);
  }
  static __device__ __forceinline__ void ld_elem(fe& r, const char* p, u32 k) {
    const i32* e = reinterpret_cast<const i32*>(p + 36u * k);
#pragma unroll
    for (int i = 0; i < 9; i++) r.l[i] = e[i];
  }
  static __device__ __forceinline__ void st_elem(char* p, u32 k, const fe& a) {
    i32* e = reinterpret_cast<i32*>(p + 36u * k);
#pragma unroll
    for (int i = 0; i < 9; i++) e[i] = a.l[i];
  }
  static __device__ __forceinline__ void sel(fe& r, bool c, const fe& a, const fe& b) {
#pragma unroll
    for (int i = 0; i < 9; i++) r.l[i] = c ? a.l[i] : b.l[i];
  }
  static __device__ __forceinline__ bool add4_mem(const char* pa, const char* pb, char* dst, u32 q) {
    const bool odd = (q & 1u) != 0, hi = q >= 2u;
    fe A, B, C, E, r1, x1, D;
    ld_elem(A, odd ? pb : pa, hi ? 1u : 0u);
    ld_elem(B, odd ? pa : pb, hi ? 3u : 2u);
    ld_elem(C, pa, hi ? 3u : 2u);
    ld_elem(E, pb, hi ? 3u : 2u);
    int sp = (F::limbs_zero(C) || F::limbs_zero(E)) ? 1 : 0;
    F::mul(r1, A, B);
    quad_move<0xB1>(x1, r1);
    F::sub(D, x1, r1); F::cneg(D, D, odd);
    fe A2, B2, r2;
    sel(A2, odd, C, D); sel(B2, odd, E, D);
    F::mul(r2, A2, B2);
    const int pz = pp_is_zero(r2) ? 1 : 0;
    sp |= __builtin_amdgcn_update_dpp(0, pz, 0x00, 0xf, 0xf, false);
    sp |= __builtin_amdgcn_update_dpp(0, sp, 0xB1, 0xf, 0xf, false);
    sp |= __builtin_amdgcn_update_dpp(0, sp, 0x4E, 0xf, 0xf, false);
    if (sp) return false;
    fe bPP, bU1, A3, r3;
    quad_move<0x00>(bPP, r2); quad_move<0x00>(bU1, r1);
    sel(A3, q == 0u, D, r2); sel(A3, q == 2u, bU1, A3);
    F::mul(r3, A3, bPP);
    fe bPPP, T, X3, V, bS1, A4, B4, r4, bY, Y3;
    quad_move<0x00>(bPPP, r3);
#pragma unroll
    for (int i = 0; i < 9; i++) T.l[i] = r2.l[i] - bPPP.l[i] - 2 * r3.l[i];
    F::wnorm(T); F::reduce_small(X3, T);
    F::sub(V, r3, X3);
    quad_move<0xAA>(bS1, r1);
    sel(A4, q == 0u, bS1, r2); sel(A4, q == 2u, D, A4);
    sel(B4, q == 2u, V, bPPP);
    F::mul(r4, A4, B4);
    quad_move<0x00>(bY, r4);
    F::sub(Y3, r4, bY); F::wnorm(Y3);
    if (q == 1u) st_elem(dst, 2u, r3);
    if (q == 3u) st_elem(dst, 3u, r4);
    if (q == 2u) { st_elem(dst, 0u, X3); st_elem(dst, 1u, Y3); }
    return true;
  }

  template <int CTRL, int ROW_MASK>
  static __device__ __forceinline__ void dpp_move(pt& r, const pt& p) {
#pragma unroll
    for (int i = 0; i < 9; i++) {
      r.x.l[i] = (i32)__builtin_amdgcn_update_dpp(0, (int)p.x.l[i], CTRL, ROW_MASK, 0xf, false);
      r.y.l[i] = (i32)__builtin_amdgcn_update_dpp(0, (int)p.y.l[i], CTRL, ROW_MASK, 0xf, false);
      r.zz.l[i] = (i32)__builtin_amdgcn_update_dpp(0, (int)p.zz.l[i], CTRL, ROW_MASK, 0xf, false);
      r.zzz.l[i] = (i32)__builtin_amdgcn_update_dpp(0, (int)p.zzz.l[i], CTRL, ROW_MASK, 0xf, false);
    }
  }
  static __device__ __forceinline__ void scan_fetch(pt& r, const pt& p, int step) {
    switch (step) {
      case 0: dpp_move<0x111, 0xf>(r, p); break;
      case 1: dpp_move<0x112, 0xf>(r, p); break;
      case 2: dpp_move<0x114, 0xf>(r, p); break;
      case 3: dpp_move<0x118, 0xf>(r, p); break;
      case 4: dpp_move<0x142, 0xa>(r, p); break;
      default: dpp_move<0x143, 0xc>(r, p); break;
    }
  }

  static constexpr u32 PT_BYTES = 160;
  static __device__ __forceinline__ void load(pt& p, const void* mem) {
    const uint4* q = reinterpret_cast<const uint4*>(mem);
    u32 w[40];
#pragma unroll
    for (int i = 0; i < 10; i++) { uint4 v = q[i]; w[4 * i] = v.x; w[4 * i + 1] = v.y; w[4 * i + 2] = v.z; w[4 * i + 3] = v.w; }
#pragma unroll
    for (int i = 0; i < 9; i++) { p.x.l[i] = (i32)w[i]; p.y.l[i] = (i32)w[9 + i]; p.zz.l[i] = (i32)w[18 + i]; p.zzz.l[i] = (i32)w[27 + i]; }
  }
  static constexpr int RAW_WORDS = 9;
  static __device__ __forceinline__ void load_raw(uint4 (&r)[RAW_WORDS], const void* mem) {
    const uint4* q = reinterpret_cast<const uint4*>(mem);
#pragma unroll
    for (int i = 0; i < RAW_WORDS; i++) r[i] = q[i];
  }
  static __device__ __forceinline__ void from_raw(pt& p, const uint4 (&r)[RAW_WORDS]) {
    u32 w[36];
#pragma unroll
    for (int i = 0; i < 9; i++) { w[4 * i] = r[i].x; w[4 * i + 1] = r[i].y; w[4 * i + 2] = r[i].z; w[4 * i + 3] = r[i].w; }
#pragma unroll
    for (int i = 0; i < 9; i++) { p.x.l[i] = (i32)w[i]; p.y.l[i] = (i32)w[9 + i]; p.zz.l[i] = (i32)w[18 + i]; p.zzz.l[i] = (i32)w[27 + i]; }
  }
  static __device__ __forceinline__ void store(void* mem, const pt& p) {
    uint4* q = reinterpret_cast<uint4*>(mem);
    u32 w[40];
#pragma unroll
    for (int i = 0; i < 9; i++) { w[i] = (u32)p.x.l[i]; w[9 + i] = (u32)p.y.l[i]; w[18 + i] = (u32)p.zz.l[i]; w[27 + i] = (u32)p.zzz.l[i]; }
    w[36] = w[37] = w[38] = w[39] = 0;
#pragma unroll
    for (int i = 0; i < 10; i++) q[i] = make_uint4(w[4 * i], w[4 * i + 1], w[4 * i + 2], w[4 * i + 3]);
  }
};

}
```

Before: 874.7 million.

## Drop stored block counts, fuse merge kernels, skip redundant workspace clears

Digit and count kernels now write only the per-block offsets. Scatter kernels recompute the per-block bin counts in LDS, which halves the counter traffic. The serial and wave merge kernels are fused into one launch that splits blocks by index, saving a launch and letting both run concurrently. Workspace zeroing is tracked across calls so regions already cleared at the end of the previous call are not memset again. The accumulate path also skips setting the accumulator to identity at segment starts and adds a register-settling asm barrier in the doubling fallback.

```diff
diff --git a/halo2_liam_eagen_msm_amd/csrc/fixed_base.inc b/halo2_liam_eagen_msm_amd/csrc/fixed_base.inc
--- a/halo2_liam_eagen_msm_amd/csrc/fixed_base.inc
+++ b/halo2_liam_eagen_msm_amd/csrc/fixed_base.inc
@@ -94,7 +94,7 @@
 
 __global__ __launch_bounds__(256) void k_fixed_digits(const uint4* __restrict__ scalars, FixedDigitArgs fa, GroupPlan pl,
                                                       uint16_t* __restrict__ dig16, unsigned long long* __restrict__ signbm,
-                                                      u32* __restrict__ block_counts, u32* __restrict__ bin_total, u32* __restrict__ err) {
+                                                      u32* __restrict__ block_offs, u32* __restrict__ bin_total, u32* __restrict__ err) {
   __shared__ u32 hist[MAX_BINS];
   const u32 tid = threadIdx.x, r = blockIdx.x;
   for (u32 i = tid; i < pl.nbins; i += 256) hist[i] = 0;
@@ -146,18 +146,17 @@
     const u32 cnt = hist[i];
     const u32 wl = i / pl.BW, bin = i - wl * pl.BW;
     const size_t slot = ((size_t)wl * pl.nblk1 + r) * pl.BW + bin;
-    block_counts[slot] = cnt;
-    block_counts[(size_t)pl.nblk1 * pl.nbins + slot] = cnt ? atomicAdd(&bin_total[i], cnt) : 0u;
+    block_offs[slot] = cnt ? atomicAdd(&bin_total[i], cnt) : 0u;
   }
 }
 
 struct FixedProvider {
   const uint4* scalars; FixedDigitArgs fa;
   typedef PipDec Dec;
-  int prepare(lemsm_ctx*, hipStream_t st, const GroupPlan& pl, uint16_t* dig16, unsigned long long* signbm, u32* block_counts,
+  int prepare(lemsm_ctx*, hipStream_t st, const GroupPlan& pl, uint16_t* dig16, unsigned long long* signbm, u32* block_offs,
               u32* bin_total, u32* err, Dec& dec) const {
     dec.dig16 = dig16; dec.signbm = pl.c == 17 ? signbm : nullptr;
-    hipLaunchKernelGGL(k_fixed_digits, dim3(pl.nblk1), dim3(256), 0, st, scalars, fa, pl, dig16, signbm, block_counts, bin_total, err);
+    hipLaunchKernelGGL(k_fixed_digits, dim3(pl.nblk1), dim3(256), 0, st, scalars, fa, pl, dig16, signbm, block_offs, bin_total, err);
     return LEMSM_OK;
   }
 };
diff --git a/halo2_liam_eagen_msm_amd/csrc/inst_fq_lazy.hip b/halo2_liam_eagen_msm_amd/csrc/inst_fq_lazy.hip
--- a/halo2_liam_eagen_msm_amd/csrc/inst_fq_lazy.hip
+++ b/halo2_liam_eagen_msm_amd/csrc/inst_fq_lazy.hip
@@ -7,8 +7,7 @@
 template __global__ void lemsm::k_accum1<G, 3, true, true>(GroupPlan, const u32*, const u32*, u32*, const uint4*, char*, u32*, char*);
 template __global__ void lemsm::k_accum1<G, 4>(GroupPlan, const u32*, const u32*, u32*, const uint4*, char*, u32*, char*);
 template __global__ void lemsm::k_merge_pairs<G>(GroupPlan, u32, MqLayout, const u32*, const u32*, const u32*, const char*, char*, u32*, uint4*);
-template __global__ void lemsm::k_merge_serial<G>(u32, MqLayout, const u32*, const uint4*, const char*, char*);
-template __global__ void lemsm::k_merge_waves<G>(u32, MqLayout, const u32*, const uint4*, const char*, char*, char*, u32*);
+template __global__ void lemsm::k_merge_queues<G>(u32, u32, MqLayout, const u32*, const uint4*, const char*, char*, char*, u32*);
 template __global__ void lemsm::k_merge_final<G>(u32, MqLayout, const u32*, const uint4*, const char*, char*, u32*);
 template __global__ void lemsm::k_pyramid<G>(const PyrTask*, u32, u32, u32, char*, u32);
 template __global__ void lemsm::k_pyramid_first2<G>(PyrFirst2Args, const u32*, char*, u32*);
diff --git a/halo2_liam_eagen_msm_amd/csrc/inst_fq_strict.hip b/halo2_liam_eagen_msm_amd/csrc/inst_fq_strict.hip
--- a/halo2_liam_eagen_msm_amd/csrc/inst_fq_strict.hip
+++ b/halo2_liam_eagen_msm_amd/csrc/inst_fq_strict.hip
@@ -3,8 +3,7 @@
 typedef XYZZ<Field32<FqParams>> G;
 template __global__ void lemsm::k_accum1<G, 4>(GroupPlan, const u32*, const u32*, u32*, const uint4*, char*, u32*, char*);
 template __global__ void lemsm::k_merge_pairs<G>(GroupPlan, u32, MqLayout, const u32*, const u32*, const u32*, const char*, char*, u32*, uint4*);
-template __global__ void lemsm::k_merge_serial<G>(u32, MqLayout, const u32*, const uint4*, const char*, char*);
-template __global__ void lemsm::k_merge_waves<G>(u32, MqLayout, const u32*, const uint4*, const char*, char*, char*, u32*);
+template __global__ void lemsm::k_merge_queues<G>(u32, u32, MqLayout, const u32*, const uint4*, const char*, char*, char*, u32*);
 template __global__ void lemsm::k_merge_final<G>(u32, MqLayout, const u32*, const uint4*, const char*, char*, u32*);
 template __global__ void lemsm::k_pyramid<G>(const PyrTask*, u32, u32, u32, char*, u32);
 template __global__ void lemsm::k_pyramid_first2<G>(PyrFirst2Args, const u32*, char*, u32*);
diff --git a/halo2_liam_eagen_msm_amd/csrc/inst_fr_lazy.hip b/halo2_liam_eagen_msm_amd/csrc/inst_fr_lazy.hip
--- a/halo2_liam_eagen_msm_amd/csrc/inst_fr_lazy.hip
+++ b/halo2_liam_eagen_msm_amd/csrc/inst_fr_lazy.hip
@@ -7,8 +7,7 @@
 template __global__ void lemsm::k_accum1<G, 3, true, true>(GroupPlan, const u32*, const u32*, u32*, const uint4*, char*, u32*, char*);
 template __global__ void lemsm::k_accum1<G, 4>(GroupPlan, const u32*, const u32*, u32*, const uint4*, char*, u32*, char*);
 template __global__ void lemsm::k_merge_pairs<G>(GroupPlan, u32, MqLayout, const u32*, const u32*, const u32*, const char*, char*, u32*, uint4*);
-template __global__ void lemsm::k_merge_serial<G>(u32, MqLayout, const u32*, const uint4*, const char*, char*);
-template __global__ void lemsm::k_merge_waves<G>(u32, MqLayout, const u32*, const uint4*, const char*, char*, char*, u32*);
+template __global__ void lemsm::k_merge_queues<G>(u32, u32, MqLayout, const u32*, const uint4*, const char*, char*, char*, u32*);
 template __global__ void lemsm::k_merge_final<G>(u32, MqLayout, const u32*, const uint4*, const char*, char*, u32*);
 template __global__ void lemsm::k_pyramid<G>(const PyrTask*, u32, u32, u32, char*, u32);
 template __global__ void lemsm::k_pyramid_first2<G>(PyrFirst2Args, const u32*, char*, u32*);
diff --git a/halo2_liam_eagen_msm_amd/csrc/inst_fr_strict.hip b/halo2_liam_eagen_msm_amd/csrc/inst_fr_strict.hip
--- a/halo2_liam_eagen_msm_amd/csrc/inst_fr_strict.hip
+++ b/halo2_liam_eagen_msm_amd/csrc/inst_fr_strict.hip
@@ -3,8 +3,7 @@
 typedef XYZZ<Field32<FrParams>> G;
 template __global__ void lemsm::k_accum1<G, 4>(GroupPlan, const u32*, const u32*, u32*, const uint4*, char*, u32*, char*);
 template __global__ void lemsm::k_merge_pairs<G>(GroupPlan, u32, MqLayout, const u32*, const u32*, const u32*, const char*, char*, u32*, uint4*);
-template __global__ void lemsm::k_merge_serial<G>(u32, MqLayout, const u32*, const uint4*, const char*, char*);
-template __global__ void lemsm::k_merge_waves<G>(u32, MqLayout, const u32*, const uint4*, const char*, char*, char*, u32*);
+template __global__ void lemsm::k_merge_queues<G>(u32, u32, MqLayout, const u32*, const uint4*, const char*, char*, char*, u32*);
 template __global__ void lemsm::k_merge_final<G>(u32, MqLayout, const u32*, const uint4*, const char*, char*, u32*);
 template __global__ void lemsm::k_pyramid<G>(const PyrTask*, u32, u32, u32, char*, u32);
 template __global__ void lemsm::k_pyramid_first2<G>(PyrFirst2Args, const u32*, char*, u32*);
diff --git a/halo2_liam_eagen_msm_amd/csrc/kernels.cuh b/halo2_liam_eagen_msm_amd/csrc/kernels.cuh
--- a/halo2_liam_eagen_msm_amd/csrc/kernels.cuh
+++ b/halo2_liam_eagen_msm_amd/csrc/kernels.cuh
@@ -22,7 +22,7 @@
           int BS = 256 >
 __global__ __launch_bounds__(BS) void k_pip_digits(const uint4* __restrict__ scalars, KAdd kadd, GroupPlan pl,
                                                     uint16_t* __restrict__ dig16, unsigned long long* __restrict__ signbm,
-                                                    u32* __restrict__ block_counts,
+                                                    u32* __restrict__ block_offs,
                                                     u32* __restrict__ bin_total, u32* __restrict__ err) {
   __shared__ u32 hist[MAX_BINS];
   const u32 tid = threadIdx.x, r = blockIdx.x;
@@ -90,8 +90,7 @@
     u32 cnt = hist[i];
     u32 wl = i / pl.BW, bin = i - wl * pl.BW;
     const size_t slot = ((size_t)wl * pl.nblk1 + r) * pl.BW + bin;
-    block_counts[slot] = cnt;
-    block_counts[(size_t)pl.nblk1 * pl.nbins + slot] = cnt ? atomicAdd(&bin_total[i], cnt) : 0u;
+    block_offs[slot] = cnt ? atomicAdd(&bin_total[i], cnt) : 0u;
   }
 }
 
@@ -148,7 +147,7 @@
 static const u32 STAGE2 = 8192;
 
 template <class Dec>
-__global__ __launch_bounds__(256) void k_count1(Dec dec, GroupPlan pl, u32* __restrict__ block_counts,
+__global__ __launch_bounds__(256) void k_count1(Dec dec, GroupPlan pl, u32* __restrict__ block_offs,
                                                 u32* __restrict__ bin_total) {
   __shared__ u32 hist[256];
   const u32 tid = threadIdx.x, wl = blockIdx.x, r = blockIdx.y, w = pl.w0 + wl;
@@ -182,8 +181,7 @@
   if (tid < pl.BW) {
     u32 cnt = hist[tid];
     const size_t slot = ((size_t)wl * pl.nblk1 + r) * pl.BW + tid;
-    block_counts[slot] = cnt;
-    block_counts[(size_t)pl.nblk1 * pl.nbins + slot] = cnt ? atomicAdd(&bin_total[wl * pl.BW + tid], cnt) : 0u;
+    block_offs[slot] = cnt ? atomicAdd(&bin_total[wl * pl.BW + tid], cnt) : 0u;
   }
 }
 
@@ -239,7 +237,7 @@
 
 template <class Dec, int STG , int BS = 256,
           bool LEAN = false >
-__global__ __launch_bounds__(BS) void k_scatter1(Dec dec, GroupPlan pl, const u32* __restrict__ block_counts,
+__global__ __launch_bounds__(BS) void k_scatter1(Dec dec, GroupPlan pl, const u32* __restrict__ block_offs ,
                                                  const u32* __restrict__ bin_start,
                                                  u32* __restrict__ entries, u32 xcd_windows ) {
   static_assert(BS == 256 || BS == 1024, "block size");
@@ -303,9 +301,16 @@
     }
   }
   const size_t crow = ((size_t)wl * pl.nblk1 + r) * pl.BW;
-  const u32* __restrict__ block_offs = block_counts + (size_t)pl.nblk1 * pl.nbins;
   u32 total;
   const bool few = !Dec::VEC && BS == 256 && !LEAN && pl.BW <= 16u;
+  if (!few) {
+    for (u32 i = tid; i < BW_MAX; i += BS) lcur[i] = 0;
+    __syncthreads();
+#pragma unroll
+    for (int k = 0; k < PER; k++)
+      if (bk[k]) atomicAdd(&lcur[((bk[k] & 0x7fffffffu) - 1u) >> pl.LB], 1u);
+    __syncthreads();
+  }
   if (few) {
     lcur[tid] = 0;
     __syncthreads();
@@ -323,7 +328,7 @@
     const u32 b0 = 2u * tid;
     const bool h = b0 < pl.BW;
     const uint2 z2 = make_uint2(0u, 0u);
-    const uint2 cnt = h ? *reinterpret_cast<const uint2*>(block_counts + crow + b0) : z2;
+    const uint2 cnt = h ? *reinterpret_cast<const uint2*>(&lcur[b0]) : z2;
     const uint2 clm = h ? *reinterpret_cast<const uint2*>(block_offs + crow + b0) : z2;
     const uint2 bs = h ? *reinterpret_cast<const uint2*>(bin_start + (size_t)wl * pl.BW + b0) : z2;
     const u32 off0 = block_excl_scan_256(cnt.x + cnt.y, &total, wsum), off1 = off0 + cnt.x;
@@ -331,7 +336,7 @@
     *reinterpret_cast<uint2*>(&lcur[b0]) = make_uint2(off0, off1);
   } else if constexpr (BS == 256) {
     const bool h0 = tid < pl.BW, h1 = tid + 256u < pl.BW;
-    u32 cnt0 = h0 ? block_counts[crow + tid] : 0u, cnt1 = h1 ? block_counts[crow + tid + 256u] : 0u;
+    u32 cnt0 = h0 ? lcur[tid] : 0u, cnt1 = h1 ? lcur[tid + 256u] : 0u;
     u32 g0 = h0 ? bin_start[wl * pl.BW + tid] + block_offs[crow + tid] : 0u;
     u32 g1 = h1 ? bin_start[wl * pl.BW + tid + 256u] + block_offs[crow + tid + 256u] : 0u;
     u32 total0, total1;
@@ -342,7 +347,7 @@
     lcur[tid] = off0; lcur[tid + 256u] = off1;
   } else {
     const bool h0 = tid < pl.BW;
-    u32 cnt0 = h0 ? block_counts[crow + tid] : 0u;
+    u32 cnt0 = h0 ? lcur[tid] : 0u;
     u32 g0 = h0 ? bin_start[wl * pl.BW + tid] + block_offs[crow + tid] : 0u;
     u32 off0 = block_excl_scan_1024(cnt0, &total, wsum);
     if (tid < BW_MAX) { delta[tid] = g0 - off0; lcur[tid] = off0; }
diff --git a/halo2_liam_eagen_msm_amd/csrc/kernels_ec.cuh b/halo2_liam_eagen_msm_amd/csrc/kernels_ec.cuh
--- a/halo2_liam_eagen_msm_amd/csrc/kernels_ec.cuh
+++ b/halo2_liam_eagen_msm_amd/csrc/kernels_ec.cuh
@@ -85,7 +85,7 @@
       key++; kend = kend2; kend2 = kend3;
       while (i >= kend) { key++; kend = kend2; kend2 = bucket_start[min(key + 2u, nkeys)]; }
       kbeg = i; seg_begin = i;
-      G::set_identity(acc); empty = true;
+      empty = true;
     }
     if (i + 1 < end) {
       if constexpr (RING) {
@@ -103,6 +103,8 @@
     if (!G::aff_is_identity(px, py)) {
       F::cneg(py, py, (e >> 31) != 0);
       if (ABI) G::madd_abi(acc, px, py, empty); else G::madd(acc, px, py, empty);
+    } else if (empty) {
+      G::set_identity(acc);
     }
   }
   flush(end);
@@ -198,17 +200,15 @@
 static const u32 MERGE_LDS_PAD_WORDS = 21504;
 
 template <class G>
-__global__ __launch_bounds__(256) void k_merge_serial(u32 scaled, MqLayout lay, const u32* __restrict__ mq_cnt,
-                                                      const uint4* __restrict__ mq_items, const char* __restrict__ rec_pt,
-                                                      char* __restrict__ bucket_sum) {
-  __shared__ u32 pad_[MERGE_LDS_PAD_WORDS];
-  if (scaled > 1) pad_[threadIdx.x] = scaled;
+__device__ __forceinline__ void merge_serial_block(u32 bid, u32 nblk, u32 scaled, const MqLayout& lay, const u32* __restrict__ mq_cnt,
+                                                   const uint4* __restrict__ mq_items, const char* __restrict__ rec_pt,
+                                                   char* __restrict__ bucket_sum) {
   const u32 cS = min(mq_cnt[MQ_S], lay.capS), cMall = min(mq_cnt[MQ_M], lay.capM);
   const u32 cM = cMall > lay.wave_th ? cMall : 0u;
   const u32 chS = (cS + 63u) >> 6, chM = (cM + 63u) >> 6;
   const u32 lane = threadIdx.x & 63u;
 #pragma unroll 1
-  for (u32 c = blockIdx.x + gridDim.x * (threadIdx.x >> 6); c < chS + chM; c += gridDim.x * 4u) {
+  for (u32 c = bid + nblk * (threadIdx.x >> 6); c < chS + chM; c += nblk * 4u) {
     uint4 it;
     if (c < chS) { const u32 v = 64u * c + lane; if (v >= cS) continue; it = mq_items[lay.offS + v]; }
     else { const u32 v = 64u * (c - chS) + lane; if (v >= cM) continue; it = mq_items[lay.offM + v]; }
@@ -225,18 +225,16 @@
 }
 
 template <class G>
-__global__ __launch_bounds__(256) void k_merge_waves(u32 scaled, MqLayout lay, const u32* __restrict__ mq_cnt,
-                                                     const uint4* __restrict__ mq_items, const char* __restrict__ rec_pt,
-                                                     char* __restrict__ partial, char* __restrict__ bucket_sum, u32* __restrict__ dbg) {
-  __shared__ u32 pad_[MERGE_LDS_PAD_WORDS];
-  if (scaled > 1) pad_[threadIdx.x] = scaled;
+__device__ __forceinline__ void merge_waves_block(u32 bid, u32 nblk, u32 scaled, const MqLayout& lay, const u32* __restrict__ mq_cnt,
+                                                  const uint4* __restrict__ mq_items, const char* __restrict__ rec_pt,
+                                                  char* __restrict__ partial, char* __restrict__ bucket_sum, u32* __restrict__ dbg) {
   const unsigned long long tk0 = __builtin_amdgcn_s_memtime();
   const u32 cMall = min(mq_cnt[MQ_M], lay.capM), cL = min(mq_cnt[MQ_L], lay.capL);
   const u32 lane = threadIdx.x & 63u;
-  const u32 nwaves = gridDim.x * 4u;
+  const u32 nwaves = nblk * 4u;
   const u32 cM = cMall > lay.wave_th ? 0u : cMall;
 #pragma unroll 1
-  for (u32 w = blockIdx.x * 4u + (threadIdx.x >> 6); w < cM + cL; w += nwaves) {
+  for (u32 w = bid * 4u + (threadIdx.x >> 6); w < cM + cL; w += nwaves) {
     const uint4 it = w < cM ? mq_items[lay.offM + w] : mq_items[lay.offL + (w - cM)];
     const u32 key = it.x, dst = it.w;
     typename G::pt acc;
@@ -249,6 +247,16 @@
     }
     if (dbg && w == 0 && lane == 0) { dbg[8] = (u32)(tk1 - tk0); dbg[9] = (u32)(tk2 - tk1); dbg[10] = (u32)(__builtin_amdgcn_s_memtime() - tk2); dbg[11] = it.z; }
   }
+}
+
+template <class G>
+__global__ __launch_bounds__(256) void k_merge_queues(u32 scaled, u32 nser, MqLayout lay, const u32* __restrict__ mq_cnt,
+                                                      const uint4* __restrict__ mq_items, const char* __restrict__ rec_pt,
+                                                      char* __restrict__ partial, char* __restrict__ bucket_sum, u32* __restrict__ dbg) {
+  __shared__ u32 pad_[MERGE_LDS_PAD_WORDS];
+  if (scaled > 1) pad_[threadIdx.x] = scaled;
+  if (blockIdx.x < nser) merge_serial_block<G>(blockIdx.x, nser, scaled, lay, mq_cnt, mq_items, rec_pt, bucket_sum);
+  else merge_waves_block<G>(blockIdx.x - nser, gridDim.x - nser, scaled, lay, mq_cnt, mq_items, rec_pt, partial, bucket_sum, dbg);
 }
 
 template <class G>
diff --git a/halo2_liam_eagen_msm_amd/csrc/lemsm.hip b/halo2_liam_eagen_msm_amd/csrc/lemsm.hip
--- a/halo2_liam_eagen_msm_amd/csrc/lemsm.hip
+++ b/halo2_liam_eagen_msm_amd/csrc/lemsm.hip
@@ -47,8 +47,7 @@
 }
 #define LEMSM_EXTERN_G(G)                                                                                   \
   extern template __global__ void lemsm::k_merge_pairs<G>(GroupPlan, u32, MqLayout, const u32*, const u32*, const u32*, const char*, char*, u32*, uint4*); \
-  extern template __global__ void lemsm::k_merge_serial<G>(u32, MqLayout, const u32*, const uint4*, const char*, char*); \
-  extern template __global__ void lemsm::k_merge_waves<G>(u32, MqLayout, const u32*, const uint4*, const char*, char*, char*, u32*); \
+  extern template __global__ void lemsm::k_merge_queues<G>(u32, u32, MqLayout, const u32*, const uint4*, const char*, char*, char*, u32*); \
   extern template __global__ void lemsm::k_merge_final<G>(u32, MqLayout, const u32*, const uint4*, const char*, char*, u32*); \
   extern template __global__ void lemsm::k_pyramid<G>(const PyrTask*, u32, u32, u32, char*, u32); \
   extern template __global__ void lemsm::k_pyramid_first2<G>(PyrFirst2Args, const u32*, char*, u32*); \
@@ -120,6 +119,8 @@
   uint32_t dbg_stamps[8] = {0, 0, 0, 0, 0, 0, 0, 0};
   uint64_t dbg_merge[4] = {0, 0, 0, 0};
   double accum_clock_mhz = 0;
+  std::vector<std::pair<size_t, size_t>> ws_cleared, ws_clear_next;
+  bool ws_clear_record = false;
   size_t bad_index = 0;
   size_t truncated = 0;
   std::map<std::vector<u32>, PyrCacheEntry> pyr_cache;
@@ -142,6 +143,7 @@
 }
 
 int reserve(lemsm_ctx* ctx, DevBuf& b, size_t bytes) {
+  if (&b == &ctx->ws) ctx->ws_cleared.clear();
   if (b.cap >= bytes) return LEMSM_OK;
   if (b.p) { HIPCHK(ctx, hipFree(b.p)); b.p = nullptr; b.cap = 0; }
   size_t want = bytes + bytes / 8 + 4096;
@@ -252,6 +254,15 @@
 
 template <class F> struct FieldTag {};
 
+int clear_ws(lemsm_ctx* ctx, char* p, size_t bytes, hipStream_t st) {
+  const size_t off = (size_t)(p - (char*)ctx->ws.p);
+  if (ctx->ws_clear_record) ctx->ws_clear_next.emplace_back(off, bytes);
+  for (auto it = ctx->ws_cleared.begin(); it != ctx->ws_cleared.end(); ++it)
+    if (it->first == off && it->second == bytes) { ctx->ws_cleared.erase(it); return LEMSM_OK; }
+  HIPCHK(ctx, hipMemsetAsync(p, 0, bytes, st));
+  return LEMSM_OK;
+}
+
 size_t align_up(size_t x, size_t a) { return (x + a - 1) / a * a; }
 
 struct GroupWs {
@@ -259,7 +270,7 @@
   char* arena;
   u32* bin_total; u32* bin_cursor; u32* bin_start; u32* tile_prefix; u32* meta;
   u32* bucket_count; u32* bucket_cursor; u32* bucket_start;
-  u32* block_counts;
+  u32* block_offs;
   uint16_t* dig16;
   unsigned long long* signbm;
   uint4* tile_info;
@@ -297,7 +308,7 @@
   w.zero_bytes_counters = o_arena - z0;
   size_t o_bin_start = take((MAX_BINS + 1) * 4), o_tile_prefix = take((MAX_BINS + 1) * 4), o_meta = take(64);
   size_t o_bstart = take(((size_t)NBpad + 1) * 4);
-  size_t o_blockc = take((size_t)pl.nblk1 * pl.nbins * 8);
+  size_t o_blockc = take((size_t)pl.nblk1 * pl.nbins * 4);
   size_t o_dig = take(pl.c ? (size_t)pl.dstride * (pl.w1 - pl.w0) * 2 + 64 : 16);
   size_t o_tinfo = take((size_t)pl.max_tiles * 16 + 16);
   size_t o_sbm = take(pl.c == 17 ? (size_t)(pl.w1 - pl.w0) * ((pl.n + 63) / 64) * 8 + 16 : 16);
@@ -313,7 +324,7 @@
     w.bucket_count = (u32*)(base + o_bcount); w.bucket_cursor = (u32*)(base + o_bcursor);
     w.arena = base + o_arena;
     w.bin_start = (u32*)(base + o_bin_start); w.tile_prefix = (u32*)(base + o_tile_prefix); w.meta = (u32*)(base + o_meta);
-    w.bucket_start = (u32*)(base + o_bstart); w.block_counts = (u32*)(base + o_blockc); w.dig16 = (uint16_t*)(base + o_dig); w.tile_info = (uint4*)(base + o_tinfo); w.signbm = (unsigned long long*)(base + o_sbm);
+    w.bucket_start = (u32*)(base + o_bstart); w.block_offs = (u32*)(base + o_blockc); w.dig16 = (uint16_t*)(base + o_dig); w.tile_info = (uint4*)(base + o_tinfo); w.signbm = (unsigned long long*)(base + o_sbm);
     w.entries = (u32*)(base + o_entries); w.sorted = (u32*)(base + o_sorted);
     w.rec_key = (u32*)(base + o_rk); w.rec_pt = base + o_rp;
     w.mq_cnt = (u32*)(base + o_mqcnt); w.mq_items = (uint4*)(base + o_mqi); w.mq_partial = base + o_mqp;
@@ -383,25 +394,25 @@
 struct PipProvider {
   const uint4* scalars; KAdd kadd;
   typedef PipDec Dec;
-  int prepare(lemsm_ctx*, hipStream_t st, const GroupPlan& pl, uint16_t* dig16, unsigned long long* signbm, u32* block_counts,
+  int prepare(lemsm_ctx*, hipStream_t st, const GroupPlan& pl, uint16_t* dig16, unsigned long long* signbm, u32* block_offs,
               u32* bin_total, u32* err, Dec& dec) const {
     dec.dig16 = dig16; dec.signbm = nullptr;
     if (pl.c == 17) {
       dec.signbm = signbm;
       if (pl.nblk1 < 2048)
-        hipLaunchKernelGGL((k_pip_digits<2, 1024>), dim3(pl.nblk1), dim3(1024), 0, st, scalars, kadd, pl, dig16, signbm, block_counts, bin_total, err);
+        hipLaunchKernelGGL((k_pip_digits<2, 1024>), dim3(pl.nblk1), dim3(1024), 0, st, scalars, kadd, pl, dig16, signbm, block_offs, bin_total, err);
       else
-        hipLaunchKernelGGL((k_pip_digits<2>), dim3(pl.nblk1), dim3(256), 0, st, scalars, kadd, pl, dig16, signbm, block_counts, bin_total, err);
+        hipLaunchKernelGGL((k_pip_digits<2>), dim3(pl.nblk1), dim3(256), 0, st, scalars, kadd, pl, dig16, signbm, block_offs, bin_total, err);
     } else if (pl.c == 16 && pl.W == 16) {
       if (pl.nblk1 < 1024)
-        hipLaunchKernelGGL((k_pip_digits<1, 1024>), dim3(pl.nblk1), dim3(1024), 0, st, scalars, kadd, pl, dig16, signbm, block_counts, bin_total, err);
+        hipLaunchKernelGGL((k_pip_digits<1, 1024>), dim3(pl.nblk1), dim3(1024), 0, st, scalars, kadd, pl, dig16, signbm, block_offs, bin_total, err);
       else
-        hipLaunchKernelGGL((k_pip_digits<1>), dim3(pl.nblk1), dim3(256), 0, st, scalars, kadd, pl, dig16, signbm, block_counts, bin_total, err);
+        hipLaunchKernelGGL((k_pip_digits<1>), dim3(pl.nblk1), dim3(256), 0, st, scalars, kadd, pl, dig16, signbm, block_offs, bin_total, err);
     } else {
       if (pl.nblk1 < 1024)
-        hipLaunchKernelGGL((k_pip_digits<0, 1024>), dim3(pl.nblk1), dim3(1024), 0, st, scalars, kadd, pl, dig16, signbm, block_counts, bin_total, err);
+        hipLaunchKernelGGL((k_pip_digits<0, 1024>), dim3(pl.nblk1), dim3(1024), 0, st, scalars, kadd, pl, dig16, signbm, block_offs, bin_total, err);
       else
-        hipLaunchKernelGGL((k_pip_digits<0>), dim3(pl.nblk1), dim3(256), 0, st, scalars, kadd, pl, dig16, signbm, block_counts, bin_total, err);
+        hipLaunchKernelGGL((k_pip_digits<0>), dim3(pl.nblk1), dim3(256), 0, st, scalars, kadd, pl, dig16, signbm, block_offs, bin_total, err);
     }
     return LEMSM_OK;
   }
@@ -409,9 +420,9 @@
 struct NegProvider {
   const uint8_t* digitsT;
   typedef NegDec Dec;
-  int prepare(lemsm_ctx*, hipStream_t st, const GroupPlan& pl, uint16_t*, unsigned long long*, u32* block_counts, u32* bin_total, u32*, Dec& dec) const {
+  int prepare(lemsm_ctx*, hipStream_t st, const GroupPlan& pl, uint16_t*, unsigned long long*, u32* block_offs, u32* bin_total, u32*, Dec& dec) const {
     dec.digitsT = digitsT;
-    hipLaunchKernelGGL((k_count1<NegDec>), dim3(pl.w1 - pl.w0, pl.nblk1), dim3(256), 0, st, dec, pl, block_counts, bin_total);
+    hipLaunchKernelGGL((k_count1<NegDec>), dim3(pl.w1 - pl.w0, pl.nblk1), dim3(256), 0, st, dec, pl, block_offs, bin_total);
     return LEMSM_OK;
   }
 };
@@ -466,22 +477,23 @@
 
   const bool first2 = L >= 5 && ctx->opt_pyr_first2 == 1 && nba == 1;
   RoctxRange rg_group("lemsm: window group (digits + sort + accumulate + tail enqueued)");
-  HIPCHK(ctx, hipMemsetAsync(ws_base + w.zero_begin, 0, (first2 || slab_k > 0) ? w.zero_bytes_counters : w.zero_bytes, st));
+  { int rcz = clear_ws(ctx, ws_base + w.zero_begin, (first2 || slab_k > 0) ? w.zero_bytes_counters : w.zero_bytes, st); if (rcz) return rcz; }
+  ctx->ws_clear_record = false;
   for (size_t g : w.guards) HIPCHK(ctx, hipMemsetAsync(ws_base + g, 0xA5, WS_GUARD, st));
 
   typename Prov::Dec dec;
-  { int rcp = prov.prepare(ctx, st, pl, w.dig16, w.signbm, w.block_counts, w.bin_total, w.err, dec); if (rcp) return rcp; }
+  { int rcp = prov.prepare(ctx, st, pl, w.dig16, w.signbm, w.block_offs, w.bin_total, w.err, dec); if (rcp) return rcp; }
   hipLaunchKernelGGL(k_binscan, dim3(1), dim3(1024), 0, st, pl, w.bin_total, w.bin_start, w.tile_prefix, w.meta);
   const u32 xw = (gw >= 8 && ctx->opt_xcd_windows != 1) ? 1u : 0u;
   dim3 g1 = xw ? dim3(8u * ((gw + 7) / 8) * pl.nblk1) : dim3(gw, pl.nblk1);
   if (pl.spb > 2 * STAGE)
-    hipLaunchKernelGGL((k_scatter1<typename Prov::Dec, 4 * STAGE, 1024>), g1, dim3(1024), 0, st, dec, pl, w.block_counts, w.bin_start, w.entries, xw);
+    hipLaunchKernelGGL((k_scatter1<typename Prov::Dec, 4 * STAGE, 1024>), g1, dim3(1024), 0, st, dec, pl, w.block_offs, w.bin_start, w.entries, xw);
   else if (pl.spb > STAGE)
-    hipLaunchKernelGGL((k_scatter1<typename Prov::Dec, 2 * STAGE>), g1, dim3(256), 0, st, dec, pl, w.block_counts, w.bin_start, w.entries, xw);
+    hipLaunchKernelGGL((k_scatter1<typename Prov::Dec, 2 * STAGE>), g1, dim3(256), 0, st, dec, pl, w.block_offs, w.bin_start, w.entries, xw);
   else if (Prov::Dec::VEC && (pl.BW & 1u) == 0 && ctx->opt_scatter_lean == 1)
-    hipLaunchKernelGGL((k_scatter1<typename Prov::Dec, STAGE, 256, true>), g1, dim3(256), 0, st, dec, pl, w.block_counts, w.bin_start, w.entries, xw);
+    hipLaunchKernelGGL((k_scatter1<typename Prov::Dec, STAGE, 256, true>), g1, dim3(256), 0, st, dec, pl, w.block_offs, w.bin_start, w.entries, xw);
   else
-    hipLaunchKernelGGL((k_scatter1<typename Prov::Dec, STAGE>), g1, dim3(256), 0, st, dec, pl, w.block_counts, w.bin_start, w.entries, xw);
+    hipLaunchKernelGGL((k_scatter1<typename Prov::Dec, STAGE>), g1, dim3(256), 0, st, dec, pl, w.block_offs, w.bin_start, w.entries, xw);
   const u32* d_sorted = w.entries;
   const u32* d_bstart = w.bin_start;
   if (pl.LB > 0) {
@@ -525,8 +537,8 @@
     const u32 sc = abi ? 1u : 0u;
     char* bsum = w.arena + ((size_t)ar.bucket_off + (size_t)slab_k * NBpad) * ptb;
     hipLaunchKernelGGL((k_merge_pairs<G>), dim3((pl.nthr1 + 255) / 256), dim3(256), 0, st, pl, sc, mq, d_bstart, w.meta, w.rec_key, w.rec_pt, bsum, w.mq_cnt, w.mq_items);
-    hipLaunchKernelGGL((k_merge_serial<G>), dim3(std::min(ctx->num_cus, std::max(1u, (mq.capS + mq.capM + 63) / 64))), dim3(256), 0, st, sc, mq, w.mq_cnt, w.mq_items, w.rec_pt, bsum);
-    hipLaunchKernelGGL((k_merge_waves<G>), dim3(std::min(ctx->num_cus, std::max(1u, (mq.capM + mq.capL + 3) / 4))), dim3(256), 0, st, sc, mq, w.mq_cnt, w.mq_items, w.rec_pt, w.mq_partial, bsum, w.mq_cnt);
+    const u32 nser = std::min(ctx->num_cus, std::max(1u, (mq.capS + mq.capM + 63) / 64)), nwav = std::min(ctx->num_cus, std::max(1u, (mq.capM + mq.capL + 3) / 4));
+    hipLaunchKernelGGL((k_merge_queues<G>), dim3(nser + nwav), dim3(256), 0, st, sc, nser, mq, w.mq_cnt, w.mq_items, w.rec_pt, w.mq_partial, bsum, w.mq_cnt);
     hipLaunchKernelGGL((k_merge_final<G>), dim3(std::min(ctx->num_cus, std::max(1u, (mq.capF + 3) / 4))), dim3(256), 0, st, sc, mq, w.mq_cnt, w.mq_items, w.mq_partial, bsum, w.mq_cnt);
   }
   RoctxRange rg_pyr("lemsm: bucket-reduction pyramid");
@@ -680,8 +692,15 @@
   size_t conv_bytes = G::CONVERTED_DOMAIN ? align_up(std::min(SLAB, n) * 64, 256) : 0;
   wr.nslabs = nslabs; wr.nrec = nrec; wr.ng = ng; wr.out_slab = out_slab; wr.SLAB = SLAB; wr.err_slot = ERR_SLOT; wr.err_stride = err_stride; wr.err_cap = err_bytes;
   wr.nw = nw; wr.nw_pad = nw_pad; wr.L = L; wr.ptb = ptb;
-  int rc = reserve(ctx, ctx->ws, ws_total + conv_bytes + out_slab * nrec + err_bytes + WinRun::STATUS_BYTES + 4096);
+  const size_t ws_need = ws_total + conv_bytes + out_slab * nrec + err_bytes + WinRun::STATUS_BYTES + 4096;
+  std::vector<std::pair<size_t, size_t>> kept;
+  if (ctx->ws.cap >= ws_need && ctx->opt_groups <= 1) kept.swap(ctx->ws_cleared);
+  int rc = reserve(ctx, ctx->ws, ws_need);
   if (rc) return rc;
+  ctx->ws_cleared.swap(kept);
+  ctx->ws_clear_next.clear();
+  ctx->ws_clear_record = ctx->opt_groups <= 1 && ctx->opt_ws_canary == 0;
+  struct ClearScope { lemsm_ctx* c; ~ClearScope() { c->ws_clear_record = false; c->ws_cleared.clear(); } } clear_scope{ctx};
   char* ws_base = (char*)ctx->ws.p;
   char* d_conv = ws_base + ws_total;
   char* d_out = d_conv + conv_bytes;
@@ -701,7 +720,7 @@
   ctx->t_accum_ms = 0; ctx->n_accum = 0;
   if (nw_pad != nw || n == 0 || nw == 0)
     HIPCHK(ctx, hipMemsetAsync(d_out, 0, out_slab * nrec, s_acc));
-  HIPCHK(ctx, hipMemsetAsync(d_err, 0, err_bytes + WinRun::STATUS_BYTES, s_acc));
+  { int rcz = clear_ws(ctx, d_err, err_bytes + WinRun::STATUS_BYTES, s_acc); if (rcz) return rcz; }
   u32 scaled_mask = 0;
   for (size_t k = 0; k < nslabs && n && nw; k++) {
     const size_t s0 = k * SLAB;
@@ -806,6 +825,10 @@
     if (err_bytes) HIPCHK(ctx, hipMemcpyAsync(hp + raw_bytes, wr.d_err, err_bytes, hipMemcpyDeviceToHost, s_tail));
   }
   HIPCHK(ctx, hipEventRecord(ctx->ev[1], s_tail));
+  ctx->ws_cleared.clear();
+  for (const auto& r : ctx->ws_clear_next) HIPCHK(ctx, hipMemsetAsync((char*)ctx->ws.p + r.first, 0, r.second, s_tail));
+  ctx->ws_cleared.swap(ctx->ws_clear_next);
+  ctx->ws_clear_next.clear();
   const auto th0 = std::chrono::steady_clock::now();
   HIPCHK(ctx, hipEventSynchronize(ctx->ev[1]));
   ctx->host_us[0] = std::chrono::duration<double, std::micro>(std::chrono::steady_clock::now() - th0).count();
diff --git a/halo2_liam_eagen_msm_amd/csrc/xyzz.cuh b/halo2_liam_eagen_msm_amd/csrc/xyzz.cuh
--- a/halo2_liam_eagen_msm_amd/csrc/xyzz.cuh
+++ b/halo2_liam_eagen_msm_amd/csrc/xyzz.cuh
@@ -51,7 +51,10 @@
   }
 
   static __device__ __forceinline__ void madd_abi(pt& acc, const fe& x2, const fe& y2, bool& empty) { madd(acc, x2, y2, empty); }
-  static __device__ __forceinline__ void madd(pt& acc, const fe& x2, const fe& y2, bool& empty) { madd(acc, x2, y2); empty = is_identity(acc); }
+  static __device__ __forceinline__ void madd(pt& acc, const fe& x2, const fe& y2, bool& empty) {
+    if (empty) { acc.x = x2; acc.y = y2; F::set_one(acc.zz); F::set_one(acc.zzz); empty = false; return; }
+    madd(acc, x2, y2); empty = is_identity(acc);
+  }
   static __device__ __forceinline__ void unscale(pt&) {}
   static __device__ __forceinline__ void scale(pt&) {}
 
diff --git a/halo2_liam_eagen_msm_amd/csrc/xyzz29.cuh b/halo2_liam_eagen_msm_amd/csrc/xyzz29.cuh
--- a/halo2_liam_eagen_msm_amd/csrc/xyzz29.cuh
+++ b/halo2_liam_eagen_msm_amd/csrc/xyzz29.cuh
@@ -51,6 +51,11 @@
     else { F::mul(r.zz, V, p.zz); F::mul(r.zzz, W, p.zzz); }
   }
 
+  static __device__ __forceinline__ void settle(fe& a) {
+    asm volatile("" : "+v"(a.l[0]), "+v"(a.l[1]), "+v"(a.l[2]), "+v"(a.l[3]), "+v"(a.l[4]), "+v"(a.l[5]), "+v"(a.l[6]), "+v"(a.l[7]), "+v"(a.l[8]));
+  }
+  static __device__ __forceinline__ void settle(pt& p) { settle(p.x); settle(p.y); settle(p.zz); settle(p.zzz); }
+
   static __device__ __forceinline__ void madd(pt& acc, const fe& x2, const fe& y2, bool& empty) {
     if (empty) {
       acc.x = x2; acc.y = y2; F::wnorm(acc.y); F::set_one(acc.zz); F::set_one(acc.zzz);
@@ -74,7 +79,7 @@
       if (F::is_zero_mod(R)) {
         pt a, res; a.x = x2; a.y = y2; F::set_one(a.zz); F::set_one(a.zzz);
         dbl_impl<true>(res, a);
-        acc = res;
+        acc = res; settle(acc);
       } else { set_identity(acc); empty = true; }
       return;
     }
@@ -107,7 +112,7 @@
         pt a, res; F::from_abi(a.x, x2a); F::from_abi(a.y, y2a); F::set_one(a.zz); F::set_one(a.zzz);
         dbl_impl<true>(res, a);
         F::from_abi(res.zz, res.zz); F::from_abi(res.zzz, res.zzz);
-        acc = res;
+        acc = res; settle(acc);
       } else { set_identity(acc); empty = true; }
       return;
     }
```

Result: no change. 882.3 million, median of 6 (+0.9%).
